# abraj/particleSystem

Hardware: AMD Instinct MI355X
Metric: particle-updates/sec at N=2^20 (higher is better)
Workload: dtype f32

## Files before the change

include/psamd.h:

```cpp
#ifndef PSAMD_H
#define PSAMD_H

#include <stddef.h>
#include <stdint.h>

#ifdef __cplusplus
extern "C" {
#endif

#define PSAMD_ABI_VERSION 8

#define PSAMD_MAX_RANKS 64

typedef enum psamd_status {
    PSAMD_OK = 0,
    PSAMD_ERR_INVALID_ARG   = 1,
    PSAMD_ERR_NO_DEVICE     = 2,
    PSAMD_ERR_HIP           = 3,
    PSAMD_ERR_OUT_OF_MEMORY = 4,
    PSAMD_ERR_OUTSIDE_BOX   = 5,
    PSAMD_ERR_QUEUE_EMPTY   = 6,
    PSAMD_ERR_CELL_OVERFLOW = 7,
    PSAMD_ERR_STATE         = 8,
    PSAMD_ERR_UNSUPPORTED   = 9
// ... 185 lines not shown
int psamd_build_grid(psamd_ctx *ctx);
int psamd_calc_forces(psamd_ctx *ctx);
int psamd_calc_forces_pairs(psamd_ctx *ctx);
int psamd_calc_forces_apply(psamd_ctx *ctx);
int psamd_step(psamd_ctx *ctx, int32_t nsteps);
int psamd_synchronize(psamd_ctx *ctx);
int psamd_set_run_ahead(psamd_ctx *ctx, int steps);

int psamd_download_force4(psamd_ctx *ctx, void *out_float4, int64_t first, int64_t count);

int psamd_snapshot_save(psamd_ctx *ctx);
int psamd_snapshot_restore(psamd_ctx *ctx);

typedef struct psamd_slab_plan {
    int32_t world, rank, grid_dim;
    int32_t cut_lo, cut_hi;
    int32_t state_lo, state_hi;
    int32_t below_lo, below_hi;
    int32_t above_lo, above_hi;
    int32_t lentin_lo, lentin_hi;
    int32_t lentout_lo, lentout_hi;
    int32_t send_up_lo, send_up_hi;
    int32_t send_down_lo, send_down_hi;
    int32_t slot_lo[4], slot_hi[4];
    int32_t rec_lo[4], rec_hi[4];
    int32_t up_rank, down_rank;
} psamd_slab_plan;
int psamd_slab_plan_describe(const psamd_config *cfg, psamd_slab_plan *out);
int psamd_get_slab_plan(const psamd_ctx *ctx, psamd_slab_plan *out);

typedef struct psamd_slab_buffers {
    void   *halo_out[2], *halo_in[2];
    int64_t halo_out_bytes[2], halo_in_bytes[2];
    void   *force_out, *force_in;
    int64_t force_out_bytes, force_in_bytes;
    void   *xfer_out[2], *xfer_in[2];
    int64_t xfer_bytes;
    void   *status_out, *status_in;
    int64_t status_bytes;
    void   *allg_out, *allg_in;
    int64_t allg_bytes;
    void   *xfer2_out[2], *xfer2_in[2];
    int64_t xfer2_bytes;
    void   *far_out, *far_in;
    int64_t far_bytes;
    int64_t xfer_bytes_max;
} psamd_slab_buffers;
int psamd_slab_buffers_get(psamd_ctx *ctx, psamd_slab_buffers *out);

int psamd_slab_build(psamd_ctx *ctx);
int psamd_slab_pairs_interior(psamd_ctx *ctx);
int psamd_slab_pairs(psamd_ctx *ctx);
int psamd_slab_apply(psamd_ctx *ctx);
int psamd_slab_finish(psamd_ctx *ctx);
int psamd_slab_msg_download(psamd_ctx *ctx, int which, void *host, int64_t bytes);
int psamd_slab_msg_upload(psamd_ctx *ctx, int which, const void *host, int64_t bytes);

int psamd_set_stream(psamd_ctx *ctx, void *hip_stream);
int psamd_get_stream(psamd_ctx *ctx, void **hip_stream_out);

int psamd_set_graphs(psamd_ctx *ctx, int enabled);
int psamd_get_graph_stats(psamd_ctx *ctx, int64_t *launches, int64_t *captures);
int psamd_set_wait_policy(psamd_ctx *ctx, int policy);

int psamd_export_live(psamd_ctx *ctx, const psamd_export *spec);
int psamd_download_live(psamd_ctx *ctx, uint32_t fields, void *pos4, void *vel4, void *acc4, int32_t *id,
                        int32_t *cell, int64_t capacity, int64_t *count);
int psamd_live_stats_get(psamd_ctx *ctx, psamd_live_stats *out);

int psamd_inject(psamd_ctx *ctx, const psamd_inject_spec *spec);
int psamd_inject_result_get(psamd_ctx *ctx, psamd_inject_result *out);

int psamd_remove(psamd_ctx *ctx, const psamd_remove_spec *spec);
int psamd_remove_result_get(psamd_ctx *ctx, psamd_remove_result *out);

int psamd_potential(psamd_ctx *ctx, const psamd_potential_spec *spec);
int psamd_potential_result_get(psamd_ctx *ctx, psamd_potential_result *out);
int psamd_download_potential(psamd_ctx *ctx, float *phi, int64_t capacity, psamd_potential_result *out);

int psamd_get_counters(psamd_ctx *ctx, psamd_counters *out);
int psamd_live_count(psamd_ctx *ctx, int64_t *out);
int psamd_device_view_get(psamd_ctx *ctx, psamd_device_view *out);
int psamd_debug_wave_trace(psamd_ctx *ctx, uint64_t *out, int64_t n_words);

int psamd_selftest_math(psamd_ctx *ctx, uint32_t lo_bits, uint32_t hi_bits, uint64_t out24[24]);
#define PSAMD_NUM_TIMERS 9
int psamd_set_timing(psamd_ctx *ctx, int level);
int psamd_set_timing_period(psamd_ctx *ctx, int every);
int psamd_get_timing(psamd_ctx *ctx, double us_out[PSAMD_NUM_TIMERS], int64_t *launches);
int psamd_get_timing_stats(psamd_ctx *ctx, double median_us[PSAMD_NUM_TIMERS], double max_us[PSAMD_NUM_TIMERS], int64_t *samples);

#ifdef __cplusplus
}
#endif
#endif
```

particlesystem_amd/__init__.py:

```python
import contextlib
import ctypes as C
import os

import numpy as np

from . import build as _build
from .slab import (HALO_OUT as MSG_HALO_OUT, HALO_IN as MSG_HALO_IN, FORCE_OUT as MSG_FORCE_OUT, FORCE_IN as MSG_FORCE_IN,
                   XFER_OUT as MSG_XFER_OUT, XFER_IN as MSG_XFER_IN, STATUS_OUT as MSG_STATUS_OUT, STATUS_IN as MSG_STATUS_IN,
                   ALLG_OUT as MSG_ALLG_OUT, ALLG_IN as MSG_ALLG_IN, XFER2_OUT as MSG_XFER2_OUT, XFER2_IN as MSG_XFER2_IN,
                   FAR_OUT as MSG_FAR_OUT, FAR_IN as MSG_FAR_IN)

HERE = os.path.dirname(os.path.abspath(__file__))
LIB_PATH = os.environ.get("PSAMD_LIB") or os.path.join(HERE, "libpsamd.so")

ABI_VERSION = 8
MAX_RANKS = 64
FLAG_EXPLOSIONS = 0x1
FLAG_FAST_MATH = 0x2
FLAG_ALL_PAIRS = 0x4
FLAG_EULER = 0x8
NUM_TIMERS = 9
TIMER_NAMES = ("hist", "scan", "scatter", "sort_cells", "pairs", "apply", "lifecycle", "init_iframe", "collide")

P_DTYPE = np.dtype({
# ... 139 lines not shown

def merge_potential(results):
    results = list(results)
    return {"listed": sum(int(r["listed"]) for r in results), "nonfinite": sum(int(r["nonfinite"]) for r in results),
            "potential": float(sum(float(r["potential"]) for r in results)),
            "phi_min": float(min(float(r["phi_min"]) for r in results)), "phi_max": float(max(float(r["phi_max"]) for r in results))}


def merge_live_stats(stats):
    stats = list(stats)
    out = {}
    for n, _ in LiveStats._fields_:
        vals = [np.asarray(s[n], np.float64) for s in stats]
        if n in ("lo", "age_min"):
            v = np.minimum.reduce(vals)
        elif n in ("hi", "age_max"):
            v = np.maximum.reduce(vals)
        else:
            v = vals[0]
            for x in vals[1:]:
                v = v + x
        out[n] = int(v) if n in ("live", "nonfinite") else (v if v.ndim else float(v))
    return out


class PsamdError(RuntimeError):
    def __init__(self, status, message):
        super().__init__("psamd status %d: %s" % (status, message))
        self.status = status


_vp, _i32, _i64 = C.c_void_p, C.c_int32, C.c_int64
_fp = C.POINTER(C.c_float)
_ip = C.POINTER(C.c_int32)
ABI = [
    ("psamd_abi_version", C.c_int, []),
    ("psamd_status_string", C.c_char_p, [C.c_int]),
    ("psamd_default_config", C.c_int, [C.POINTER(Config)]),
    ("psamd_create", C.c_int, [C.POINTER(Config), C.POINTER(_vp)]),
    ("psamd_destroy", C.c_int, [_vp]),
    ("psamd_last_error", C.c_char_p, [_vp]),
    ("psamd_get_sizes", C.c_int, [_vp, C.POINTER(Sizes)]),
    ("psamd_describe", C.c_int, [C.POINTER(Config), C.POINTER(Sizes), _vp, _vp, _vp, _vp]),
    ("psamd_get_config", C.c_int, [_vp, C.POINTER(Config)]),
    ("psamd_fill_particles", C.c_int, [_vp, _i64, _vp, _vp, _vp, _vp, _vp, _vp, C.POINTER(_i64)]),
    ("psamd_uniform_cloud", C.c_int, [_vp, _i64, C.c_uint32, _vp]),
    ("psamd_upload_particles", C.c_int, [_vp, _vp, _i64, _i64]),
    ("psamd_download_particles", C.c_int, [_vp, _vp, _i64, _i64]),
    ("psamd_download_tdata", C.c_int, [_vp, _vp, _i64, _i64]),
    ("psamd_upload_queues", C.c_int, [_vp, _vp, _vp]),
    ("psamd_download_queues", C.c_int, [_vp, _vp, _vp]),
    ("psamd_download_cellgrid", C.c_int, [_vp, _vp]),
    ("psamd_download_chunkgrid", C.c_int, [_vp, _vp]),
    ("psamd_download_force_counts", C.c_int, [_vp, _vp]),
    ("psamd_get_pkgdistrib", C.c_int, [_vp, _vp]),
    ("psamd_get_cell_table", C.c_int, [_vp, _vp]),
    ("psamd_get_gridmax", C.c_int, [_vp, _ip]),
    ("psamd_init_iframe", C.c_int, [_vp]),
    ("psamd_build_grid", C.c_int, [_vp]),
    ("psamd_calc_forces", C.c_int, [_vp]),
    ("psamd_calc_forces_pairs", C.c_int, [_vp]),
    ("psamd_calc_forces_apply", C.c_int, [_vp]),
    ("psamd_step", C.c_int, [_vp, _i32]),
    ("psamd_synchronize", C.c_int, [_vp]),
    ("psamd_download_force4", C.c_int, [_vp, _vp, _i64, _i64]),
    ("psamd_snapshot_save", C.c_int, [_vp]),
    ("psamd_snapshot_restore", C.c_int, [_vp]),
    ("psamd_set_stream", C.c_int, [_vp, _vp]),
    ("psamd_get_stream", C.c_int, [_vp, C.POINTER(C.c_void_p)]),
    ("psamd_slab_plan_describe", C.c_int, [C.POINTER(Config), C.POINTER(SlabPlan)]),
    ("psamd_get_slab_plan", C.c_int, [_vp, C.POINTER(SlabPlan)]),
    ("psamd_slab_buffers_get", C.c_int, [_vp, C.POINTER(SlabBuffers)]),
    ("psamd_slab_build", C.c_int, [_vp]),
    ("psamd_slab_pairs_interior", C.c_int, [_vp]),
    ("psamd_slab_pairs", C.c_int, [_vp]),
    ("psamd_slab_apply", C.c_int, [_vp]),
    ("psamd_slab_finish", C.c_int, [_vp]),
    ("psamd_slab_msg_download", C.c_int, [_vp, C.c_int, _vp, _i64]),
    ("psamd_slab_msg_upload", C.c_int, [_vp, C.c_int, _vp, _i64]),
    ("psamd_get_counters", C.c_int, [_vp, C.POINTER(Counters)]),
    ("psamd_live_count", C.c_int, [_vp, C.POINTER(_i64)]),
    ("psamd_device_view_get", C.c_int, [_vp, C.POINTER(DeviceView)]),
    ("psamd_debug_wave_trace", C.c_int, [_vp, _vp, _i64]),
    ("psamd_selftest_math", C.c_int, [_vp, C.c_uint32, C.c_uint32, C.POINTER(C.c_uint64)]),
    ("psamd_set_graphs", C.c_int, [_vp, C.c_int]),
    ("psamd_get_graph_stats", C.c_int, [_vp, C.POINTER(_i64), C.POINTER(_i64)]),
    ("psamd_set_wait_policy", C.c_int, [_vp, C.c_int]),
    ("psamd_set_timing", C.c_int, [_vp, C.c_int]),
    ("psamd_set_timing_period", C.c_int, [_vp, C.c_int]),
    ("psamd_get_timing", C.c_int, [_vp, C.POINTER(C.c_double), C.POINTER(_i64)]),
    ("psamd_get_timing_stats", C.c_int, [_vp, C.POINTER(C.c_double), C.POINTER(C.c_double), C.POINTER(_i64)]),
    ("psamd_set_run_ahead", C.c_int, [_vp, C.c_int]),
    ("psamd_set_tdata_mirror", C.c_int, [_vp, C.c_int]),
    ("psamd_export_live", C.c_int, [_vp, C.POINTER(Export)]),
    ("psamd_download_live", C.c_int, [_vp, C.c_uint32, _vp, _vp, _vp, _vp, _vp, _i64, C.POINTER(_i64)]),
    ("psamd_live_stats_get", C.c_int, [_vp, C.POINTER(LiveStats)]),
    ("psamd_inject", C.c_int, [_vp, C.POINTER(Inject)]),
    ("psamd_inject_result_get", C.c_int, [_vp, C.POINTER(InjectResult)]),
    ("psamd_remove", C.c_int, [_vp, C.POINTER(Remove)]),
    ("psamd_remove_result_get", C.c_int, [_vp, C.POINTER(RemoveResult)]),
    ("psamd_potential", C.c_int, [_vp, C.POINTER(Potential)]),
    ("psamd_potential_result_get", C.c_int, [_vp, C.POINTER(PotentialResult)]),
    ("psamd_download_potential", C.c_int, [_vp, _vp, _i64, C.POINTER(PotentialResult)]),
]

_lib = None


def build(force=False):
    return _build.build(force=force)


def load():
    global _lib
    if _lib is None:
        if not os.path.exists(LIB_PATH):
            raise RuntimeError("libpsamd.so is not built (run particlesystem_amd.build()); "
                               "the HIP library is the only implementation, there is no fallback")
        lib = C.CDLL(LIB_PATH)
        for name, res, args in ABI:
            fn = getattr(lib, name)
            fn.restype = res
            fn.argtypes = args
        have = lib.psamd_abi_version()
        if have != ABI_VERSION:
            raise RuntimeError("%s has ABI version %d, this module is written for %d: rebuild it (particlesystem_amd.build(force=True))"
                               % (LIB_PATH, have, ABI_VERSION))
        _lib = lib
    return _lib


def default_config(**over):
    cfg = Config()
    load().psamd_default_config(C.byref(cfg))
    for k, v in over.items():
        if k == "cuts":
            for i, c in enumerate(v):
                cfg.cuts[i] = c
        else:
            setattr(cfg, k, v)
    return cfg


def slab_plan(cfg):
    lib = load()
    plan = SlabPlan()
    st = lib.psamd_slab_plan_describe(C.byref(cfg), C.byref(plan))
    if st != 0:
        raise PsamdError(st, lib.psamd_status_string(st).decode())
    return plan


def _ptr(a):
    return None if a is None else a.ctypes.data_as(C.c_void_p)


def describe(cfg):
    lib = load()
    sizes = Sizes()
    st = lib.psamd_describe(C.byref(cfg), C.byref(sizes), None, None, None, None)
    if st != 0:
        raise PsamdError(st, lib.psamd_status_string(st).decode())
    table = np.zeros((sizes.num_cells, 3), np.int32)
    pkg = np.zeros((sizes.num_chunks, 54), np.int32)
    qi = np.zeros(sizes.queue_info_size, Q_DTYPE)
    q = np.zeros(sizes.container_size, np.int32)
# ... 310 lines not shown
            spec.flags = REMOVE_BOX | (REMOVE_OUTSIDE if outside else 0)
            for k in range(3):
                spec.lo[k], spec.hi[k] = float(box[0][k]), float(box[1][k])
        else:
            assert ids is not None and not outside, "remove: ids or box"
            m = int(ids.shape[0])
            assert ids.dtype == torch.int32 and ids.dim() == 1 and ids.is_contiguous() and ids.is_cuda, "remove: bad ids tensor"
            spec.max_count = m
            spec.ids = ids.data_ptr() if m > 0 else None
            if count is not None:
                assert count.dtype == torch.int64 and tuple(count.shape) == (1,) and count.is_cuda, "remove: bad count tensor"
                spec.count_dev = count.data_ptr()
            if outcome:
                out = torch.full((max(m, 1),), -1, dtype=torch.int32, device=dev)
                spec.outcome_dev = out.data_ptr()
        with self._on_stream(dev):
            self._ck(self.lib.psamd_remove(self.h, C.byref(spec)))
        res = self.remove_result()
        if out is not None:
            res["outcome"] = out[:int(ids.shape[0])]
        return res

    def remove_result(self):
        r = RemoveResult()
        self._ck(self.lib.psamd_remove_result_get(self.h, C.byref(r)))
        return r.to_dict()

    def potential(self, phi=False, capacity=None):
        import torch
        dev = torch.device("cuda", int(self.cfg.device))
        spec = Potential()
        result = torch.zeros(C.sizeof(PotentialResult), dtype=torch.uint8, device=dev)
        spec.result_dev = result.data_ptr()
        out = count = None
        if phi:
            capacity = self.owned_slots() if capacity is None else int(capacity)
            out = torch.empty(max(capacity, 1), dtype=torch.float32, device=dev)
            count = torch.zeros(1, dtype=torch.int64, device=dev)
            spec.phi, spec.capacity = out.data_ptr(), capacity
        with self._on_stream(dev):
            self._ck(self.lib.psamd_potential(self.h, C.byref(spec)))
            if phi:
                self._ck(self.lib.psamd_export_live(self.h, C.byref(Export(fields=0, capacity=0, count_dev=count.data_ptr()))))
        res = PotentialResult.from_device(result).to_dict()
        if phi:
            res["phi"] = out[:min(int(count.item()), capacity)]
        return res

    def potential_result(self):
        r = PotentialResult()
        self._ck(self.lib.psamd_potential_result_get(self.h, C.byref(r)))
        return r.to_dict()

    def download_potential(self, phi=True, capacity=None):
        r = PotentialResult()
        if not phi:
            self._ck(self.lib.psamd_download_potential(self.h, None, 0, C.byref(r)))
            return r.to_dict()
        capacity = self.owned_slots() if capacity is None else int(capacity)
        out = np.full(max(capacity, 1), np.nan, np.float32)
        self._ck(self.lib.psamd_download_potential(self.h, _ptr(out), capacity, C.byref(r)))
        res = r.to_dict()
        n = C.c_int64()
        self._ck(self.lib.psamd_download_live(self.h, 0, None, None, None, None, None, 0, C.byref(n)))
        res["phi"] = out[:min(n.value, capacity)]
        return res

    def energy(self):
        u = self.potential()["potential"]
        k = float(self.live_stats()["kinetic"])
        return {"kinetic": k, "potential": u, "total": k + u}

    def device_view(self):
        v = DeviceView()
        self._ck(self.lib.psamd_device_view_get(self.h, C.byref(v)))
        return v

    def wave_trace(self):
        n = 3 * (self.sizes.num_cells * ((self.sizes.max_per_cell + 63) // 64) + 4)
        out = np.zeros(n, np.uint64)
        self._ck(self.lib.psamd_debug_wave_trace(self.h, _ptr(out), n))
        return out.reshape(-1, 3)

    def selftest_math(self, lo_bits, hi_bits):
        out = (C.c_uint64 * 24)()
        self._ck(self.lib.psamd_selftest_math(self.h, lo_bits, hi_bits, out))
        return list(out)

    def set_graphs(self, on=True):
        self._ck(self.lib.psamd_set_graphs(self.h, 1 if on else 0))

    def graph_stats(self):
        a, b = C.c_int64(), C.c_int64()
        self._ck(self.lib.psamd_get_graph_stats(self.h, C.byref(a), C.byref(b)))
        return a.value, b.value

    def set_wait_policy(self, policy):
        self._ck(self.lib.psamd_set_wait_policy(self.h, int(policy)))

    def set_tdata_mirror(self, on):
        self._ck(self.lib.psamd_set_tdata_mirror(self.h, 1 if on else 0))

    def set_run_ahead(self, steps):
        self._ck(self.lib.psamd_set_run_ahead(self.h, int(steps)))

    def set_timing(self, on=True, every_stage=False, period=1):
        self._ck(self.lib.psamd_set_timing_period(self.h, int(period)))
        self._ck(self.lib.psamd_set_timing(self.h, (2 if every_stage else 1) if on else 0))

    def timing(self):
        us = (C.c_double * NUM_TIMERS)()
        n = C.c_int64()
        self._ck(self.lib.psamd_get_timing(self.h, us, C.byref(n)))
        return dict(zip(TIMER_NAMES, list(us))), n.value

    def timing_stats(self):
        med, mx = (C.c_double * NUM_TIMERS)(), (C.c_double * NUM_TIMERS)()
        n = C.c_int64()
        self._ck(self.lib.psamd_get_timing_stats(self.h, med, mx, C.byref(n)))
        return dict(zip(TIMER_NAMES, list(med))), dict(zip(TIMER_NAMES, list(mx))), n.value
```

particlesystem_amd/csrc/apply.hip:

```cpp
#include "kernels_common.hpp"

namespace psamd {

struct ApplyEmit {
    int id, new_cell, new_rec, old_chunk;
    unsigned bits;
};

__global__ __launch_bounds__(1024) void k_apply(DevParams P, SegLayout S, const StepState *__restrict__ stp,
                                                const uint8_t *__restrict__ flag_slot,
                                                float4 *pos4, float4 *vel4, float4 *acc4,
                                                int *cell_arr, uint8_t *pflags,
                                                const CellInfo *__restrict__ celltab,
                                                uint64_t *op_keys, int *op_args, int ops_cap,
                                                MoveRec *moves, int moves_cap,
                                                Outboxes out,
                                                const int *__restrict__ chunk_count, const uint8_t *__restrict__ chunk_skip,
                                                FrameScalars *fs, DevCounters *ctr)
{
    constexpr int ITEMS = 1;
    __shared__ int s_ops, s_moves, s_base_ops, s_base_moves;
    __shared__ unsigned int s_cnt[4];
    if (threadIdx.x == 0) { s_ops = 0; s_moves = 0; s_cnt[0] = s_cnt[1] = s_cnt[2] = s_cnt[3] = 0; }
    const int chunk_over = fs->chunk_over;
    const int step = (P.flags & PSAMD_FLAG_EXPLOSIONS) ? stp->step : 0;
    int old_cells[ITEMS];
    bool any_active = false;
#pragma unroll
    for (int it = 0; it < ITEMS; it++) {
        const int si = (blockIdx.x * ITEMS + it) * 1024 + (int)threadIdx.x;
        int oc = -1;
        if (si < P.slots_total) oc = cell_arr[si];
        if (oc <= -2) { cell_arr[si] = -1; oc = -1; }
        bool act = oc >= 0 && oc < P.num_cells_global;
        if (chunk_over && act && chunk_count[celltab[oc].chunk] > P.max_per_chunk && chunk_skip[si]) act = false;
        old_cells[it] = act ? oc : -1;
        any_active |= act;
    }
    if (!__syncthreads_or(any_active)) return;

    ApplyEmit em[ITEMS];
    int n_op = 0, n_mv = 0;
    unsigned cnt_moved = 0, cnt_surv = 0, cnt_age = 0, cnt_coll = 0;
#pragma unroll
    for (int it = 0; it < ITEMS; it++) {
        const int si = (blockIdx.x * ITEMS + it) * 1024 + (int)threadIdx.x;
        const int old_cell = old_cells[it];
        const bool active = old_cell >= 0;
        const int id = active ? slot_of_index(P, si) : 0;

    int flag = 0, new_cell = 0;
    float4 f = make_float4(0.f, 0.f, 0.f, 0.f);
    float4 p = f, v = f;
    float fert = 0.f;
    uint8_t pf0 = 0;
    if (active) { p = pos4[si]; v = vel4[si]; f = acc4[si]; pf0 = pflags[si]; flag = (int)flag_slot[si]; fert = f.w; }
    const CellInfo old_ci = active ? celltab[old_cell] : CellInfo{0, 1, 0, 0};

    const bool killed = active && flag == 2, survived = active && flag == 1, moved = active && flag == 0;
    bool died_of_age = false, born = false, relocate = false;
    int new_rec = 0;

    if (killed) {
        died_of_age = v.w > P.life_thr;
        cell_arr[si] = -1; pflags[si] = 0;
        pos4[si] = make_float4(0.f, 0.f, 0.f, 0.f);
        vel4[si] = make_float4(0.f, 0.f, 0.f, 0.f);
        acc4[si] = make_float4(0.f, 0.f, 0.f, 0.f);
    } else if (survived) {
        vel4[si] = make_float4(0.f, 0.f, 0.f, 0.f);
        acc4[si] = make_float4(0.f, 0.f, 0.f, fert);
        pflags[si] = 0;
    } else if (moved) {
        float axv = f.x, ayv = f.y, azv = f.z;
        const float t = P.t;
        if (P.drag > 0.f) { axv -= P.drag * v.x; ayv -= P.drag * v.y; azv -= P.drag * v.z; }
        float dx = (float)((double)(v.x * t) + ((0.5 * (double)axv) * (double)t) * (double)t);
        float dy = (float)((double)(v.y * t) + ((0.5 * (double)ayv) * (double)t) * (double)t);
        float dz = (float)((double)(v.z * t) + ((0.5 * (double)azv) * (double)t) * (double)t);
        if (P.flags & PSAMD_FLAG_EULER) { dx = v.x * t; dy = v.y * t; dz = v.z * t; }
        dx = clamp_mag(dx, P.dmax); dy = clamp_mag(dy, P.dmax); dz = clamp_mag(dz, P.dmax);
        float rx = p.x + dx, ry = p.y + dy, rz = p.z + dz;

        const int G = P.G;
        const double cs = P.cell_size;
        auto to_int = [](double d) { return (d >= -2147483648.0 && d < 2147483648.0) ? (int)d : (int)0x80000000; };
        int i1 = to_int(floor((-1.0 * (double)ry) / cs) + (double)(G / 2));
        int i2 = to_int(floor((1.0 * (double)rx) / cs) + (double)(G / 2));
        int i3 = to_int(floor((-1.0 * (double)rz) / cs) + (double)(G / 2));
        for (int guard = 0; guard < 64 &&
             !((i1 >= 0 && i1 < G) && (i2 >= 0 && i2 < G) && (i3 >= 0 && i3 < G)); guard++) {
            if (!(i1 >= 0 && i1 < G)) { const int o = i1; i1 = (i1 + G) % G; ry = (float)((double)ry + (-1.0 * (double)(i1 - o) * cs)); }
            if (!(i2 >= 0 && i2 < G)) { const int o = i2; i2 = (i2 + G) % G; rx = (float)((double)rx + ((double)(i2 - o) * cs)); }
            if (!(i3 >= 0 && i3 < G)) { const int o = i3; i3 = (i3 + G) % G; rz = (float)((double)rz + (-1.0 * (double)(i3 - o) * cs)); }
        }
        i1 = min(max(i1, 0), G - 1); i2 = min(max(i2, 0), G - 1); i3 = min(max(i3, 0), G - 1);
        new_cell = i3 * G * G + i1 * G + i2;

        float vx = v.x + axv * t, vy = v.y + ayv * t, vz = v.z + azv * t;
        vx = clamp_mag(vx, P.vmax); vy = clamp_mag(vy, P.vmax); vz = clamp_mag(vz, P.vmax);
        const float age = v.w + t;
        uint8_t pf = pf0;
        const CellInfo new_ci = celltab[new_cell];
        new_rec = segment_record(S, new_ci.seg_type, new_ci.seg_tid);

        if ((P.flags & PSAMD_FLAG_EXPLOSIONS) && (age >= fert) && !(pf & 1)) {
            const uint64_t h0 = splitmix64(P.seed ^ ((uint64_t)(uint32_t)step << 32) ^ (uint64_t)(uint32_t)id);
            const uint64_t h1 = splitmix64(h0), h2 = splitmix64(h1);
            const int r0 = (int)((double)(h0 >> 11) * (1.0 / 9007199254740992.0) * 100.0) - 50;
            const int r1 = (int)((double)(h1 >> 11) * (1.0 / 9007199254740992.0) * 100.0) - 50;
            const int r2 = (int)((double)(h2 >> 11) * (1.0 / 9007199254740992.0) * 100.0) - 50;
            float ux = (float)r0, uy = (float)r1, uz = (float)r2;
            const float mag = sqrtf((float)((double)(ux * ux) + (double)(uy * uy) + (double)(uz * uz)));
            ux /= mag; uy /= mag; uz /= mag;
            vx = (float)((double)ux * P.expl_speed);
            vy = (float)((double)uy * P.expl_speed);
            vz = (float)((double)uz * P.expl_speed);
            pf |= 1;
            born = true;
        }
        pos4[si] = make_float4(rx, ry, rz, p.w);
        vel4[si] = make_float4(vx, vy, vz, age);
        if (P.drag > 0.f) acc4[si] = make_float4(axv, ayv, azv, fert);
        cell_arr[si] = new_cell;
        pflags[si] = pf;
        relocate = (new_ci.seg_type != old_ci.seg_type || new_ci.seg_tid != old_ci.seg_tid);
    }

    const bool remote_ = (born || relocate) && P.world > 1 && !owns_record(P, new_rec);
    const int GG = P.G * P.G;
    const int layers_up = ((new_cell / GG) - (old_cell / GG) + P.G) % P.G;
    bool up_ = remote_ && (layers_up == 1 || layers_up == 2);
    bool hop2_ = false, far_ = false;
    if (remote_ && !nbr_owns_record(P, up_ ? 1 : 0, new_rec)) {
        const bool near2 = layers_up == 1 || layers_up == 2 || layers_up >= P.G - 2;
        if (nbr_owns_record(P, up_ ? 0 : 1, new_rec)) up_ = !up_;
        else if (P.xfer2_cap > 0 && (near2 || P.far_cap <= 0)) hop2_ = true;
        else if (P.far_cap > 0) far_ = true;
        else atomicOr(&fs->error, ERR_FOREIGN_CELL);
    }

        em[it].id = id; em[it].new_cell = new_cell; em[it].new_rec = new_rec; em[it].old_chunk = old_ci.chunk;
        em[it].bits = (killed ? 1u : 0u) | (born ? 2u : 0u) | (relocate ? 4u : 0u) | (remote_ ? 8u : 0u) | (up_ ? 16u : 0u) | (hop2_ ? 32u : 0u) | (far_ ? 64u : 0u);
        n_op += (killed ? 1 : 0) + ((born && !remote_) ? 1 : 0) + (relocate ? (remote_ ? 1 : 2) : 0);
        n_mv += (born ? 1 : 0) + (relocate ? 1 : 0);
        cnt_moved += (unsigned)__popcll(__ballot(moved)); cnt_surv += (unsigned)__popcll(__ballot(survived));
        cnt_age += (unsigned)__popcll(__ballot(killed && died_of_age)); cnt_coll += (unsigned)__popcll(__ballot(killed && !died_of_age));
    }
// ... 9 lines not shown
        if (cnt_surv) atomicAdd(&s_cnt[1], cnt_surv);
        if (cnt_age) atomicAdd(&s_cnt[2], cnt_age);
        if (cnt_coll) atomicAdd(&s_cnt[3], cnt_coll);
    }
    wave_ops = __shfl(wave_ops, 63); wave_moves = __shfl(wave_moves, 63);
    __syncthreads();
    if (threadIdx.x == 0) {
        DevCounters *mine = ctr + (blockIdx.x % COUNTER_COPIES);
        if (s_cnt[0]) atomicAdd(&mine->integrated, (unsigned long long)s_cnt[0]);
        if (s_cnt[1]) atomicAdd(&mine->survives, (unsigned long long)s_cnt[1]);
        if (s_cnt[2]) atomicAdd(&mine->deaths_age, (unsigned long long)s_cnt[2]);
        if (s_cnt[3]) atomicAdd(&mine->deaths_collision, (unsigned long long)s_cnt[3]);
        if (s_ops | s_moves) {
            const unsigned long long both = ((unsigned long long)(unsigned)s_moves << 32) | (unsigned)s_ops;
            const unsigned long long old = atomicAdd((unsigned long long *)&fs->n_ops, both);
            s_base_ops = (int)(old & 0xffffffffull); s_base_moves = (int)(old >> 32);
        }
    }
    __syncthreads();
    int k = s_base_ops + wave_ops + op_incl - n_op;
    int m = s_base_moves + wave_moves + mv_incl - n_mv;
    const bool room = k + n_op <= ops_cap && m + n_mv <= moves_cap;
    if (!room && (n_op || n_mv)) atomicOr(&fs->error, ERR_OPS_OVERFLOW);
#pragma unroll
    for (int it = 0; it < ITEMS; it++) {
        const unsigned bits = (room && (n_op || n_mv)) ? em[it].bits : 0u;
        const bool killed = bits & 1u, born = bits & 2u, relocate = bits & 4u, remote = bits & 8u, up = bits & 16u, hop2 = bits & 32u, far = bits & 64u;
        const int id = em[it].id, new_cell = em[it].new_cell;
        const int own_r = segment_record_of_slot(S, id);
        const int box = far ? 4 : (up ? 1 : 0) + (hop2 ? 2 : 0);
        int out_base[2] = {0, 0};
        if (P.world > 1) {
#pragma unroll
            for (int dir = 0; dir < 5; dir++) {
                if (dir >= 2 && (dir == 4 ? P.far_cap : P.xfer2_cap) <= 0) continue;
                const bool mine = remote && box == dir;
                const int want = mine ? ((born ? 1 : 0) + (relocate ? 1 : 0)) : 0;
                if (__any(want > 0)) {
                    const int incl = wave_incl_scan(want);
                    int base = 0;
                    if (lane == 63) base = atomicAdd(&fs->n_out[dir], incl);
                    base = __shfl(base, 63) + incl - want;
                    if (mine) { out_base[1] = base; out_base[0] = base + (born ? 1 : 0); }
                }
            }
        }
        if (!(bits & 7u)) continue;
        const uint64_t key = ((uint64_t)(uint32_t)(em[it].old_chunk + 1) << P.key_chunk_shift) | ((uint64_t)(uint32_t)id << 2);
        const uint64_t own_rec = (uint64_t)(uint32_t)own_r << P.key_rec_shift;
        const uint64_t dst_rec = (uint64_t)(uint32_t)em[it].new_rec << P.key_rec_shift;
        auto depart = [&](int kind, uint64_t sub) -> int {
            const int o = out_base[kind];
            if (o >= (far ? P.far_cap : hop2 ? P.xfer2_cap : P.xfer_cap)) { atomicOr(&fs->error, ERR_HALO_OVERFLOW); return -1; }
            XferRec *x = out.o[box] + o;
            x->key = dst_rec | key | sub; x->new_cell = new_cell; x->kind = kind;
            return o;
        };
        if (killed) { op_keys[k] = own_rec | key | 2ull; op_args[k] = id; k++; }
        if (born) {
            if (remote) moves[m] = {id, depart(1, 0ull), 1 | MOVE_OUT | (up ? MOVE_UP : 0) | (hop2 ? MOVE_HOP2 : 0) | (far ? MOVE_FAR : 0), new_cell};
            else {
                moves[m] = {id, -1, 1, new_cell};
                op_keys[k] = dst_rec | key | 0ull; op_args[k] = m;
                k++;
            }
            m++;
        }
        if (relocate) {
            if (remote) moves[m] = {id, depart(0, 1ull), 0 | MOVE_OUT | (up ? MOVE_UP : 0) | (hop2 ? MOVE_HOP2 : 0) | (far ? MOVE_FAR : 0), new_cell};
            else {
                moves[m] = {id, -1, 0, new_cell};
                op_keys[k] = dst_rec | key | 1ull; op_args[k] = m;
                k++;
            }
            m++;
            op_keys[k] = own_rec | key | 2ull; op_args[k] = id; k++;
        }
    }
}

hipError_t launch_apply(hipStream_t st, const DevParams &P, const SegLayout &S, const DeviceState &d)
{
    if (P.slots_total <= 0) return hipSuccess;
    k_apply<<<(P.slots_total + 1023) / 1024, 1024, 0, st>>>(P, S, d.st, d.flag_slot, d.pos4, d.vel4, d.acc4, d.cell, d.pflags, d.celltab,
                                                        d.op_keys, d.op_args, d.ops_cap, d.moves, d.moves_cap,
                                                        Outboxes{{d.xfer_out[0], d.xfer_out[1], d.xfer_out[2], d.xfer_out[3], d.xfer_out[4]}},
                                                        d.chunk_count, d.chunk_skip, d.fs, d.ctr);
    PS_LAUNCH_CHECK();
    return hipSuccess;
}

}
```

particlesystem_amd/csrc/create.hip:

```cpp
#include <cmath>
#include <new>

#include "context.hpp"

const char *psamd::status_text(int s)
{
    switch (s) {
    case PSAMD_OK: return "ok";
    case PSAMD_ERR_INVALID_ARG: return "invalid argument";
    case PSAMD_ERR_NO_DEVICE: return "no usable HIP device (the HIP path is the only path)";
    case PSAMD_ERR_HIP: return "HIP runtime error";
    case PSAMD_ERR_OUT_OF_MEMORY: return "out of device memory";
    case PSAMD_ERR_OUTSIDE_BOX: return "particle location outside box";
    case PSAMD_ERR_QUEUE_EMPTY: return "overflow: reserved space of the segment is full";
    case PSAMD_ERR_CELL_OVERFLOW: return "cell or queue-op capacity exceeded on device";
    case PSAMD_ERR_STATE: return "stage called out of order";
    case PSAMD_ERR_UNSUPPORTED: return "unsupported";
    }
    return "unknown status";
}

extern "C" {

int psamd_abi_version(void) { return PSAMD_ABI_VERSION; }
// ... 171 lines not shown
    d.cell_count = frame; d.chunk_count = frame + LC; d.rec_count = d.chunk_count + g.num_chunks;
    d.rec_cursor = d.rec_count + g.queue_infos;
    d.halo_count = d.rec_cursor + g.queue_infos;
    d.active_count = d.halo_count + LC;
    d.task_ready = d.active_count + LC;
    c->frame_ints = frame_ints;
    PS_HIP(c, dev_alloc(c, &d.halo_f, (size_t)3 * LC * HALO_CAP + 64));
    PS_HIP(c, dev_alloc(c, &d.halo_id, LC * HALO_CAP + 64));
    PS_HIP(c, dev_alloc(c, &d.active_list, SC));
    PS_HIP(c, dev_alloc(c, &d.snap_cid, SC));
    PS_HIP(c, dev_alloc(c, &d.task_list2, LC * P.slices));
    PS_HIP(c, dev_alloc(c, &d.merged_tasks, LC));
    PS_HIP(c, dev_alloc(c, &d.task_cost, LC));
    PS_HIP(c, dev_alloc(c, &d.ctask_start, 2 * LC + 2));
    PS_HIP(c, dev_alloc(c, &d.cost_start, 2 * LC + 2));
    PS_HIP(c, dev_alloc(c, &d.wave_pos, (size_t)MAX_PAIR_WAVES + 1));
    PS_HIP(c, dev_alloc(c, &d.rec_start, (size_t)g.queue_infos + 1));
    PS_HIP(c, dev_alloc(c, &d.fs, 1));
    PS_HIP(c, dev_alloc(c, &d.st, 1));
    PS_HIP(c, hipMemsetAsync(d.st, 0, sizeof(StepState), c->stream));
    PS_HIP(c, dev_alloc(c, &d.cell_start, LC + 1));
    PS_HIP(c, dev_alloc(c, &d.cursor, LC));
    PS_HIP(c, dev_alloc(c, &d.task_start, LC + 1));
    PS_HIP(c, dev_alloc(c, &d.task_list, LC * P.slices));
    PS_HIP(c, dev_alloc(c, &d.sorted_id, SC));
    PS_HIP(c, dev_alloc(c, &d.flag_slot, C));
    PS_HIP(c, dev_alloc(c, &d.snap_soa, 4 * (size_t)P.sorted_cap + 64));
    PS_HIP(c, dev_alloc(c, &d.snap_age, SC));
    PS_HIP(c, dev_alloc(c, &d.force4, SC));
    PS_HIP(c, dev_alloc(c, &d.celltab, (size_t)g.num_cells));
    if (P.flags & PSAMD_FLAG_ALL_PAIRS) {
        d.part_tasks = (int)(SC / 64 + 1);
        PS_HIP(c, dev_alloc(c, &d.part_acc, (size_t)ALLP_PARTS * d.part_tasks * 64));
        PS_HIP(c, dev_alloc(c, &d.act_start, LC + 1));
        PS_HIP(c, dev_alloc(c, &d.dense_gi, SC));
        PS_HIP(c, dev_alloc(c, &d.dense_cell, SC));
    }
    PS_HIP(c, dev_alloc(c, &d.chunk_skip, C));
    PS_HIP(c, dev_alloc(c, &d.chunk_segs, (size_t)g.num_chunks * 27));
    {
        std::vector<int2> segs((size_t)g.num_chunks * 27);
        for (int ch = 0; ch < g.num_chunks; ch++) {
            Pair pk[27];
            g.chunk_segments(ch, pk);
            for (int j = 0; j < 27; j++) {
                const int k = seg_index(pk[j].c);
                segs[(size_t)ch * 27 + j] = make_int2(g.seg_base[k] + pk[j].p * g.seg_size_t[k], g.seg_size_t[k]);
            }
            std::sort(segs.begin() + (size_t)ch * 27, segs.begin() + (size_t)ch * 27 + 27, [](const int2 &a, const int2 &b) { return a.x < b.x; });
        }
        PS_HIP(c, hipMemcpy(d.chunk_segs, segs.data(), segs.size() * sizeof(int2), hipMemcpyHostToDevice));
    }
    PS_HIP(c, dev_alloc(c, &d.op_keys, (size_t)d.ops_cap));
    PS_HIP(c, dev_alloc(c, &d.op_keys_sorted, (size_t)d.ops_cap));
    PS_HIP(c, dev_alloc(c, &d.op_args, (size_t)d.ops_cap));
    PS_HIP(c, dev_alloc(c, &d.op_args_sorted, (size_t)d.ops_cap));
    PS_HIP(c, hipHostMalloc((void **)&c->h_fs, 2 * sizeof(FrameScalars), hipHostMallocMapped | hipHostMallocCoherent));
    std::memset(c->h_fs, 0, 2 * sizeof(FrameScalars));
    PS_HIP(c, hipHostGetDevicePointer((void **)&c->d.fs_host, c->h_fs, 0));
    PS_HIP(c, dev_alloc(c, &d.moves, (size_t)d.moves_cap));
    PS_HIP(c, dev_alloc(c, &d.stage, 3 * (size_t)d.moves_cap));
    PS_HIP(c, dev_alloc(c, &d.ctr, (size_t)COUNTER_COPIES));
    PS_HIP(c, dev_alloc(c, &d.exp_count, (size_t)slot_tiles(P.slots_total)));
    PS_HIP(c, dev_alloc(c, &d.exp_tiles, (size_t)slot_tiles(P.slots_total)));
    PS_HIP(c, dev_alloc(c, &d.exp_out, 1));
    PS_HIP(c, dev_alloc(c, &d.pot_sorted, SC));
    PS_HIP(c, dev_alloc(c, &d.pot_slot, C));
    PS_HIP(c, dev_alloc(c, &d.pot_tiles, (size_t)slot_tiles(P.slots_total)));
    PS_HIP(c, dev_alloc(c, &d.pot_count, (size_t)slot_tiles(P.slots_total)));
    PS_HIP(c, dev_alloc(c, &d.pot_out, 1));
    PS_HIP(c, hipMemsetAsync(d.pot_out, 0, sizeof(PotOut), c->stream));
    PS_HIP(c, dev_alloc(c, &c->inj.removed, (size_t)g.queue_infos));
    PS_HIP(c, dev_alloc(c, &c->inj.hdr, 2));
    PS_HIP(c, dev_alloc(c, &c->inj.own, 1));
    PS_HIP(c, hipMemsetAsync(c->inj.own, 0, sizeof(psamd_inject_result), c->stream));
    PS_HIP(c, dev_alloc(c, &c->rem.claim, C));
    PS_HIP(c, dev_alloc(c, &c->rem.ins, (size_t)g.queue_infos));
    PS_HIP(c, dev_alloc(c, &c->rem.prefix, C + 1));
    PS_HIP(c, dev_alloc(c, &c->rem.tile_sel, (size_t)slot_tiles(P.slots_total)));
    PS_HIP(c, dev_alloc(c, &c->rem.tile_live, (size_t)slot_tiles(P.slots_total)));
    PS_HIP(c, dev_alloc(c, &c->rem.own, 1));
    PS_HIP(c, hipMemsetAsync(c->rem.own, 0, sizeof(psamd_remove_result), c->stream));
    PS_HIP(c, dev_alloc(c, &d.trace, 3 * (LC * P.slices + 4)));
    PS_HIP(c, hipMemsetAsync(d.trace, 0, 3 * (LC * P.slices + 4) * sizeof(unsigned long long), c->stream));
    return PSAMD_OK;
}

static hipError_t alloc_msg(psamd_ctx *c, int which, size_t bytes, size_t alloc = 0)
{
    SlabMsg &m = c->msg[which];
    m.bytes = bytes; m.alloc = alloc ? alloc : bytes;
    const hipError_t e = dev_alloc(c, &m.ptr, m.alloc / sizeof(int));
    return e != hipSuccess ? e : hipMemsetAsync(m.ptr, 0, m.alloc, c->stream);
}

static int alloc_slab_msgs(psamd_ctx *c)
{
    const Geometry &g = c->geo; const DevParams &P = c->P; const SlabPlan &pl = c->plan; DeviceState &d = c->d;
    if (P.world <= 1) return PSAMD_OK;
    const int GG = g.G * g.G;
    auto halo_bytes = [&](int cells) { return ((size_t)MSG_HEADER_WORDS + (size_t)cells + 6 * (size_t)cells * P.halo_cap_cell) * sizeof(int); };
        c->halo_out_cells[0] = (pl.send_down_hi - pl.send_down_lo) * GG; c->halo_out_c0[0] = (pl.send_down_lo - pl.state_lo) * GG;
        c->halo_out_cells[1] = (pl.send_up_hi - pl.send_up_lo) * GG;     c->halo_out_c0[1] = (pl.send_up_lo - pl.state_lo) * GG;
        c->halo_in_cells[0] = (pl.below_hi - pl.below_lo) * GG;
        c->halo_in_cells[1] = (pl.above_hi - pl.above_lo) * GG;
    for (int k = 0; k < 2; k++) {
        if (c->halo_out_cells[k] > 0) {
            PS_HIP(c, alloc_msg(c, MSG_HALO_OUT + k, halo_bytes(c->halo_out_cells[k])));
            PS_HIP(c, dev_alloc(c, &c->pack_off[k], (size_t)c->halo_out_cells[k] + 1));
        }
        if (c->halo_in_cells[k] > 0) {
            PS_HIP(c, alloc_msg(c, MSG_HALO_IN + k, halo_bytes(c->halo_in_cells[k])));
            PS_HIP(c, dev_alloc(c, &c->unpack_off[k], (size_t)c->halo_in_cells[k] + 1));
        }
    }
    auto force_bytes = [&](int cells) { return ((size_t)MSG_HEADER_WORDS + 4 * (size_t)cells * P.halo_cap_cell) * sizeof(int); };
    if (P.reg_layers[2] > 0) PS_HIP(c, alloc_msg(c, MSG_FORCE_OUT, force_bytes(P.reg_layers[2] * GG)));
    if (P.lentout_c1 > P.lentout_c0) PS_HIP(c, alloc_msg(c, MSG_FORCE_IN, force_bytes(P.lentout_c1 - P.lentout_c0)));
    for (int k = 0; k < 2; k++) {
        PS_HIP(c, alloc_msg(c, MSG_XFER_OUT + k, xfer_msg_bytes((size_t)P.xfer_cap + 1), xfer_msg_bytes(xfer_room(P))));
        PS_HIP(c, alloc_msg(c, MSG_XFER_IN + k, xfer_msg_bytes((size_t)P.xfer_cap + 1), xfer_msg_bytes(xfer_room(P))));
    }
    for (int k = 0; k < 2 && P.xfer2_cap > 0; k++) {
        PS_HIP(c, alloc_msg(c, MSG_XFER2_OUT + k, xfer_msg_bytes((size_t)P.xfer2_cap)));
        PS_HIP(c, alloc_msg(c, MSG_XFER2_IN + k, xfer_msg_bytes((size_t)P.xfer2_cap)));
    }
    if (P.far_cap > 0) {
        PS_HIP(c, alloc_msg(c, MSG_FAR_OUT, xfer_msg_bytes((size_t)P.far_cap)));
        PS_HIP(c, alloc_msg(c, MSG_FAR_IN, xfer_msg_bytes((size_t)P.far_cap) * (size_t)P.world));
    }
    const int outbox[5] = {MSG_XFER_OUT, MSG_XFER_OUT + 1, MSG_XFER2_OUT, MSG_XFER2_OUT + 1, MSG_FAR_OUT};
    for (int k = 0; k < 5; k++)
        if (c->msg[outbox[k]].ptr) d.xfer_out[k] = reinterpret_cast<XferRec *>(c->msg[outbox[k]].ptr + MSG_HEADER_WORDS);
    if (P.flags & PSAMD_FLAG_ALL_PAIRS) {
        const size_t block = (size_t)P.allg_block * sizeof(int);
        PS_HIP(c, alloc_msg(c, MSG_ALLG_OUT, block));
        PS_HIP(c, alloc_msg(c, MSG_ALLG_IN, block * P.world, block * P.world + 64 * sizeof(int)));
            PS_HIP(c, dev_alloc(c, &d.gstart, (size_t)g.num_cells + 1));
            PS_HIP(c, dev_alloc(c, &d.gn, (size_t)g.num_cells + 1));
            PS_HIP(c, hipMemsetAsync(d.gstart, 0, ((size_t)g.num_cells + 1) * sizeof(int), c->stream));
            PS_HIP(c, hipMemsetAsync(d.gn, 0, ((size_t)g.num_cells + 1) * sizeof(int), c->stream));
        d.allg_in = c->msg[MSG_ALLG_IN].ptr;
    }
    PS_HIP(c, alloc_msg(c, MSG_STATUS_OUT, (size_t)P.status_words * sizeof(int)));
    PS_HIP(c, alloc_msg(c, MSG_STATUS_IN, (size_t)P.status_words * sizeof(int) * P.world));
    d.status_out = c->msg[MSG_STATUS_OUT].ptr;
    return PSAMD_OK;
}

static int probe_eps_f32(psamd_ctx *c, const psamd_config *cfg)
{
    DevParams &P = c->P;
    if (P.lean_math && cfg->eps2 > 0) {
        const float d2_max = (float)max_d2(c->geo);
        unsigned long long *bad = (unsigned long long *)c->d.fs;
        auto fbits = [](float f) { uint32_t u; std::memcpy(&u, &f, 4); return u; };
        for (double mult : {1.5, 2.0, 4.0, 8.0, 16.0, 64.0}) {
            const float from = (float)(mult * cfg->eps2);
            if (!(from < d2_max)) break;
            unsigned long long h_bad = 1;
            PS_HIP(c, hipMemsetAsync(bad, 0, sizeof(unsigned long long), c->stream));
            PS_HIP(c, launch_validate_eps(c->stream, fbits(from), fbits(d2_max), cfg->eps2, P.eps2f, bad));
            PS_HIP(c, hipMemcpyAsync(&h_bad, bad, sizeof h_bad, hipMemcpyDeviceToHost, c->stream));
            PS_HIP(c, hipStreamSynchronize(c->stream));
            if (h_bad == 0) { P.eps_f32_from = from; break; }
        }
    }
    P.slow_below = std::max(P.eps_f32_from, std::nextafterf(P.coll_d2_gate, INFINITY));
    return PSAMD_OK;
}

static void split_interior(psamd_ctx *c)
{
    const Geometry &g = c->geo; const DevParams &P = c->P; const SlabPlan &pl = c->plan;
    const int GG = g.G * g.G, lo = std::max(pl.cut_lo, pl.state_lo), hi = std::min(pl.cut_hi, pl.state_hi);
    auto own = [&](int l) { return l < 0 || l >= g.G || (l >= pl.state_lo && l < pl.state_hi); };
    int i0 = lo, i1 = lo;
    for (int l = lo; l < hi; l++) if (own(l - 1) && own(l + 1)) { if (i1 == i0) i0 = l; i1 = l + 1; } else if (i1 > i0) break;
    c->P_int = P; c->P_rest = P;
    c->have_interior = P.world > 1 && P.two_pass && P.lean_math && i1 > i0 && (i1 - i0) < (hi - lo) + (pl.lentin_hi - pl.lentin_lo)
                       && !(P.flags & PSAMD_FLAG_ALL_PAIRS);
    if (c->have_interior) {
        const int a = (i0 - pl.state_lo) * GG, b = (i1 - pl.state_lo) * GG;
        c->P_int.comp_lo[0] = a; c->P_int.comp_hi[0] = b;
        c->P_int.comp_lo[1] = c->P_int.comp_hi[1] = c->P_int.comp_lo[2] = c->P_int.comp_hi[2] = 0;
        c->P_rest.comp_lo[1] = P.own_comp0; c->P_rest.comp_hi[1] = a;
        c->P_rest.comp_lo[2] = b; c->P_rest.comp_hi[2] = P.own_comp1;
    }
}

static int init_state(psamd_ctx *c)
{
    const Geometry &g = c->geo; const DevParams &P = c->P; DeviceState &d = c->d;
    const size_t C = (size_t)P.slots_total, SC = (size_t)P.sorted_cap + 64, LC = (size_t)P.n_local_cells;
    c->wait_policy = P.world > 1 ? 1 : 0;
    if (const char *lim = std::getenv("PSAMD_WAIT_LIMIT_S")) c->wait_limit_s = std::max(0.05, std::atof(lim));
    for (float4 *a : {d.pos4, d.vel4, d.acc4}) PS_HIP(c, hipMemsetAsync(a, 0, std::max<size_t>(C, 1) * sizeof(float4), c->stream));
    PS_HIP(c, hipMemsetAsync(d.pflags, 0, std::max<size_t>(C, 1), c->stream));
    PS_HIP(c, hipMemsetAsync(d.force4, 0, SC * sizeof(float4), c->stream));
    PS_HIP(c, hipMemsetAsync(d.flag_slot, 0, std::max<size_t>(C, 1), c->stream));
    PS_HIP(c, hipMemsetAsync(d.fs, 0, sizeof(FrameScalars), c->stream));
    PS_HIP(c, hipMemsetAsync(d.ctr, 0, sizeof(DevCounters) * COUNTER_COPIES, c->stream));
    PS_HIP(c, hipMemsetAsync(d.cell_count, 0, c->frame_ints * sizeof(int), c->stream));
    PS_HIP(c, hipMemsetAsync(d.cell_start, 0, (LC + 1) * sizeof(int), c->stream));
    PS_HIP(c, launch_fill_int(c->stream, d.cell, -1, C));
    PS_HIP(c, launch_fill_int(c->stream, c->rem.claim, INT32_MAX, C));
    PS_HIP(c, launch_init_tdata(c->stream, P, d));
    g.initial_queues(c->h_qinfo, c->h_queue);
    c->celltab = g.cell_table();
    PS_HIP(c, hipMemcpyAsync(d.celltab, c->celltab.data(), c->celltab.size() * sizeof(CellInfo), hipMemcpyHostToDevice, c->stream));
    {
        const int cell_off = P.reg_first[0] * g.G * g.G;
        std::vector<int> order((size_t)std::max(P.n_own_cells, 1), 0);
        for (int lc = 0; lc < P.n_own_cells; lc++) order[(size_t)lc] = lc;
        std::stable_sort(order.begin(), order.begin() + P.n_own_cells, [&](int a, int b) {
            const CellInfo &x = c->celltab[(size_t)(a + cell_off)], &y = c->celltab[(size_t)(b + cell_off)];
            if (x.chunk != y.chunk) return x.chunk < y.chunk;
            if (x.seg_type != y.seg_type) return x.seg_type < y.seg_type;
            return x.seg_tid < y.seg_tid;
        });
        PS_HIP(c, dev_alloc(c, &d.cell_order, order.size()));
        PS_HIP(c, hipMemcpy(d.cell_order, order.data(), order.size() * sizeof(int), hipMemcpyHostToDevice));
    }
    return push_queues(c);
}

int psamd_create(const psamd_config *cfg, psamd_ctx **out)
{
    if (!cfg || !out) return PSAMD_ERR_INVALID_ARG;
    *out = nullptr;
    psamd_ctx *c = new (std::nothrow) psamd_ctx();
    if (!c) return PSAMD_ERR_OUT_OF_MEMORY;
    *out = c;
    if (!c->geo.init(*cfg)) return fail(c, PSAMD_ERR_INVALID_ARG, "bad configuration (chunk_dim >= 3, sizes > 0, container < 2^31)");
    if (cfg->world < 1 || cfg->world > PSAMD_MAX_RANKS || cfg->rank < 0 || cfg->rank >= cfg->world) return fail(c, PSAMD_ERR_INVALID_ARG, "rank/world");
    const Geometry &g = c->geo;
    c->plan = plan_for(g, *cfg);
    if (!c->plan.valid) return fail(c, PSAMD_ERR_UNSUPPORTED, "no slab partition for this grid and world size (every rank needs >= 2 cell layers "
                                                                "and its neighbours must hold every layer it reads)");

    int ndev = 0;
    if (hipGetDeviceCount(&ndev) != hipSuccess || ndev <= 0) return fail(c, PSAMD_ERR_NO_DEVICE, "hipGetDeviceCount found none");
    if (cfg->device < 0 || cfg->device >= ndev) return fail(c, PSAMD_ERR_NO_DEVICE, "device ordinal out of range");
    PS_HIP(c, hipSetDevice(cfg->device));
    PS_HIP(c, hipStreamCreateWithFlags(&c->own_stream, hipStreamNonBlocking));
    c->stream = c->own_stream;
    PS_HIP(c, hipStreamCreateWithFlags(&c->d.side_stream, hipStreamNonBlocking));
    PS_HIP(c, hipEventCreateWithFlags(&c->d.ev_fork, hipEventDisableTiming));
    PS_HIP(c, hipEventCreateWithFlags(&c->d.ev_join, hipEventDisableTiming));

    int rc = derive_params(c, cfg);
    if (rc == PSAMD_OK) rc = alloc_step_arrays(c);
    if (rc == PSAMD_OK) rc = alloc_slab_msgs(c);
    if (rc == PSAMD_OK) rc = probe_eps_f32(c, cfg);
    if (rc != PSAMD_OK) return rc;
    split_interior(c);
    return init_state(c);
}

int psamd_destroy(psamd_ctx *c)
{
    if (!c) return PSAMD_OK;
    if (c->stream) (void)hipStreamSynchronize(c->stream);
    drop_graphs(c);
    for (void *p : c->allocs) (void)hipFree(p);
    if (c->staging) (void)hipFree(c->staging);
    for (const EntryScratch &e : {c->inj.e, c->rem.e})
        for (void *p : {(void *)e.ent, (void *)e.tcount, (void *)e.tile_out}) if (p) (void)hipFree(p);
    if (c->h_fs) (void)hipHostFree(c->h_fs);
    if (c->ev_made) for (auto &set : c->ev) for (auto &e : set) (void)hipEventDestroy(e);
    if (c->d.ev_fork) (void)hipEventDestroy(c->d.ev_fork);
    if (c->d.ev_join) (void)hipEventDestroy(c->d.ev_join);
    if (c->d.side_stream) (void)hipStreamDestroy(c->d.side_stream);
    if (c->own_stream) (void)hipStreamDestroy(c->own_stream);
    delete c;
    return PSAMD_OK;
}

static void fill_sizes(const Geometry &g, psamd_sizes *o)
{
    std::memset(o, 0, sizeof *o);
    o->grid_dim = g.G; o->num_cells = g.num_cells; o->num_chunks = g.num_chunks;
    o->cells_per_chunk = g.cells_per_chunk; o->max_per_cell = g.max_per_cell; o->max_per_chunk = g.max_per_chunk;
    o->container_size = g.container; o->queue_info_size = g.queue_infos;
    o->n_chunkgrid = (int64_t)g.num_chunks * (1 + (int64_t)g.max_per_chunk);
    o->n_cellgrid = (int64_t)g.num_cells * (1 + (int64_t)g.max_per_cell);
    o->n_pkgdistrib = g.num_chunks * 27;
    for (int k = 0; k < 4; k++) { o->seg_count[k] = g.seg_count[k]; o->seg_size_t[k] = g.seg_size_t[k]; o->seg_size[k] = g.seg_size[k]; }
// ... 66 lines not shown
```

particlesystem_amd/csrc/grid.hip:

```cpp
#include "kernels_common.hpp"

namespace psamd {

__global__ void k_unpack_aos(DevParams P, const uint32_t *__restrict__ aos, int first, int count, float half_box,
                             float4 *pos4, float4 *vel4, float4 *acc4, int *cell, uint8_t *pflags,
                             FrameScalars *fs)
{
    const int i = blockIdx.x * blockDim.x + threadIdx.x;
    if (i >= count) return;
    const uint32_t *r = aos + (size_t)18 * i;
    const int slot = first + i;
    if ((int)r[0] != slot) atomicOr(&fs->error, ERR_BAD_ID);
    const int si = slot_index(P, slot);
    if (si < 0) return;
    if ((int)r[1] >= 0) {
        const float x = __uint_as_float(r[9]), y = __uint_as_float(r[10]), z = __uint_as_float(r[11]);
        bool bad = (int)r[1] >= P.num_cells_global;
        if (!bad) {
            const int c = (int)r[1], G = P.G, i3 = c / (G * G), i1 = (c - i3 * G * G) / G, i2 = c - i3 * G * G - i1 * G;
            const float cs = (float)P.cell_size, tol = 1e-4f * cs, h = (float)(G / 2);
            int lost = (int)0x80000000;
            for (int guard = 0; guard < 4 && !(lost >= 0 && lost < G); guard++) lost = (lost + G) % G;
            auto axis_ok = [&](float v, float sign, int idx) {
                if ((__float_as_uint(v) & 0x7f800000u) == 0x7f800000u) return idx == lost;
                if (!(fabsf(v) <= half_box)) return false;
                const float u = (sign * v / cs + h - (float)idx) * cs;
                return u >= -tol && u <= cs + tol;
            };
            bad = !(axis_ok(x, 1.0f, i2) && axis_ok(y, -1.0f, i1) && axis_ok(z, -1.0f, i3));
        }
        if (bad) atomicOr(&fs->error, ERR_BAD_POS);
    }
    cell[si] = (int)r[1];
    if ((int)r[1] < 0) {
        pflags[si] = 0;
        pos4[si] = vel4[si] = acc4[si] = make_float4(0.f, 0.f, 0.f, 0.f);
        return;
    }
    pflags[si] = ((r[5] >> 8) & 0xffu) ? 1 : 0;
    pos4[si] = make_float4(__uint_as_float(r[9]), __uint_as_float(r[10]), __uint_as_float(r[11]), __uint_as_float(r[6]));
    vel4[si] = make_float4(__uint_as_float(r[12]), __uint_as_float(r[13]), __uint_as_float(r[14]), __uint_as_float(r[7]));
    acc4[si] = make_float4(__uint_as_float(r[15]), __uint_as_float(r[16]), __uint_as_float(r[17]), __uint_as_float(r[8]));
}

__global__ void k_pack_aos(DevParams P, uint32_t *__restrict__ aos, int first, int count,
                           const float4 *pos4, const float4 *vel4, const float4 *acc4, const int *cell,
                           const uint8_t *pflags, const CellInfo *celltab)
{
    const int i = blockIdx.x * blockDim.x + threadIdx.x;
    if (i >= count) return;
    uint32_t *r = aos + (size_t)18 * i;
    const int slot = first + i;
    const int si = slot_index(P, slot);
    const int c = si >= 0 ? cell[si] : -1;
    CellInfo ci = {-1, -1, -1, 0};
    if (c >= 0 && c < P.num_cells_global) ci = celltab[c];
    const float4 zero = make_float4(0.f, 0.f, 0.f, 0.f);
    const float4 p = si >= 0 ? pos4[si] : zero, v = si >= 0 ? vel4[si] : zero, a = si >= 0 ? acc4[si] : zero;
    r[0] = (uint32_t)slot; r[1] = (uint32_t)c; r[2] = (uint32_t)ci.chunk;
    r[3] = (uint32_t)ci.seg_type; r[4] = (uint32_t)ci.seg_tid;
    r[5] = (si >= 0 && pflags[si]) ? 0x100u : 0u;
    r[6] = __float_as_uint(p.w); r[7] = __float_as_uint(v.w); r[8] = __float_as_uint(a.w);
    r[9] = __float_as_uint(p.x); r[10] = __float_as_uint(p.y); r[11] = __float_as_uint(p.z);
    r[12] = __float_as_uint(v.x); r[13] = __float_as_uint(v.y); r[14] = __float_as_uint(v.z);
    r[15] = __float_as_uint(a.x); r[16] = __float_as_uint(a.y); r[17] = __float_as_uint(a.z);
}

__global__ void k_place(DevParams P, int n, const int *__restrict__ ids, const float4 *__restrict__ p,
                        const float4 *__restrict__ v, const float4 *__restrict__ a,
                        const int *__restrict__ cells, float4 *pos4, float4 *vel4, float4 *acc4,
                        int *cell, uint8_t *pflags)
{
    const int i = blockIdx.x * blockDim.x + threadIdx.x;
    if (i >= n) return;
    const int si = slot_index(P, ids[i]);
    if (si < 0) return;
    pos4[si] = p[i]; vel4[si] = v[i]; acc4[si] = a[i];
    cell[si] = cells[i]; pflags[si] = 0;
}

__global__ void k_restore(int n, const float4 *__restrict__ s_pos, const float4 *__restrict__ s_vel,
                          const float4 *__restrict__ s_acc, const int *__restrict__ s_cell,
                          const uint8_t *__restrict__ s_flags, const int *__restrict__ s_queue,
                          const int *__restrict__ s_qinfo, int qinfo_words, int step, StepState *st,
                          float4 *pos4, float4 *vel4, float4 *acc4, int *cell, uint8_t *pflags, int *queue, int *qinfo)
{
    const int i = blockIdx.x * blockDim.x + threadIdx.x;
    if (i == 0) { st->step = step; st->pending = 0; }
    if (i < qinfo_words) qinfo[i] = s_qinfo[i];
    if (i >= n) return;
    queue[i] = s_queue[i];
    const int cs = s_cell[i];
    if (cs < 0 && cell[i] < 0) return;
    pos4[i] = s_pos[i]; vel4[i] = s_vel[i]; acc4[i] = s_acc[i];
    cell[i] = cs; pflags[i] = s_flags[i];
}

hipError_t launch_restore(hipStream_t st, int n, const void *s_pos, const void *s_vel, const void *s_acc,
                          const void *s_cell, const void *s_flags, const void *s_queue, const void *s_qinfo, int qinfo_words,
                          int step, const DeviceState &d)
{
    const int threads = std::max(std::max(n, qinfo_words), 1);
    k_restore<<<(threads + 255) / 256, 256, 0, st>>>(n, (const float4 *)s_pos, (const float4 *)s_vel, (const float4 *)s_acc,
                                                    (const int *)s_cell, (const uint8_t *)s_flags, (const int *)s_queue,
                                                    (const int *)s_qinfo, qinfo_words, step, d.st, d.pos4, d.vel4, d.acc4,
                                                    d.cell, d.pflags, d.queue, (int *)d.qinfo);
    return hipGetLastError();
}

__global__ void k_fill_int(int *p, int v, size_t n)
{
    size_t i = (size_t)blockIdx.x * blockDim.x + threadIdx.x;
    const size_t stride = (size_t)gridDim.x * blockDim.x;
    for (; i < n; i += stride) p[i] = v;
}

__global__ void k_init_tdata(DevParams P, uint32_t *tdata)
{
    const int i = blockIdx.x * blockDim.x + threadIdx.x;
    if (i >= P.slots_total) return;
    uint32_t *r = tdata + (size_t)6 * i;
    r[0] = (uint32_t)slot_of_index(P, i); r[1] = r[2] = r[3] = r[4] = r[5] = 0u;
}

__device__ __forceinline__ int hist_window(const DevParams &P, const int (&mine)[SLOTS_PER_WG / 1024], int *s_min)
{
    if (P.n_own_cells <= LDS_CELLS) return 0;
    if (threadIdx.x == 0) *s_min = 0x7fffffff;
    __syncthreads();
    int m = 0x7fffffff;
#pragma unroll
    for (int i = 0; i < SLOTS_PER_WG / 1024; i++) if (mine[i] >= 0) m = min(m, mine[i]);
    for (int d = 32; d > 0; d >>= 1) m = min(m, __shfl_xor(m, d));
    if ((threadIdx.x & 63) == 0 && m != 0x7fffffff) atomicMin(s_min, m);
    __syncthreads();
    return *s_min;
}

constexpr int SCAN_LDS_CHUNKS = 4096;

__global__ __launch_bounds__(1024) void k_hist_lds(DevParams P, const int *__restrict__ cell, int *__restrict__ cell_count,
                                                    FrameScalars *fs, StepState *st)
{
    __shared__ int h[LDS_CELLS];
    __shared__ int s_min;
    const int tid = threadIdx.x, base = blockIdx.x * SLOTS_PER_WG, ncell = P.n_own_cells;
    if (blockIdx.x == 0 && tid == 0 && st->pending) { st->step += 1; st->pending = 0; }
    int mine[SLOTS_PER_WG / 1024];
#pragma unroll
    for (int i = 0; i < SLOTS_PER_WG / 1024; i++) {
        const int si = base + i * 1024 + tid;
        mine[i] = si < P.slots_total ? own_local_cell(P, cell[si], fs) : -1;
    }
    const int w0 = hist_window(P, mine, &s_min);
    if (w0 == 0x7fffffff) return;
    const int span = min(ncell - w0, LDS_CELLS);
    for (int c = tid; c < span; c += 1024) h[c] = 0;
    __syncthreads();
#pragma unroll
    for (int i = 0; i < SLOTS_PER_WG / 1024; i++) {
        const int c = mine[i];
        if (c < 0) continue;
        if (c - w0 < LDS_CELLS) atomicAdd(&h[c - w0], 1); else atomicAdd(&cell_count[c], 1);
    }
    __syncthreads();
    for (int c = tid; c < span; c += 1024) {
        const int v = h[c];
        if (v) atomicAdd(&cell_count[w0 + c], v);
    }
}
template <bool ROWS>
__global__ __launch_bounds__(1024) void k_scatter_lds(DevParams P, int nwg, const int *__restrict__ cell, int *__restrict__ cursor,
                                                       int *__restrict__ sorted_id, const int *__restrict__ chunk_count,
                                                       const CellInfo *__restrict__ celltab, const int2 *__restrict__ chunk_segs,
                                                       uint8_t *__restrict__ chunk_skip,
                                                       const float4 *__restrict__ pos4, const float4 *__restrict__ vel4,
                                                       uint32_t *__restrict__ tdata)
{
    if ((int)blockIdx.x >= nwg) { chunk_cap_block(P, (int)blockIdx.x - nwg, chunk_count, cell, celltab, chunk_segs, chunk_skip, nullptr); return; }
    __shared__ int h[LDS_CELLS];
    __shared__ int s_min;
    const int tid = threadIdx.x, base = blockIdx.x * SLOTS_PER_WG, ncell = P.n_own_cells;
    int mine[SLOTS_PER_WG / 1024];
#pragma unroll
    for (int i = 0; i < SLOTS_PER_WG / 1024; i++) {
        const int si = base + i * 1024 + tid;
        int c = -1;
        if (si < P.slots_total) {
            c = cell[si];
            c = (c < 0 || c >= P.num_cells_global) ? -1 : c - P.reg_first[0] * P.G * P.G;
            if (c < 0 || c >= ncell) c = -1;
        }
        mine[i] = c;
    }
    const int w0 = hist_window(P, mine, &s_min);
    if (w0 == 0x7fffffff) return;
    const int span = min(ncell - w0, LDS_CELLS);
    for (int c = tid; c < span; c += 1024) h[c] = 0;
    __syncthreads();
#pragma unroll
    for (int i = 0; i < SLOTS_PER_WG / 1024; i++)
        if (mine[i] >= 0 && mine[i] - w0 < LDS_CELLS) atomicAdd(&h[mine[i] - w0], 1);
    __syncthreads();
    for (int c = tid; c < span; c += 1024) {
        const int v = h[c];
        if (v) h[c] = atomicAdd(&cursor[w0 + c], v);
    }
    __syncthreads();
#pragma unroll
    for (int i = 0; i < SLOTS_PER_WG / 1024; i++)
        if (mine[i] >= 0) {
            const int c = mine[i];
            const int pos = c - w0 < LDS_CELLS ? atomicAdd(&h[c - w0], 1) : atomicAdd(&cursor[c], 1);
            const int si = base + i * 1024 + tid, id = slot_of_index(P, si);
            sorted_id[pos] = id;
            if (ROWS) {
                const float4 p = pos4[si];
                const float age = vel4[si].w;
                uint2 *t = reinterpret_cast<uint2 *>(tdata + (size_t)6 * si);
                t[0] = make_uint2((uint32_t)id, __float_as_uint(p.x));
                t[1] = make_uint2(__float_as_uint(p.y), __float_as_uint(p.z));
                t[2] = make_uint2(__float_as_uint(p.w), __float_as_uint(age));
            }
        }
}

__global__ __launch_bounds__(1024) void k_scan(DevParams P, const int *__restrict__ cell_count,
                                                int *__restrict__ cell_start, int *__restrict__ cursor,
                                                int *__restrict__ task_start, int *__restrict__ task_list,
                                                int *__restrict__ chunk_count,
                                                const CellInfo *__restrict__ celltab, int *__restrict__ status_out, FrameScalars *fs)
{
    __shared__ long long wave_tot[16];
    __shared__ int maxcell_s, maxraw_s;
    __shared__ int chunk_s[SCAN_LDS_CHUNKS];
    constexpr int LDS_CHUNKS = SCAN_LDS_CHUNKS;
    const int tid = threadIdx.x, lane = tid & 63, wv = tid >> 6;
    const bool chunks_in_lds = P.num_chunks <= LDS_CHUNKS;
    const int ncell = P.n_own_cells, cell_off = P.reg_first[0] * P.G * P.G;
    if (tid == 0) { maxcell_s = 0; maxraw_s = 0; }
    if (chunks_in_lds) for (int ch = tid; ch < P.num_chunks; ch += 1024) chunk_s[ch] = 0;
    __syncthreads();
    const int per = (ncell + 1023) / 1024;
    const int c0 = min(ncell, tid * per), c1 = min(ncell, c0 + per);
    auto word = [&](int c, int v) {
        const bool computed = c >= P.own_comp0 && c < P.own_comp1;
        return ((long long)(computed ? (min(v, P.max_per_cell) + 63) >> 6 : 0) << 32) | (long long)v;
    };
    long long mine = 0;
    int mymax = 0, myraw = 0;
    constexpr int KEEP = 8;
    int kept[KEEP];
    CellInfo kci[KEEP];
#pragma unroll
    for (int k = 0; k < KEEP; k++) kept[k] = (c0 + k < c1) ? cell_count[c0 + k] : 0;
#pragma unroll
    for (int k = 0; k < KEEP; k++) if (kept[k] > 0) kci[k] = celltab[c0 + k + cell_off];
    auto census = [&](int c, int v, const CellInfo &ci) {
        if (chunks_in_lds) atomicAdd(&chunk_s[ci.chunk], v);
        else atomicAdd(&chunk_count[ci.chunk], v);
        if (P.world > 1) atomicAdd(&status_out[STATUS_CHUNK_OFF + 4 * ci.chunk + (ci.seg_type == 1 ? 0 : ci.seg_type == 2 ? 1 : ci.seg_type == 4 ? 2 : 3)], v);
    };
#pragma unroll
    for (int k = 0; k < KEEP; k++) {
        const int c = c0 + k, v = kept[k];
        if (c >= c1) continue;
        mymax = max(mymax, min(v, P.max_per_cell)); myraw = max(myraw, v);
        mine += word(c, v);
        if (v > 0) census(c, v, kci[k]);
    }
    for (int c = c0 + KEEP; c < c1; c++) {
        const int v = cell_count[c];
        mymax = max(mymax, min(v, P.max_per_cell)); myraw = max(myraw, v);
        mine += word(c, v);
        if (v > 0) census(c, v, celltab[c + cell_off]);
    }
    long long incl = mine;
    for (int d = 1; d < 64; d <<= 1) {
        const long long o = __shfl_up(incl, d);
        if (lane >= d) incl += o;
    }
    if (lane == 63) wave_tot[wv] = incl;
    if (mymax) atomicMax(&maxcell_s, mymax);
    if (myraw > P.max_per_cell || myraw > 1024) atomicMax(&maxraw_s, myraw);
    __syncthreads();
    long long run = incl - mine, total = 0;
    for (int k = 0; k < 16; k++) { if (k < wv) run += wave_tot[k]; total += wave_tot[k]; }
    auto place = [&](int c, int v) {
        const int excl = (int)(run & 0xffffffffll);
        cell_start[c] = excl;
        cursor[c] = excl;
        const int t0 = (int)(run >> 32);
        task_start[c] = t0;
        const long long w = word(c, v);
        if (!P.two_pass) for (int sl = 0; sl < (int)(w >> 32); sl++) task_list[t0 + sl] = c * P.slices + sl;
        run += w;
    };
#pragma unroll
    for (int k = 0; k < KEEP; k++) if (c0 + k < c1) place(c0 + k, kept[k]);
    for (int c = c0 + KEEP; c < c1; c++) place(c, cell_count[c]);
    if (tid == 0) {
        cell_start[ncell] = (int)(total & 0xffffffffll);
        task_start[ncell] = (int)(total >> 32);
        fs->live = (int)(total & 0xffffffffll);
        fs->n_tasks = (int)(total >> 32);
        fs->gridmax[1] = maxcell_s;
        fs->max_cell_raw = max(maxraw_s, maxcell_s);
    }
    int cm = 0;
    bool over = false;
    if (chunks_in_lds) {
        for (int ch = tid; ch < P.num_chunks; ch += 1024) {
            const int v = chunk_s[ch];
            chunk_count[ch] = v;
            over |= v > P.max_per_chunk;
            cm = max(cm, min(v, P.max_per_chunk));
        }
    } else {
        __threadfence();
        __syncthreads();
        for (int ch = tid; ch < P.num_chunks; ch += 1024) { const int v = chunk_count[ch]; over |= v > P.max_per_chunk; cm = max(cm, min(v, P.max_per_chunk)); }
    }
    if (cm > 0) atomicMax(&fs->gridmax[0], cm);
    if (over && P.world == 1) fs->chunk_over = 1;
}
template <int CAP>
__device__ __forceinline__ void sort_cell(const DevParams &P, const int c, const bool take_big, const int *__restrict__ cell_start,
                                                     int *__restrict__ sorted_id, int *__restrict__ scratch_ids,
                                                     float4 *pos4, float4 *vel4, float4 *acc4,
                                                     int *cell_arr, uint8_t *pflags,
                                                     float *__restrict__ snap_soa,
                                                     float *__restrict__ snap_age,
                                                     uint64_t *op_keys, int *op_args, int ops_cap,
                                                     int *__restrict__ halo_count, float *__restrict__ halo_f,
                                                     int *__restrict__ halo_id, int *__restrict__ snap_cid,
                                                     int *__restrict__ status_out, FrameScalars *fs, DevCounters *ctr)
{
    constexpr int SMALL = 1024;
    static_assert(CAP == SMALL || CAP == SORT_MAX, "two instances: ordinary cells, crowded cells");
    __shared__ __attribute__((aligned(16))) int ids[CAP + 4];
    __shared__ int ordered[CAP];
    __shared__ int s_halo[27], s_halo_base[27];
    constexpr int BITMAP_WORDS = 512;
    __shared__ unsigned bitmap[BITMAP_WORDS];
    __shared__ int s_lo, s_hi, s_wt[4], s_total;
    const int tid = threadIdx.x;
    if (tid < 27) s_halo[tid] = 0;
    if (tid == 0) { s_lo = 0x7fffffff; s_hi = -1; s_total = 0; }
    const int start = cell_start[c];
    const int n = cell_start[c + 1] - start;
    if (n == 0) return;
    if (CAP == SMALL ? (n > SMALL && !take_big) : n <= SMALL) return;
    const bool in_lds = n <= CAP;
    int ci1, ci2, ci3;
    cell_coords(P, c, ci1, ci2, ci3);
    if (in_lds) for (int e = tid; e < n; e += 256) ids[e] = sorted_id[start + e];
    __syncthreads();
    auto id_at = [&](int e) { return in_lds ? ids[e] : sorted_id[start + e]; };
    int lo = 0x7fffffff, hi = -1;
    for (int e = tid; e < n; e += 256) { const int v = id_at(e); lo = min(lo, v); hi = max(hi, v); }
#pragma unroll
    for (int sft = 32; sft > 0; sft >>= 1) { lo = min(lo, __shfl_xor(lo, sft)); hi = max(hi, __shfl_xor(hi, sft)); }
    if ((tid & 63) == 0) { atomicMin(&s_lo, lo); atomicMax(&s_hi, hi); }
    __syncthreads();
    const int id_lo = s_lo, id_hi = s_hi;
    int *ordered_out = in_lds ? ordered : scratch_ids + start;
    for (int w0 = id_lo; w0 <= id_hi; w0 += BITMAP_WORDS * 32) {
        const int span = min(id_hi - w0 + 1, BITMAP_WORDS * 32), words = (span + 31) >> 5;
        const bool whole = w0 == id_lo && span == id_hi - id_lo + 1;
        for (int w = tid; w < words; w += 256) bitmap[w] = 0;
        __syncthreads();
        for (int e = tid; e < n; e += 256) { const int b = id_at(e) - w0; if (whole || (b >= 0 && b < span)) atomicOr(&bitmap[b >> 5], 1u << (b & 31)); }
        __syncthreads();
        constexpr int WPT = BITMAP_WORDS / 256;
        unsigned w[WPT];
        int cnt = 0;
#pragma unroll
        for (int i = 0; i < WPT; i++) { w[i] = (WPT * tid + i < words) ? bitmap[WPT * tid + i] : 0u; cnt += __popc(w[i]); }
        const int incl = wave_incl_scan(cnt);
        if ((tid & 63) == 63) s_wt[tid >> 6] = incl;
        __syncthreads();
        int pos = s_total + incl - cnt;
        for (int k = 0; k < (tid >> 6); k++) pos += s_wt[k];
#pragma unroll
        for (int i = 0; i < WPT; i++)
            for (unsigned m = w[i]; m; m &= m - 1) ordered_out[pos++] = w0 + (WPT * tid + i) * 32 + (__ffs(m) - 1);
        __syncthreads();
        if (tid == 0) s_total += s_wt[0] + s_wt[1] + s_wt[2] + s_wt[3];
        __syncthreads();
    }
    constexpr int KR = CAP == SMALL ? SMALL / 256 : 1;
    float hx[KR], hy[KR], hz[KR];
    int hid[KR], hm3[KR];
#pragma unroll
    for (int k = 0; k < KR; k++) hm3[k] = 0;
    bool wild_any = false;
    const bool regs = CAP == SMALL && in_lds;
    auto row = [&](int e, int k) {
        const int id = ordered_out[e], si = slot_index(P, id);
        float4 p = pos4[si];
        const float age = vel4[si].w;
        if (age < P.kid_thr) p.x = p.y = p.z = 0.0f;
        if (e < P.max_per_cell) {
            sorted_id[start + e] = id;
            const float w_eff = (age < P.kid_thr) ? 0.0f : (P.force_sign < 0.f ? -p.w : p.w);
            {
                const size_t cap = (size_t)P.sorted_cap;
                snap_soa[start + e] = p.x; snap_soa[cap + start + e] = p.y;
                snap_soa[2 * cap + start + e] = p.z; snap_soa[3 * cap + start + e] = w_eff;
            }
            snap_age[start + e] = age;
            const bool collides = !(age < P.kid_thr) && !(age > P.life_thr);
            snap_cid[start + e] = collides ? id : -1;
            const int m3 = !(halo_count && collides) ? 0 : regs ? halo_dirs_of_numbers(P, ci1, ci2, ci3, p.x, p.y, p.z)
                                                                : halo_dirs(P, ci1, ci2, ci3, p.x, p.y, p.z);
            if (regs && halo_count && collides && !finite3(p.x, p.y, p.z)) wild_any = true;
            if (m3) {
                if (regs) {
#pragma unroll
                    for (int m = 1; m < 8; m++) { const int dir = halo_dir_of_subset(m3, m); if (dir >= 0) atomicAdd(&s_halo[dir], 1); }
                    hx[k] = p.x; hy[k] = p.y; hz[k] = p.z; hid[k] = id; hm3[k] = m3;
                } else
                    for_each_halo_dir(m3, [&](int dir) { atomicAdd(&s_halo[dir], 1); });
            }
        } else {
            sorted_id[start + e] = -1;
            cell_arr[si] = P.world > 1 ? -2 - cell_arr[si] : -1; pflags[si] = 0;
            pos4[si] = make_float4(0.f, 0.f, 0.f, 0.f);
            vel4[si] = make_float4(0.f, 0.f, 0.f, 0.f);
            acc4[si] = make_float4(0.f, 0.f, 0.f, 0.f);
            atomicAdd(&(ctr + (blockIdx.x % COUNTER_COPIES))->cell_overflow_kills, 1ull);
            if (owns_record(P, 0)) {
                const int k2 = atomicAdd(&fs->n_ops, 1);
                if (k2 < ops_cap) { op_keys[k2] = ((uint64_t)(uint32_t)id << 2) | 2ull; op_args[k2] = id; }
                else atomicOr(&fs->error, ERR_OPS_OVERFLOW);
            } else {
                const int k2 = atomicAdd(&status_out[0], 1);
                if (k2 < STATUS_KILL_CAP) status_out[MSG_HEADER_WORDS + k2] = id;
                else atomicOr(&fs->error, ERR_REMOTE_RECORD0);
            }
        }
    };
    if (regs) {
#pragma unroll
        for (int k = 0; k < KR; k++) { const int e = tid + 256 * k; if (e < n) row(e, k); }
    } else {
        for (int e = tid; e < n; e += 256) row(e, 0);
    }
    if (!halo_count) return;
    const bool wild_cell = __syncthreads_or(wild_any);
    if (!regs) {
        list_in_neighbour_halos(P, c, start, min(n, P.max_per_cell), SnapSoa{snap_soa, (size_t)P.sorted_cap}, snap_cid, halo_count, halo_f, halo_id, s_halo, s_halo_base, true);
        return;
    }
    auto for_each_wild = [&](auto fn) {
        const size_t cap = (size_t)P.sorted_cap;
        for (int e = tid; e < min(n, P.max_per_cell); e += 256) {
            const int id = snap_cid[start + e];
            const float x = snap_soa[start + e], y = snap_soa[cap + start + e], z = snap_soa[2 * cap + start + e];
            if (id >= 0 && !finite3(x, y, z)) fn(id, x, y, z);
        }
    };
    if (wild_cell) {
        for_each_wild([&](int, float, float, float) { for (int dir = 0; dir < 27; dir++) if (dir != 13) atomicAdd(&s_halo[dir], 1); });
        __syncthreads();
    }
    if (tid < 27) {
        int base = -1;
        const int cnt = s_halo[tid];
        if (cnt > 0) {
            const int nc = halo_neighbour(P, ci1, ci2, ci3, tid);
            if (nc >= 0) base = atomicAdd(&halo_count[nc], cnt);
        }
        s_halo_base[tid] = base;
        s_halo[tid] = 0;
    }
    __syncthreads();
    const size_t plane = (size_t)P.n_local_cells * HALO_CAP;
#pragma unroll
    for (int k = 0; k < KR; k++) {
        if (!hm3[k]) continue;
#pragma unroll
        for (int m = 1; m < 8; m++) {
            const int dir = halo_dir_of_subset(hm3[k], m);
            if (dir < 0 || s_halo_base[dir] < 0) continue;
            const int kk = s_halo_base[dir] + atomicAdd(&s_halo[dir], 1);
            if (kk < HALO_CAP) {
                const size_t at = (size_t)halo_neighbour(P, ci1, ci2, ci3, dir) * HALO_CAP + kk;
                halo_f[at] = hx[k]; halo_f[plane + at] = hy[k]; halo_f[2 * plane + at] = hz[k];
                halo_id[at] = hid[k];
            }
        }
    }
    if (wild_cell)
        for_each_wild([&](int id, float x, float y, float z) {
            for (int dir = 0; dir < 27; dir++) {
                if (dir == 13 || s_halo_base[dir] < 0) continue;
                const int kk = s_halo_base[dir] + atomicAdd(&s_halo[dir], 1);
                if (kk < HALO_CAP) {
                    const size_t at = (size_t)halo_neighbour(P, ci1, ci2, ci3, dir) * HALO_CAP + kk;
                    halo_f[at] = x; halo_f[plane + at] = y; halo_f[2 * plane + at] = z;
                    halo_id[at] = id;
                }
            }
        });
}

template <int CAP>
__global__ __launch_bounds__(256) void k_sort_cells(DevParams P, int take_big, const int *__restrict__ cell_order, const int *__restrict__ cell_start, int *__restrict__ sorted_id,
                                                     int *__restrict__ scratch_ids,
                                                     float4 *pos4, float4 *vel4, float4 *acc4, int *cell_arr, uint8_t *pflags,
                                                     float *__restrict__ snap_soa, float *__restrict__ snap_age,
                                                     uint64_t *op_keys, int *op_args, int ops_cap,
                                                     int *__restrict__ halo_count, float *__restrict__ halo_f,
                                                     int *__restrict__ halo_id, int *__restrict__ snap_cid,
                                                     int *__restrict__ status_out, FrameScalars *fs, DevCounters *ctr)
{
    if (CAP == 1024) {
        sort_cell<CAP>(P, cell_order[xcd_contiguous((int)blockIdx.x, (int)gridDim.x)], take_big != 0, cell_start, sorted_id, scratch_ids, pos4, vel4, acc4, cell_arr, pflags, snap_soa, snap_age,
                       op_keys, op_args, ops_cap, halo_count, halo_f, halo_id, snap_cid, status_out, fs, ctr);
        return;
    }
    if (fs->max_cell_raw <= 1024) return;
    for (int c = blockIdx.x; c < P.n_own_cells; c += gridDim.x) {
        sort_cell<CAP>(P, c, true, cell_start, sorted_id, scratch_ids, pos4, vel4, acc4, cell_arr, pflags, snap_soa, snap_age,
                       op_keys, op_args, ops_cap, halo_count, halo_f, halo_id, snap_cid, status_out, fs, ctr);
        __syncthreads();
    }
}

hipError_t launch_unpack_aos(hipStream_t st, const DevParams &P, const void *aos, int first, int count, float half_box,
                             const DeviceState &d)
{
    if (count <= 0) return hipSuccess;
    k_unpack_aos<<<(count + 255) / 256, 256, 0, st>>>(P, (const uint32_t *)aos, first, count, half_box,
                                                      d.pos4, d.vel4, d.acc4, d.cell, d.pflags, d.fs);
    PS_LAUNCH_CHECK();
    return hipSuccess;
}

hipError_t launch_pack_aos(hipStream_t st, const DevParams &P, void *aos, int first, int count, const DeviceState &d)
{
    if (count <= 0) return hipSuccess;
    k_pack_aos<<<(count + 255) / 256, 256, 0, st>>>(P, (uint32_t *)aos, first, count, d.pos4, d.vel4,
                                                    d.acc4, d.cell, d.pflags, d.celltab);
    PS_LAUNCH_CHECK();
    return hipSuccess;
}

hipError_t launch_place(hipStream_t st, const DevParams &P, int n, const int *ids, const float4 *p, const float4 *v, const float4 *a,
                        const int *cells, const DeviceState &d)
{
    if (n <= 0) return hipSuccess;
    k_place<<<(n + 255) / 256, 256, 0, st>>>(P, n, ids, p, v, a, cells, d.pos4, d.vel4, d.acc4, d.cell, d.pflags);
    PS_LAUNCH_CHECK();
    return hipSuccess;
}

__global__ void k_frame_reset(int *frame, size_t n, FrameScalars *fs, StepState *st, int *status_out, int status_table)
{
    const size_t i = (size_t)blockIdx.x * blockDim.x + threadIdx.x;
    if (i < n) frame[i] = 0;
    if (i == 0) {
        const int err = fs->error;
        *fs = FrameScalars{};
        fs->error = err;
        if (st->pending) { st->step += 1; st->pending = 0; }
    }
    if (status_out) {
        if (i < (size_t)MSG_HEADER_WORDS) status_out[i] = 0;
        if (i < (size_t)status_table) status_out[STATUS_CHUNK_OFF + i] = 0;
    }
}

hipError_t launch_frame_reset(hipStream_t st, const DeviceState &d, size_t frame_ints, int status_table)
{
    const size_t n = std::max(frame_ints, (size_t)status_table);
    k_frame_reset<<<(unsigned)((n + 1023) / 1024), 1024, 0, st>>>(d.cell_count, frame_ints, d.fs, d.st, d.status_out, d.status_out ? status_table : 0);
    return hipGetLastError();
}
hipError_t launch_fill_int(hipStream_t st, int *p, int v, size_t n)
{
    if (n == 0) return hipSuccess;
    k_fill_int<<<blocks_for(n, 256), 256, 0, st>>>(p, v, n);
    PS_LAUNCH_CHECK();
    return hipSuccess;
}

hipError_t launch_init_tdata(hipStream_t st, const DevParams &P, const DeviceState &d)
{
    if (P.slots_total <= 0) return hipSuccess;
    k_init_tdata<<<(P.slots_total + 255) / 256, 256, 0, st>>>(P, d.tdata);
    PS_LAUNCH_CHECK();
    return hipSuccess;
}

__global__ void k_force_gather(DevParams P, const int *__restrict__ cell_start, const int *__restrict__ sorted_id,
                               const float4 *__restrict__ force4, const float4 *__restrict__ acc4, const uint8_t *__restrict__ flag_slot,
                               float4 *__restrict__ out, int first, int count)
{
    const int i = blockIdx.x * blockDim.x + threadIdx.x;
    if (i >= count) return;
    const int gi = first + i;
    float4 v = make_float4(0.f, 0.f, 0.f, 0.f);
    if (gi < cell_start[P.n_own_cells]) {
        const int id = sorted_id[gi], si = id >= 0 ? slot_index(P, id) : -1;
        if (si >= 0) { const float4 a = acc4[si]; v = make_float4(a.x, a.y, a.z, __int_as_float((int)flag_slot[si])); }
    } else if (gi >= P.reg_sorted[1] && P.world > 1) v = force4[gi];
    out[i] = v;
}

hipError_t launch_force_gather(hipStream_t st, const DevParams &P, const DeviceState &d, void *out, int first, int count)
{
    if (count <= 0) return hipSuccess;
    k_force_gather<<<(count + 255) / 256, 256, 0, st>>>(P, d.cell_start, d.sorted_id, d.force4, d.acc4, d.flag_slot, (float4 *)out, first, count);
    return hipGetLastError();
}

hipError_t launch_build_grid(hipStream_t st, const DevParams &P, const DeviceState &d, hipEvent_t *ev, bool tdata_rows, bool big_cells)
{
    const int nwg = std::max(1, (P.slots_total + SLOTS_PER_WG - 1) / SLOTS_PER_WG);
    if (ev) (void)hipEventRecord(ev[0], st);
    k_hist_lds<<<nwg, 1024, 0, st>>>(P, d.cell, d.cell_count, d.fs, d.st);
    PS_LAUNCH_CHECK();
    if (ev) (void)hipEventRecord(ev[1], st);
    k_scan<<<1, 1024, 0, st>>>(P, d.cell_count, d.cell_start, d.cursor, d.task_start, d.task_list, d.chunk_count, d.celltab, d.status_out, d.fs);
    PS_LAUNCH_CHECK();
    if (ev) (void)hipEventRecord(ev[2], st);
    const int grid = nwg + (P.world == 1 ? P.num_chunks : 0);
    if (tdata_rows) k_scatter_lds<true><<<grid, 1024, 0, st>>>(P, nwg, d.cell, d.cursor, d.sorted_id, d.chunk_count, d.celltab, d.chunk_segs, d.chunk_skip, d.pos4, d.vel4, d.tdata);
    else k_scatter_lds<false><<<grid, 1024, 0, st>>>(P, nwg, d.cell, d.cursor, d.sorted_id, d.chunk_count, d.celltab, d.chunk_segs, d.chunk_skip, d.pos4, d.vel4, d.tdata);
    PS_LAUNCH_CHECK();
    if (ev) (void)hipEventRecord(ev[3], st);
    k_sort_cells<1024><<<P.n_own_cells, 256, 0, st>>>(P, big_cells ? 0 : 1, d.cell_order, d.cell_start, d.sorted_id, d.active_list, d.pos4, d.vel4, d.acc4, d.cell,
                                               d.pflags, d.snap_soa, d.snap_age, d.op_keys, d.op_args, d.ops_cap,
                                               P.two_pass ? d.halo_count : nullptr, d.halo_f, d.halo_id, d.snap_cid, d.status_out, d.fs, d.ctr);
    PS_LAUNCH_CHECK();
    if (big_cells) {
        k_sort_cells<SORT_MAX><<<std::min(P.n_own_cells, 512), 256, 0, st>>>(P, 1, d.cell_order, d.cell_start, d.sorted_id, d.active_list, d.pos4, d.vel4, d.acc4, d.cell,
                                               d.pflags, d.snap_soa, d.snap_age, d.op_keys, d.op_args, d.ops_cap,
                                               P.two_pass ? d.halo_count : nullptr, d.halo_f, d.halo_id, d.snap_cid, d.status_out, d.fs, d.ctr);
        PS_LAUNCH_CHECK();
    }
    if (ev) (void)hipEventRecord(ev[4], st);
    return hipSuccess;
}

}
```

particlesystem_amd/csrc/inject.hip:

```cpp
#include "multisplit.hpp"

namespace psamd {

constexpr int INJ_NOT_MINE = -1, INJ_OUTSIDE = -2;

__device__ __forceinline__ bool inject_locate(const DevParams &P, float x, float y, float z, int &cell)
{
    const double cs = P.cell_size, h = (double)(P.G / 2), g = (double)P.G;
    const double d1 = floor((-1.0 * (double)y) / cs) + h;
    const double d2 = floor((1.0 * (double)x) / cs) + h;
    const double d3 = floor((-1.0 * (double)z) / cs) + h;
    if (!(d1 >= 0.0 && d1 < g && d2 >= 0.0 && d2 < g && d3 >= 0.0 && d3 < g)) return false;
    cell = ((int)d3 * P.G + (int)d1) * P.G + (int)d2;
    return true;
}

template <bool LDS>
__global__ void __launch_bounds__(SPLIT_THREADS) k_inject_locate(DevParams P, SegLayout S, int nrec, const CellInfo *__restrict__ celltab,
                                                                 const float4 *__restrict__ pos4, int64_t max_count, const int64_t *count_dev,
                                                                 int2 *__restrict__ ent, int *__restrict__ tcount, int *__restrict__ tile_out)
{
    extern __shared__ int lds_cnt[];
    __shared__ int s_first_out;
    const int n = entry_count(count_dev, max_count);
    const int t = (int)blockIdx.x;
    if (t * ENTRY_TILE >= n) return;
    if (threadIdx.x == 0) s_first_out = INT_MAX;
    SplitKeys k;
    split_tile_begin<LDS>(t, nrec, lds_cnt, tcount, k);
    int first_out = INT_MAX;
#pragma unroll
    for (int g = 0; g < SPLIT_GROUPS; g++) {
        const int i = split_entry(t, g);
        int r = INJ_NOT_MINE;
        if (i < n) {
            const float4 p = pos4[i];
            int cell;
            if (!inject_locate(P, p.x, p.y, p.z, cell)) { r = INJ_OUTSIDE; first_out = min(first_out, i); }
            else {
                const CellInfo ci = celltab[cell];
                const int sr = segment_record(S, ci.seg_type, ci.seg_tid);
                r = owns_record(P, sr) ? sr : INJ_NOT_MINE;
            }
        }
        k.rec[g] = r;
        split_group_rank(r, (int)threadIdx.x & 63, k.in_rank[g], k.pop[g], k.lead[g]);
    }
    if (first_out != INT_MAX) atomicMin(&s_first_out, first_out);
    split_tile_store<LDS>(t, n, nrec, k, ent, tcount);
    if (threadIdx.x == 0) tile_out[t] = s_first_out;
}

__global__ void __launch_bounds__(1024) k_inject_scan(int nrec, int64_t max_count, const int64_t *count_dev, int *__restrict__ tcount,
                                                      const int *__restrict__ tile_out, int *__restrict__ removed, int *__restrict__ hdr)
{
    __shared__ int s_min;
    const int n = entry_count(count_dev, max_count), tiles = entry_tiles(n);
    const int tid = (int)threadIdx.x;
    if (tid == 0) s_min = INT_MAX;
    __syncthreads();
    int m = INT_MAX;
    for (int t = tid; t < tiles; t += 1024) m = min(m, tile_out[t]);
    if (m != INT_MAX) atomicMin(&s_min, m);
    for (int r = tid; r < nrec; r += 1024) {
        (void)split_tile_prefix(tcount, nrec, tiles, r);
        removed[r] = 0;
    }
    __syncthreads();
    if (tid == 0) { hdr[0] = s_min; hdr[1] = INT_MAX; }
}

__global__ void k_inject_fail(int nrec, int64_t max_count, const int64_t *count_dev, const int *__restrict__ tcount,
                              const QueueInfo *__restrict__ qinfo, int2 *__restrict__ ent, int *__restrict__ hdr)
{
    const int n = entry_count(count_dev, max_count);
    const int64_t i64 = (int64_t)blockIdx.x * blockDim.x + threadIdx.x;
    if (i64 >= n) return;
    const int i = (int)i64;
    int2 e = ent[i];
    if (e.x < 0) return;
    e.y += tcount[(size_t)(i / ENTRY_TILE) * nrec + e.x];
    ent[i] = e;
    if (e.y == qinfo[e.x].count) atomicMin(&hdr[1], i);
}

__global__ void k_inject_place(DevParams P, int64_t max_count, const int64_t *count_dev, const float4 *__restrict__ pos4,
                               const float4 *__restrict__ vel4, const float *__restrict__ fert, const int2 *__restrict__ ent,
                               const int *__restrict__ hdr, const QueueInfo *__restrict__ qinfo, int *__restrict__ queue,
                               int *__restrict__ ids, int *__restrict__ removed, float4 *d_pos4, float4 *d_vel4, float4 *d_acc4,
                               int *d_cell, uint8_t *d_pflags)
{
    const int n = entry_count(count_dev, max_count);
    const int64_t i64 = (int64_t)blockIdx.x * blockDim.x + threadIdx.x;
    if (i64 >= n) return;
    const int i = (int)i64;
    const int F = min(min(hdr[0], hdr[1]), n);
    const int2 e = ent[i];
    int slot = -1;
    if (i < F && e.x >= 0) {
        const QueueInfo q = qinfo[e.x];
        const int k = e.y;
        const int off = (q.front - q.rloc + k) % q.seg_size;
        const int qi = slot_index(P, q.rloc) + off;
        slot = queue[qi];
        queue[qi] = -1;
        const int si = slot_index(P, slot);
        if (si >= 0) {
            const float4 p = pos4[i];
            int cell = -1;
            (void)inject_locate(P, p.x, p.y, p.z, cell);
            d_pos4[si] = p;
            d_vel4[si] = vel4 ? vel4[i] : make_float4(0.f, 0.f, 0.f, 0.f);
            d_acc4[si] = make_float4(0.f, 0.f, 0.f, fert ? fert[i] : 0.f);
            d_cell[si] = cell;
            d_pflags[si] = 0;
        }
        atomicMax(&removed[e.x], k + 1);
    }
    if (ids) ids[i] = slot;
}

__global__ void __launch_bounds__(1024) k_inject_commit(int nrec, int64_t max_count, const int64_t *count_dev, const int *__restrict__ hdr,
                                                        const int *__restrict__ removed, QueueInfo *qinfo, psamd_inject_result *own,
                                                        psamd_inject_result *out)
{
    __shared__ unsigned long long s_placed[1];
    const int n = entry_count(count_dev, max_count);
    const int tid = (int)threadIdx.x;
    long long placed[1] = {0}, sum[1];
    for (int r = tid; r < nrec; r += 1024) {
        const int R = removed[r];
        if (R <= 0) continue;
        QueueInfo q = qinfo[r];
        q.count -= R;
        if (q.count == 0) { q.front = -1; q.rear = -1; }
        else q.front = q.rloc + (q.front - q.rloc + R) % q.seg_size;
        qinfo[r] = q;
        placed[0] += R;
    }
    block_sum(placed, s_placed, sum);
    if (tid == 0) {
        const int fo = hdr[0], ff = hdr[1];
        const int F = min(min(fo, ff), n);
        psamd_inject_result res;
        res.done = F;
        res.placed = sum[0];
        res.status = F == n ? PSAMD_OK : F == fo ? PSAMD_ERR_OUTSIDE_BOX : PSAMD_ERR_QUEUE_EMPTY;
        res.reserved = 0;
        write_result(own, out, res);
    }
}

hipError_t launch_inject(hipStream_t st, const DevParams &P, const SegLayout &S, const DeviceState &d, int nrec, const InjectArgs &a,
                         const InjectScratch &s)
{
    const int64_t tiles = (a.max_count + ENTRY_TILE - 1) / ENTRY_TILE;
    if (nrec <= SPLIT_LDS_RECORDS)
        k_inject_locate<true><<<(unsigned)tiles, SPLIT_THREADS, (size_t)nrec * sizeof(int), st>>>(P, S, nrec, d.celltab, a.pos4, a.max_count,
                                                                                                a.count_dev, s.e.ent, s.e.tcount, s.e.tile_out);
    else
        k_inject_locate<false><<<(unsigned)tiles, SPLIT_THREADS, 0, st>>>(P, S, nrec, d.celltab, a.pos4, a.max_count, a.count_dev,
                                                                        s.e.ent, s.e.tcount, s.e.tile_out);
    PS_LAUNCH_CHECK();
    k_inject_scan<<<1, 1024, 0, st>>>(nrec, a.max_count, a.count_dev, s.e.tcount, s.e.tile_out, s.removed, s.hdr);
    PS_LAUNCH_CHECK();
    const unsigned blocks = (unsigned)((a.max_count + 255) / 256);
    k_inject_fail<<<blocks, 256, 0, st>>>(nrec, a.max_count, a.count_dev, s.e.tcount, d.qinfo, s.e.ent, s.hdr);
    PS_LAUNCH_CHECK();
    k_inject_place<<<blocks, 256, 0, st>>>(P, a.max_count, a.count_dev, a.pos4, a.vel4, a.fert_age, s.e.ent, s.hdr, d.qinfo, d.queue,
                                           a.ids, s.removed, d.pos4, d.vel4, d.acc4, d.cell, d.pflags);
    PS_LAUNCH_CHECK();
    k_inject_commit<<<1, 1024, 0, st>>>(nrec, a.max_count, a.count_dev, s.hdr, s.removed, d.qinfo, s.own, a.result);
    PS_LAUNCH_CHECK();
    return hipSuccess;
}

}
```

particlesystem_amd/csrc/io.hip:

```cpp
#include <random>

#include "context.hpp"

int psamd::ensure_staging(psamd_ctx *c, size_t bytes)
{
    if (bytes <= c->staging_bytes) return PSAMD_OK;
    if (c->staging) (void)hipFree(c->staging);
    c->staging = nullptr; c->staging_bytes = 0;
    PS_HIP(c, hipMalloc(&c->staging, bytes));
    c->staging_bytes = bytes;
    return PSAMD_OK;
}

template <typename F>
static void for_owned_ranges(const psamd_ctx *c, F fn)
{
    size_t off = 0;
    for (int t = 0; t < 4; t++) {
        const int n = c->P.slot_n[t];
        if (n > 0) fn((size_t)c->P.slot_lo[t], (size_t)n, off);
        off += (size_t)n;
    }
}

// ... 302 lines not shown
    o->force_in = m[MSG_FORCE_IN].ptr; o->force_in_bytes = (int64_t)m[MSG_FORCE_IN].bytes;
    o->xfer_bytes = (int64_t)m[MSG_XFER_OUT].bytes; o->xfer2_bytes = (int64_t)m[MSG_XFER2_OUT].bytes;
    o->xfer_bytes_max = c->P.world > 1 ? (int64_t)xfer_msg_bytes((size_t)c->P.xfer_cap_max + 1) : 0;
    o->status_out = m[MSG_STATUS_OUT].ptr; o->status_in = m[MSG_STATUS_IN].ptr; o->status_bytes = (int64_t)m[MSG_STATUS_OUT].bytes;
    o->allg_out = m[MSG_ALLG_OUT].ptr; o->allg_in = m[MSG_ALLG_IN].ptr; o->allg_bytes = (int64_t)m[MSG_ALLG_OUT].bytes;
    o->far_out = m[MSG_FAR_OUT].ptr; o->far_in = m[MSG_FAR_IN].ptr; o->far_bytes = (int64_t)m[MSG_FAR_OUT].bytes;
    return PSAMD_OK;
}

static int msg_copy(psamd_ctx *c, int which, void *host, int64_t bytes, hipMemcpyKind kind)
{
    if (!c || !host || which < 0 || which >= MSG_COUNT || bytes < 0 || (size_t)bytes > c->msg[which].bytes) return PSAMD_ERR_INVALID_ARG;
    if (bytes == 0) return PSAMD_OK;
    const bool up = kind == hipMemcpyHostToDevice;
    PS_HIP(c, hipMemcpyAsync(up ? c->msg[which].ptr : host, up ? host : c->msg[which].ptr, (size_t)bytes, kind, c->stream));
    PS_HIP(c, hipStreamSynchronize(c->stream));
    return PSAMD_OK;
}

int psamd_slab_msg_download(psamd_ctx *c, int which, void *host, int64_t bytes) { return msg_copy(c, which, host, bytes, hipMemcpyDeviceToHost); }
int psamd_slab_msg_upload(psamd_ctx *c, int which, const void *host, int64_t bytes) { return msg_copy(c, which, (void *)host, bytes, hipMemcpyHostToDevice); }

int psamd_get_counters(psamd_ctx *c, psamd_counters *o)
{
    if (!c || !o) return PSAMD_ERR_INVALID_ARG;
    (void)drain_scalars(c, true);
    DevCounters copies[COUNTER_COPIES];
    PS_HIP(c, hipMemcpy(copies, c->d.ctr, sizeof copies, hipMemcpyDeviceToHost));
    DevCounters d{};
    for (const DevCounters &k : copies) {
        d.deaths_age += k.deaths_age; d.deaths_collision += k.deaths_collision; d.survives += k.survives;
        d.integrated += k.integrated; d.relocations += k.relocations; d.relocations_lost += k.relocations_lost;
        d.births += k.births; d.births_failed += k.births_failed; d.cell_overflow_kills += k.cell_overflow_kills;
    }
    o->deaths_age = (int64_t)d.deaths_age; o->deaths_collision = (int64_t)d.deaths_collision;
    o->survives = (int64_t)d.survives; o->integrated = (int64_t)d.integrated;
    o->relocations = (int64_t)d.relocations; o->relocations_lost = (int64_t)d.relocations_lost;
    o->births = (int64_t)d.births; o->births_failed = (int64_t)d.births_failed;
    o->cell_overflow_kills = (int64_t)d.cell_overflow_kills;
    o->steps = c->steps_total;
    o->particles_processed = c->processed_total;
    o->max_ops_one_queue = c->max_bucket_seen;
    return PSAMD_OK;
}

int psamd_live_count(psamd_ctx *c, int64_t *out)
{
    if (!c || !out) return PSAMD_ERR_INVALID_ARG;
    PS_HIP(c, hipStreamSynchronize(c->stream));
    std::vector<int> cells((size_t)std::max(c->P.slots_total, 1));
    PS_HIP(c, hipMemcpy(cells.data(), c->d.cell, (size_t)c->P.slots_total * sizeof(int), hipMemcpyDeviceToHost));
    int64_t n = 0;
    for (int i = 0; i < c->P.slots_total; i++) n += (cells[(size_t)i] >= 0 && cells[(size_t)i] < c->geo.num_cells) ? 1 : 0;
    *out = n;
    return PSAMD_OK;
}

int psamd_device_view_get(psamd_ctx *c, psamd_device_view *o)
{
    if (!c || !o) return PSAMD_ERR_INVALID_ARG;
    o->pos4 = c->d.pos4; o->vel4 = c->d.vel4; o->acc4 = c->d.acc4; o->cell = c->d.cell; o->pflags = c->d.pflags;
    o->sorted_id = c->d.sorted_id; o->snap_soa = c->d.snap_soa; o->sorted_cap = c->P.sorted_cap; o->force4 = c->d.force4; o->cell_start = c->d.cell_start;
    o->container_size = c->P.slots_total; o->num_cells = c->P.n_own_cells;
    o->live = c->live_at_build;
    o->stream = (void *)c->stream;
    return PSAMD_OK;
}

int psamd_download_force4(psamd_ctx *c, void *out, int64_t first, int64_t count)
{
    if (!c || !out || first < 0 || count < 0 || first + count > c->P.sorted_cap) return PSAMD_ERR_INVALID_ARG;
    if (count == 0) return PSAMD_OK;
    int rc = ensure_staging(c, (size_t)count * sizeof(float4));
    if (rc != PSAMD_OK) return rc;
    PS_HIP(c, launch_force_gather(c->stream, c->P, c->d, c->staging, (int)first, (int)count));
    PS_HIP(c, hipMemcpyAsync(out, c->staging, (size_t)count * sizeof(float4), hipMemcpyDeviceToHost, c->stream));
    PS_HIP(c, hipStreamSynchronize(c->stream));
    return PSAMD_OK;
}

static size_t snapshot_bytes(const psamd_ctx *c)
{
    const size_t C = (size_t)c->P.slots_total;
    return C * (3 * sizeof(float4) + sizeof(int) + 1) + (size_t)c->geo.queue_infos * sizeof(QueueInfo) + C * sizeof(int);
}

static int snapshot_copy(psamd_ctx *c, bool save)
{
    const size_t C = (size_t)c->P.slots_total;
    char *p = c->snapshot;
    char *s_pos = p, *s_vel = s_pos + C * sizeof(float4), *s_acc = s_vel + C * sizeof(float4);
    char *s_cell = s_acc + C * sizeof(float4);
    char *s_qinfo = s_cell + C * sizeof(int);
    char *s_queue = s_qinfo + (size_t)c->geo.queue_infos * sizeof(QueueInfo);
    char *s_flags = s_queue + C * sizeof(int);
    if (save) {
        struct { void *dev; char *snap; size_t bytes; } parts[] = {
            {c->d.pos4, s_pos, C * sizeof(float4)}, {c->d.vel4, s_vel, C * sizeof(float4)},
            {c->d.acc4, s_acc, C * sizeof(float4)}, {c->d.cell, s_cell, C * sizeof(int)},
            {c->d.pflags, s_flags, C},
        };
        for (auto &part : parts) PS_HIP(c, hipMemcpyAsync(part.snap, part.dev, part.bytes, hipMemcpyDeviceToDevice, c->stream));
        PS_HIP(c, hipMemcpyAsync(s_qinfo, c->d.qinfo, (size_t)c->geo.queue_infos * sizeof(QueueInfo), hipMemcpyDeviceToDevice, c->stream));
        PS_HIP(c, hipMemcpyAsync(s_queue, c->d.queue, C * sizeof(int), hipMemcpyDeviceToDevice, c->stream));
    } else {
        PS_HIP(c, launch_restore(c->stream, (int)C, s_pos, s_vel, s_acc, s_cell, s_flags, s_queue, s_qinfo,
                                 (int)((size_t)c->geo.queue_infos * sizeof(QueueInfo) / sizeof(int)), c->step, c->d));
    }
    return PSAMD_OK;
}

int psamd_snapshot_save(psamd_ctx *c)
{
    if (!c) return PSAMD_ERR_INVALID_ARG;
    if (!c->snapshot) PS_HIP(c, dev_alloc(c, &c->snapshot, snapshot_bytes(c)));
    c->snapshot_step = c->step;
    c->snapshot_live_bound = c->live_bound;
    return snapshot_copy(c, true);
}

int psamd_snapshot_restore(psamd_ctx *c)
{
    if (!c) return PSAMD_ERR_INVALID_ARG;
    if (!c->snapshot) return fail(c, PSAMD_ERR_STATE, "snapshot_restore without a saved snapshot");
    c->step = c->snapshot_step;
    c->live_bound = c->snapshot_live_bound;
    end_frame(c);
    c->frame_reset = false;
    return snapshot_copy(c, false);
}

int psamd_debug_wave_trace(psamd_ctx *c, uint64_t *out, int64_t n_words)
{
    if (!c || !out) return PSAMD_ERR_INVALID_ARG;
    const int64_t have = 3 * ((int64_t)c->P.n_local_cells * c->P.slices + 4);
    PS_HIP(c, hipStreamSynchronize(c->stream));
    PS_HIP(c, hipMemcpy(out, c->d.trace, (size_t)std::min(have, n_words) * sizeof(uint64_t), hipMemcpyDeviceToHost));
    return PSAMD_OK;
}

int psamd_selftest_math(psamd_ctx *c, uint32_t lo_bits, uint32_t hi_bits, uint64_t out24[24])
{
    if (!c || !out24 || hi_bits < lo_bits) return PSAMD_ERR_INVALID_ARG;
    unsigned long long *d = nullptr;
    PS_HIP(c, hipMalloc((void **)&d, 26 * sizeof(unsigned long long)));
    hipError_t e = hipMemsetAsync(d, 0, 26 * sizeof(unsigned long long), c->stream);
    if (e == hipSuccess) e = launch_selftest_math(c->stream, lo_bits, hi_bits, d);
    if (e == hipSuccess) e = hipStreamSynchronize(c->stream);
    if (e == hipSuccess) e = hipMemcpy(out24, d, 24 * sizeof(unsigned long long), hipMemcpyDeviceToHost);
    (void)hipFree(d);
    if (e != hipSuccess) return hip_fail(c, e, "selftest_math");
    return PSAMD_OK;
}

}
```

particlesystem_amd/csrc/kernels.h:

```cpp
#pragma once

#include <hip/hip_runtime.h>

#include "../../include/psamd.h"
#include "device_types.h"
#include "geometry.hpp"

namespace psamd {

constexpr int SLOT_TILE = 4096;
constexpr int ENTRY_TILE = 4096;
inline int slot_tiles(int slots_total) { return (slots_total + SLOT_TILE - 1) / SLOT_TILE; }
struct EntryScratch {
    int2 *ent;
    int *tcount;
    int *tile_out;
    int64_t cap;
};

constexpr int EXPORT_SUMS = 9;
struct __align__(16) ExportTile {
    double sum[EXPORT_SUMS];
    float lo[4], hi[4];
    int nonfinite, pad;
};
struct ExportFields {
    float4 *pos4, *vel4, *acc4;
    int *id, *cell;
};
struct ExportOut {
    int64_t count;
    psamd_live_stats stats;
};

struct InjectArgs {
    const float4 *pos4, *vel4;
    const float *fert_age;
    int64_t max_count;
    const int64_t *count_dev;
    int *ids;
    psamd_inject_result *result;
};
struct InjectScratch {
    EntryScratch e;
    int *removed;
    int *hdr;
    psamd_inject_result *own;
};

struct RemoveArgs {
    const int *ids;
    int64_t max_count;
    const int64_t *count_dev;
    int *outcome;
    psamd_remove_result *result;
};
struct RemoveScratch {
    EntryScratch e;
    int *claim;
    int2 *ins;
    int *prefix;
    int *tile_sel, *tile_live;
    psamd_remove_result *own;
};

constexpr int POT_TILE = SLOT_TILE;
struct __align__(16) PotTile {
    double u;
    float lo, hi;
    int listed, nonfinite;
    int pad[2];
};
struct PotOut {
    psamd_potential_result result;
    int64_t live;
};

struct SegLayout {
    int32_t seg_base[5];
    int32_t info_base[5];
    int32_t seg_size_t[4];
};

struct DeviceState {
    float4 *pos4 = nullptr;
    float4 *vel4 = nullptr;
    float4 *acc4 = nullptr;
    int *cell = nullptr;
    uint8_t *pflags = nullptr;
    uint32_t *tdata = nullptr;
    QueueInfo *qinfo = nullptr;
    int *queue = nullptr;
    int *cell_count = nullptr;
    int *chunk_count = nullptr;
    uint8_t *chunk_skip = nullptr;
    int2 *chunk_segs = nullptr;
    FrameScalars *fs = nullptr;
    FrameScalars *fs_host = nullptr;
    StepState *st = nullptr;
    int *cell_start = nullptr;
    int *cursor = nullptr;
    int *task_start = nullptr;
    int *task_list = nullptr;
    int *halo_count = nullptr;
    float *halo_f = nullptr;
    int *halo_id = nullptr;
    int *snap_cid = nullptr;
    int *active_list = nullptr;
    int *active_count = nullptr;
    int *task_list2 = nullptr;
    int *task_cost = nullptr;
    int *ctask_start = nullptr;
    long long *cost_start = nullptr;
    long long *wave_pos = nullptr;
    int *task_ready = nullptr;
    int4 *merged_tasks = nullptr;
    hipStream_t side_stream = nullptr;
    hipEvent_t ev_fork = nullptr, ev_join = nullptr;
    int *sorted_id = nullptr;
    float *snap_soa = nullptr;
    float *snap_age = nullptr;
    float4 *force4 = nullptr;
    int *cell_order = nullptr;
    uint8_t *flag_slot = nullptr;
    CellInfo *celltab = nullptr;
    uint64_t *op_keys = nullptr, *op_keys_sorted = nullptr;
    int *op_args = nullptr, *op_args_sorted = nullptr;
    int ops_cap = 0;
    int *rec_count = nullptr;
    int *rec_start = nullptr;
    int *rec_cursor = nullptr;
    MoveRec *moves = nullptr;
    int moves_cap = 0;
    float4 *stage = nullptr;
    XferRec *xfer_out[5] = {nullptr, nullptr, nullptr, nullptr, nullptr};
    int *status_out = nullptr;
    const int *allg_in = nullptr;
    int *gstart = nullptr, *gn = nullptr;
    float4 *part_acc = nullptr;
    int part_tasks = 0;
    int *act_start = nullptr;
    int *dense_gi = nullptr;
    int *dense_cell = nullptr;
    DevCounters *ctr = nullptr;
    int *exp_count = nullptr;
    ExportTile *exp_tiles = nullptr;
    ExportOut *exp_out = nullptr;
    float *pot_sorted = nullptr;
    float *pot_slot = nullptr;
    PotTile *pot_tiles = nullptr;
    int *pot_count = nullptr;
    PotOut *pot_out = nullptr;
    unsigned long long *trace = nullptr;
};

hipError_t launch_unpack_aos(hipStream_t st, const DevParams &P, const void *aos, int first, int count, float half_box,
                             const DeviceState &d);
hipError_t launch_pack_aos(hipStream_t st, const DevParams &P, void *aos, int first, int count, const DeviceState &d);
hipError_t launch_place(hipStream_t st, const DevParams &P, int n, const int *ids, const float4 *p, const float4 *v, const float4 *a,
                        const int *cells, const DeviceState &d);
hipError_t launch_fill_int(hipStream_t st, int *p, int v, size_t n);
hipError_t launch_restore(hipStream_t st, int n, const void *s_pos, const void *s_vel, const void *s_acc,
                          const void *s_cell, const void *s_flags, const void *s_queue, const void *s_qinfo, int qinfo_words,
                          int step, const DeviceState &d);
hipError_t launch_validate_eps(hipStream_t st, uint32_t lo_bits, uint32_t hi_bits, double eps2, float eps2f,
                               unsigned long long *out);
hipError_t launch_selftest_math(hipStream_t st, uint32_t lo_bits, uint32_t hi_bits, unsigned long long *out24);
hipError_t launch_init_tdata(hipStream_t st, const DevParams &P, const DeviceState &d);
hipError_t launch_build_grid(hipStream_t st, const DevParams &P, const DeviceState &d, hipEvent_t *ev, bool tdata_rows, bool big_cells);
hipError_t launch_force_gather(hipStream_t st, const DevParams &P, const DeviceState &d, void *out, int first, int count);
hipError_t launch_pairs(hipStream_t st, const DevParams &P, const DeviceState &d, hipEvent_t ev_force, int64_t tasks_hint, int pass, int64_t live_bound);
uint64_t launch_pairs_shape(const DevParams &P, int64_t tasks_hint);
void launch_collide(hipStream_t st, const DevParams &P, const DeviceState &d);
void launch_plan_force(hipStream_t st, const DevParams &P, const DeviceState &d, int nw, bool merge, int pass);
void launch_allpairs_far(hipStream_t st, const DevParams &P, const DeviceState &d, bool fast, int64_t live_bound);
hipError_t launch_apply(hipStream_t st, const DevParams &P, const SegLayout &S, const DeviceState &d);
hipError_t launch_frame_reset(hipStream_t st, const DeviceState &d, size_t frame_ints, int status_table);
hipError_t launch_lifecycle(hipStream_t st, const DevParams &P, const DeviceState &d, int nrec, int64_t live_hint, int cap0,
                            size_t frame_ints, int status_table);
hipError_t launch_pack_halos(hipStream_t st, const DevParams &P, const DeviceState &d, const int c0[2], const int ncell[2],
                             int *const msg[2], int *const pack_off[2]);
hipError_t launch_unpack_halos(hipStream_t st, const DevParams &P, const DeviceState &d, int ncell_below, const int *msg_below,
                               int *off_below, int ncell_above, const int *msg_above, int *off_above);
hipError_t launch_pack_force(hipStream_t st, const DevParams &P, const DeviceState &d, int *msg, int cap_bodies);
hipError_t launch_outbox_close(hipStream_t st, const DevParams &P, const DeviceState &d, int64_t live_hint, int *const msgs[5]);
hipError_t launch_inbox_merge(hipStream_t st, const DevParams &P, const DeviceState &d, const int *const msgs[5]);
hipError_t launch_allg_pack(hipStream_t st, const DevParams &P, const DeviceState &d, int *msg);
hipError_t launch_allg_index(hipStream_t st, const DevParams &P, const DeviceState &d);
hipError_t launch_chunk_census(hipStream_t st, const DevParams &P, const DeviceState &d, const int *status_all);
hipError_t launch_status_merge(hipStream_t st, const DevParams &P, const DeviceState &d, const int *status_all,
                               int force_j0, const int *force_msg, const int *pack_off);

hipError_t launch_export_live(hipStream_t st, const DevParams &P, const DeviceState &d, const ExportFields &out,
                              int64_t capacity, int64_t *count_out, psamd_live_stats *stats_out);

hipError_t launch_potential(hipStream_t st, const DevParams &P, const DeviceState &d, float *phi, int64_t capacity,
                            psamd_potential_result *result_dev);

hipError_t launch_inject(hipStream_t st, const DevParams &P, const SegLayout &S, const DeviceState &d, int nrec, const InjectArgs &a,
                         const InjectScratch &s);

hipError_t launch_remove_ids(hipStream_t st, const DevParams &P, const SegLayout &S, const DeviceState &d, int nrec, const RemoveArgs &a,
                             const RemoveScratch &s);
hipError_t launch_remove_box(hipStream_t st, const DevParams &P, const SegLayout &S, const DeviceState &d, int nrec, const float lo[3],
                             const float hi[3], bool outside, psamd_remove_result *result, const RemoveScratch &s);

}
```

particlesystem_amd/csrc/kernels_common.hpp:

```cpp
#pragma once

#include <hip/hip_runtime.h>
#include <type_traits>

#include <algorithm>
#include <cstdlib>

#include "device_types.h"
#include "geometry.hpp"
#include "kernels.h"

namespace psamd {

#define PS_LAUNCH_CHECK() do { hipError_t e_ = hipGetLastError(); if (e_ != hipSuccess) return e_; } while (0)
#define PS_WAVE_SYNC() do { __builtin_amdgcn_fence(__ATOMIC_SEQ_CST, "wavefront"); __builtin_amdgcn_wave_barrier(); } while (0)

static inline int blocks_for(size_t n, int threads, int cap = 4096)
{
    size_t b = (n + threads - 1) / threads;
    if (b > (size_t)cap) b = cap;
    return b < 1 ? 1 : (int)b;
}

constexpr int BALANCED_WAVES = 7;

static __constant__ signed char c_stencil[27][3] = {
    {0, 0, 0},
    {-1, 0, 0}, {+1, 0, 0},
    {-1, -1, 0}, {0, -1, 0}, {+1, -1, 0},
    {-1, +1, 0}, {0, +1, 0}, {+1, +1, 0},
    {-1, -1, -1}, {0, -1, -1}, {+1, -1, -1},
    {-1, 0, -1}, {0, 0, -1}, {+1, 0, -1},
    {-1, +1, -1}, {0, +1, -1}, {+1, +1, -1},
    {-1, -1, +1}, {0, -1, +1}, {+1, -1, +1},
    {-1, 0, +1}, {0, 0, +1}, {+1, 0, +1},
    {-1, +1, +1}, {0, +1, +1}, {+1, +1, +1},
};

__device__ __forceinline__ int xcd_contiguous(int b, int nb)
{
    const int xcd = b & 7, idx = b >> 3, q = nb >> 3, r = nb & 7;
    return (xcd < r ? xcd * (q + 1) : r * (q + 1) + (xcd - r) * q) + idx;
}

__device__ __forceinline__ int wave_incl_scan(int v)
{
    const int lane = (int)__lane_id();
    for (int d = 1; d < 64; d <<= 1) {
        const int o = __shfl_up(v, d);
        if (lane >= d) v += o;
    }
    return v;
}

constexpr int LDS_CELLS = 8192;
constexpr int SLOTS_PER_WG = 4096;

__device__ __forceinline__ int own_local_cell(const DevParams &P, int gc, FrameScalars *fs)
{
    if (gc < 0 || gc >= P.num_cells_global) return -1;
    const int lc = gc - P.reg_first[0] * P.G * P.G;
    if (lc < 0 || lc >= P.n_own_cells) { atomicOr(&fs->error, ERR_FOREIGN_CELL); return -1; }
    return lc;
}

__device__ __forceinline__ void chunk_cap_block(const DevParams &P, int ch, const int *__restrict__ chunk_count,
                                                const int *__restrict__ cell_arr, const CellInfo *__restrict__ celltab,
                                                const int2 *__restrict__ chunk_segs, uint8_t *__restrict__ chunk_skip,
                                                const int *__restrict__ before4)
{
    __shared__ int wave_tot[16];
    const int tid = threadIdx.x, lane = tid & 63, wv = tid >> 6;
    if (!before4 && chunk_count[ch] <= P.max_per_chunk) return;
    int run = 0, cur_t = -1;
    for (int sgi = 0; sgi < 27; sgi++) {
        const int2 sg = chunk_segs[ch * 27 + sgi];
        if (before4) {
            if (slot_index(P, sg.x) < 0) continue;
            const int t = sgi < 1 ? 0 : sgi < 7 ? 1 : sgi < 19 ? 2 : 3;
            if (t != cur_t) { cur_t = t; run = before4[t]; }
        }
        for (int b = 0; b < sg.y; b += 1024) {
            const int slot = sg.x + b + tid;
            int c = -1;
            if (b + tid < sg.y) c = cell_arr[slot_index(P, slot)];
            if (c <= -2) c = -2 - c;
            const bool in = c >= 0 && c < P.num_cells_global && celltab[c].chunk == ch;
            const unsigned long long m = __ballot(in);
            if (lane == 0) wave_tot[wv] = __popcll(m);
            __syncthreads();
            int before = 0, total = 0;
            for (int k = 0; k < 16; k++) { if (k < wv) before += wave_tot[k]; total += wave_tot[k]; }
            if (in) chunk_skip[slot_index(P, slot)] = (run + before + __popcll(m & ((1ull << lane) - 1ull))) >= P.max_per_chunk ? 1 : 0;
            run += total;
            __syncthreads();
        }
    }
}

constexpr int HALO_ALL = 0x40;
__device__ __forceinline__ bool finite3(float x, float y, float z)
{
    return (__float_as_uint(x) & 0x7f800000u) != 0x7f800000u && (__float_as_uint(y) & 0x7f800000u) != 0x7f800000u &&
           (__float_as_uint(z) & 0x7f800000u) != 0x7f800000u;
}

__device__ __forceinline__ int halo_dirs_of_numbers(const DevParams &P, int i1, int i2, int i3, float x, float y, float z);
__device__ __forceinline__ int halo_dirs(const DevParams &P, int i1, int i2, int i3, float x, float y, float z)
{
    if (!finite3(x, y, z)) return HALO_ALL;
    return halo_dirs_of_numbers(P, i1, i2, i3, x, y, z);
}

__device__ __forceinline__ int halo_dirs_of_numbers(const DevParams &P, int i1, int i2, int i3, float x, float y, float z)
{
    const int G = P.G;
    const float cs = (float)P.cell_size, half = (float)(G / 2), reach = P.halo_reach;
    const float u2 = (x / cs + half - (float)i2) * cs, u1 = (-y / cs + half - (float)i1) * cs,
                u3 = (-z / cs + half - (float)i3) * cs;
    int n2 = u2 < reach ? 1 : (cs - u2 < reach ? 2 : 0), n1 = u1 < reach ? 1 : (cs - u1 < reach ? 2 : 0),
        n3 = u3 < reach ? 1 : (cs - u3 < reach ? 2 : 0);
    if ((n2 == 1 && i2 == 0) || (n2 == 2 && i2 == G - 1)) n2 = 0;
    if ((n1 == 1 && i1 == 0) || (n1 == 2 && i1 == G - 1)) n1 = 0;
    if ((n3 == 1 && i3 == 0) || (n3 == 2 && i3 == G - 1)) n3 = 0;
    return n2 | (n1 << 2) | (n3 << 4);
}

__device__ __forceinline__ int halo_dir_of_subset(int dirs, int m)
{
    const int n2 = dirs & 3, n1 = (dirs >> 2) & 3, n3 = (dirs >> 4) & 3;
    if (((m & 1) && !n2) || ((m & 2) && !n1) || ((m & 4) && !n3)) return -1;
    const int d2 = (m & 1) ? (n2 == 1 ? -1 : 1) : 0, d1 = (m & 2) ? (n1 == 1 ? -1 : 1) : 0,
              d3 = (m & 4) ? (n3 == 1 ? -1 : 1) : 0;
    return (d3 + 1) * 9 + (d1 + 1) * 3 + (d2 + 1);
}

template <class F>
__device__ __forceinline__ void for_each_halo_dir(int dirs, F fn)
{
    if (dirs != HALO_ALL) {
#pragma unroll
        for (int m = 1; m < 8; m++) {
            const int dir = halo_dir_of_subset(dirs, m);
            if (dir >= 0) fn(dir);
        }
    } else {
// ... 145 lines not shown
```

particlesystem_amd/csrc/lifecycle.hip:

```cpp
#include "kernels_common.hpp"

namespace psamd {

constexpr int REPLAY_THREADS = 512;
constexpr int MSD_LEVELS = 4;

__device__ __forceinline__ void moves_stage_reset(const DevParams &P, int m, int n, MoveRec *moves,
                                                  float4 *pos4, float4 *vel4, float4 *acc4, int *cell_arr, uint8_t *pflags,
                                                  float4 *stage)
{
    const MoveRec r = moves[m];
    if (r.kind & MOVE_IN) return;
    const int kind = r.kind & 0xff;
    const int si = slot_index(P, r.src);
    const float4 zero = make_float4(0.f, 0.f, 0.f, 0.f);
    if (P.world > 1) {
        if (kind == 0) { cell_arr[si] = -1; pflags[si] = 0; pos4[si] = zero; vel4[si] = zero; acc4[si] = zero; }
        return;
    }
    if (kind == 1) {
        if (m + 1 < n) { const MoveRec nx = moves[m + 1]; if (nx.src == r.src && (nx.kind & 0xff) == 0) return; }
        float4 *s = stage + (size_t)3 * m;
        s[0] = pos4[si]; s[1] = vel4[si]; s[2] = acc4[si];
        return;
    }
    const float4 p = pos4[si], v = vel4[si], a = acc4[si];
    float4 *s = stage + (size_t)3 * m;
    s[0] = p; s[1] = v; s[2] = a;
    if (pflags[si]) moves[m].kind = MOVE_PARENT;
    if (m > 0) {
        const MoveRec pv = moves[m - 1];
        if (pv.src == r.src && (pv.kind & 0xff) == 1) { float4 *b = stage + (size_t)3 * (m - 1); b[0] = p; b[1] = v; b[2] = a; }
    }
    cell_arr[si] = -1; pflags[si] = 0; pos4[si] = zero; vel4[si] = zero; acc4[si] = zero;
}

__global__ __launch_bounds__(1024) void k_ops_hist(DevParams P, int nhist, const uint64_t *__restrict__ keys, const FrameScalars *fs,
                                                    int ops_cap, int rec_shift, int nrec, int *rec_count,
                                                    MoveRec *moves, int moves_cap, float4 *pos4, float4 *vel4, float4 *acc4,
                                                    int *cell_arr, uint8_t *pflags, float4 *stage)
{
    __shared__ int h[LDS_CELLS];
    const int tid = threadIdx.x;
    if ((int)blockIdx.x >= nhist) {
        const int nm = min(fs->n_moves, moves_cap), stride = ((int)gridDim.x - nhist) * 1024;
        for (int m = ((int)blockIdx.x - nhist) * 1024 + tid; m < nm; m += stride)
            moves_stage_reset(P, m, nm, moves, pos4, vel4, acc4, cell_arr, pflags, stage);
        return;
    }
    const int n = min(fs->n_ops, ops_cap);
    if ((long long)blockIdx.x * SLOTS_PER_WG >= n) return;
    const bool lds = nrec <= LDS_CELLS;
    if (lds) { for (int r = tid; r < nrec; r += 1024) h[r] = 0; __syncthreads(); }
    for (long long b0 = (long long)blockIdx.x * SLOTS_PER_WG; b0 < n; b0 += (long long)nhist * SLOTS_PER_WG)
        for (int i = tid; i < SLOTS_PER_WG; i += 1024) {
            const long long e = b0 + i;
            if (e < n) {
                const int r = (int)(keys[e] >> rec_shift);
                if (lds) atomicAdd(&h[r], 1); else atomicAdd(&rec_count[r], 1);
            }
        }
    if (lds) {
        __syncthreads();
        for (int r = tid; r < nrec; r += 1024) if (h[r]) atomicAdd(&rec_count[r], h[r]);
    }
}

__device__ __forceinline__ void publish_scalars(const FrameScalars *fs, FrameScalars *fs_host, int longest, StepState *st)
{
    constexpr int WORDS = (int)(sizeof(FrameScalars) / sizeof(int)), SKIP = (int)(offsetof(FrameScalars, max_bucket) / sizeof(int)),
                  SEQ = (int)(offsetof(FrameScalars, seq) / sizeof(int));
    static_assert(sizeof(FrameScalars) % sizeof(int) == 0, "copied word by word");
    const int seq = st->seq + 1;
    const int *src = reinterpret_cast<const int *>(fs);
    int *dst = reinterpret_cast<int *>(fs_host + (seq & 1));
    for (int i = threadIdx.x; i < WORDS; i += blockDim.x)
        if (i != SEQ) dst[i] = i == SKIP ? longest : src[i];
    __threadfence_system();
    __syncthreads();
    if (threadIdx.x == 0) {
        st->seq = seq; st->pending = 1;
        __hip_atomic_store(&fs_host[seq & 1].seq, seq, __ATOMIC_RELEASE, __HIP_MEMORY_SCOPE_SYSTEM);
    }
}

__global__ __launch_bounds__(1024) void k_ops_scan(int nrec, const int *__restrict__ rec_count,
                                                    int *__restrict__ rec_start, FrameScalars *fs, FrameScalars *fs_host, StepState *st)
{
    __shared__ int wave_tot[16];
    __shared__ int carry_s, max_s;
    const int tid = threadIdx.x, lane = tid & 63, wv = tid >> 6;
    if (tid == 0) { carry_s = 0; max_s = 0; }
    __syncthreads();
    int mymax = 0;
    for (int base = 0; base < nrec; base += 1024) {
        const int r = base + tid;
        const int v = (r < nrec) ? rec_count[r] : 0;
        mymax = max(mymax, v);
        const int incl = wave_incl_scan(v);
        if (lane == 63) wave_tot[wv] = incl;
        __syncthreads();
        int woff = 0;
        for (int k = 0; k < wv; k++) woff += wave_tot[k];
        const int excl = carry_s + woff + incl - v;
        if (r < nrec) rec_start[r] = excl;
        __syncthreads();
        if (tid == 1023) carry_s = excl + v;
        __syncthreads();
    }
    atomicMax(&max_s, mymax);
    __syncthreads();
    if (tid == 0) { rec_start[nrec] = carry_s; fs->max_bucket = max_s; }
    publish_scalars(fs, fs_host, max_s, st);
}

template <bool SCAN>
__global__ __launch_bounds__(1024) void k_ops_scatter(const uint64_t *__restrict__ keys, const int *__restrict__ args,
                                                       FrameScalars *fs, FrameScalars *fs_host, StepState *st, int ops_cap, int rec_shift, int nrec,
                                                       const int *__restrict__ rec_count, int *__restrict__ rec_start,
                                                       int *__restrict__ rec_cursor,
                                                       uint64_t *__restrict__ keys_out, int *__restrict__ args_out)
{
    __shared__ int h[LDS_CELLS];
    __shared__ int s_start[SCAN ? LDS_CELLS + 1 : 1];
    __shared__ int wave_tot[16];
    __shared__ int max_s;
    const int n = min(fs->n_ops, ops_cap);
    const int tid = threadIdx.x, lane = tid & 63, wv = tid >> 6;
    const bool publisher = SCAN && blockIdx.x == gridDim.x - 1;
    if ((long long)blockIdx.x * SLOTS_PER_WG >= n && (!SCAN || (blockIdx.x != 0 && !publisher))) return;
    const int *start = rec_start;
    if (SCAN) {
        if (tid == 0) max_s = 0;
        const int per = (nrec + 1023) / 1024, r0 = min(nrec, tid * per), r1 = min(nrec, r0 + per);
        int mine = 0, mymax = 0;
        for (int r = r0; r < r1; r++) { const int v = rec_count[r]; mine += v; mymax = max(mymax, v); }
        const int incl = wave_incl_scan(mine);
        if (lane == 63) wave_tot[wv] = incl;
        __syncthreads();
        if (mymax) atomicMax(&max_s, mymax);
        int run = incl - mine, total = 0;
        for (int k = 0; k < 16; k++) { if (k < wv) run += wave_tot[k]; total += wave_tot[k]; }
        for (int r = r0; r < r1; r++) { s_start[r] = run; run += rec_count[r]; }
        if (tid == 0) s_start[nrec] = total;
        __syncthreads();
        const int longest = max_s;
        if (blockIdx.x == 0) {
            for (int r = tid; r <= nrec; r += 1024) rec_start[r] = s_start[r];
            if (tid == 0) fs->max_bucket = longest;
        }
        if (publisher) publish_scalars(fs, fs_host, longest, st);
        start = s_start;
    }
    const bool lds = nrec <= LDS_CELLS;
    for (long long base = (long long)blockIdx.x * SLOTS_PER_WG; base < n; base += (long long)gridDim.x * SLOTS_PER_WG) {
        int mine[SLOTS_PER_WG / 1024];
        __syncthreads();
        if (lds) { for (int r = tid; r < nrec; r += 1024) h[r] = 0; __syncthreads(); }
#pragma unroll
        for (int i = 0; i < SLOTS_PER_WG / 1024; i++) {
            const long long e = base + i * 1024 + tid;
            mine[i] = (e < n) ? (int)(keys[e] >> rec_shift) : -1;
            if (lds && mine[i] >= 0) atomicAdd(&h[mine[i]], 1);
        }
        if (lds) {
            __syncthreads();
            for (int r = tid; r < nrec; r += 1024) { const int v = h[r]; if (v) h[r] = start[r] + atomicAdd(&rec_cursor[r], v); }
            __syncthreads();
        }
#pragma unroll
        for (int i = 0; i < SLOTS_PER_WG / 1024; i++)
            if (mine[i] >= 0) {
                const long long e = base + i * 1024 + tid;
                const int pos = lds ? atomicAdd(&h[mine[i]], 1) : start[mine[i]] + atomicAdd(&rec_cursor[mine[i]], 1);
                keys_out[pos] = keys[e]; args_out[pos] = args[e];
            }
    }
}

struct ParticleArrays { float4 *pos4, *vel4, *acc4; int *cell; uint8_t *pflags; };

__device__ __forceinline__ void commit_move(const DevParams &P, const StepState *__restrict__ stp, const MoveRec *__restrict__ moves, int m, int dst,
                                            const ParticleArrays &A, const float4 *__restrict__ stage)
{
    if (dst < 0) return;
    const MoveRec r = moves[m];
    const float4 *s = stage + (size_t)3 * m;
    const int di = slot_index(P, dst);
    if ((r.kind & 0xff) == 0) {
        A.pos4[di] = s[0]; A.vel4[di] = s[1]; A.acc4[di] = s[2];
        A.cell[di] = r.new_cell;
        A.pflags[di] = (r.kind & MOVE_PARENT) ? 1 : 0;
    } else {
        const uint64_t h0 = splitmix64(P.seed ^ ((uint64_t)(uint32_t)stp->step << 32) ^ (uint64_t)(uint32_t)r.src);
        const uint64_t h3 = splitmix64(splitmix64(splitmix64(h0)));
        const double u = (double)(h3 >> 11) * (1.0 / 9007199254740992.0);
        const float fert = (float)((double)P.fert_lo + u * (double)(P.fert_hi - P.fert_lo));
        const float4 pp = s[0], pv = s[1];
        A.pos4[di] = make_float4(pp.x, pp.y, pp.z, P.w_default);
        A.vel4[di] = make_float4((float)(-1.0 * (double)pv.x), (float)(-1.0 * (double)pv.y),
                                 (float)(-1.0 * (double)pv.z), 0.0f);
        A.acc4[di] = make_float4(0.f, 0.f, 0.f, fert);
        A.cell[di] = r.new_cell;
        A.pflags[di] = 0;
    }
}

struct SerialTally { unsigned long long lost = 0, reloc = 0, births = 0, births_failed = 0; };
template <typename At>
__device__ __forceinline__ void serial_op(QueueInfo &q, int sub, int arg, At at, MoveRec *moves, SerialTally &t)
{
    if (sub == 2) {
        if (q.count == q.seg_size) return;
        if (q.count == 0) { q.front = q.rloc; q.rear = q.rloc; }
        else if (q.rear == q.rloc + q.seg_size - 1) q.rear = q.rloc;
        else q.rear++;
        q.count++;
        at(q.rear) = arg;
    } else {
        int item = -1;
        if (q.count > 0) {
            const int pos = q.front;
            if (q.count == 1) { q.front = -1; q.rear = -1; }
            else if (q.front == q.rloc + q.seg_size - 1) q.front = q.rloc;
            else q.front++;
            q.count--;
            item = at(pos); at(pos) = -1;
        }
        moves[arg].dst = item;
        if (sub == 1) { if (item >= 0) t.reloc++; else t.lost++; }
        else { if (item >= 0) t.births++; else t.births_failed++; }
    }
}

template <bool ARGS>
__device__ __forceinline__ void lds_bitonic(uint64_t *kbuf, int *abuf, int np)
{
    constexpr int NT = REPLAY_THREADS;
    const int tid = threadIdx.x;
    for (int k = 2; k <= np; k <<= 1)
        for (int j = k >> 1; j > 0; j >>= 1) {
            for (int t = tid; t < (np >> 1); t += NT) {
                const int e = ((t & ~(j - 1)) << 1) | (t & (j - 1));
                const int partner = e | j;
                const uint64_t a = kbuf[e], b = kbuf[partner];
                const bool up = (e & k) == 0;
                if ((a > b) == up) {
                    kbuf[e] = b; kbuf[partner] = a;
                    if (ARGS) { const int x = abuf[e]; abuf[e] = abuf[partner]; abuf[partner] = x; }
                }
            }
            const int next_j = j > 1 ? (j >> 1) : k;
            if (j > 64 || next_j > 64) __syncthreads();
            else PS_WAVE_SYNC();
        }
    __syncthreads();
}

template <int CAP>
struct ReplayLds {
    static constexpr int KEY_BYTES = (CAP + 64) * 8, SORT_BYTES = KEY_BYTES + CAP * 4;
    static constexpr int WINDOW_SLOTS = KEY_BYTES / 4;
    static_assert(CAP * 4 <= KEY_BYTES, "abuf must survive the reuse of the key area");
    uint64_t *kbuf; int *abuf; int *window; unsigned char *sub; int *wave_tot; int *flag;
};

template <int CAP>
__device__ __forceinline__ void replay_short(const DevParams &P, const int rec, const int start, const int n,
                                             const uint64_t *__restrict__ keys, const int *__restrict__ args,
                                             QueueInfo *qinfo, int *queue, MoveRec *moves, DevCounters *ctr,
                                             const StepState *__restrict__ stp, const ParticleArrays &A, const float4 *__restrict__ stage,
                                             const ReplayLds<CAP> &L)
{
    constexpr int NT = REPLAY_THREADS;
    uint64_t *kbuf = L.kbuf;
    int *abuf = L.abuf, *window = L.window, *wave_tot = L.wave_tot;
    unsigned char *s_sub = L.sub;
    const int tid = threadIdx.x, lane = tid & 63, wv = tid >> 6;
    QueueInfo q = qinfo[rec];
    const bool in_lds = q.seg_size <= ReplayLds<CAP>::WINDOW_SLOTS;
    queue += slot_index(P, q.rloc) - q.rloc;
    constexpr int IDX_BITS = CAP == 2048 ? 11 : CAP == 4096 ? 12 : 13;
    static_assert((1 << IDX_BITS) >= CAP, "an operation's place in the bucket must fit");
    const bool packed_keys = P.key_rec_shift + IDX_BITS <= 64;
    const uint64_t low_mask = P.key_rec_shift >= 64 ? ~0ull : ((1ull << P.key_rec_shift) - 1ull);
    for (int e = tid; e < n; e += NT) {
// ... 316 lines not shown
    __shared__ unsigned char s_sub[CAP];
    __shared__ int wave_tot[2 * (REPLAY_THREADS / 64)];
    __shared__ int s_flag[3];
    __shared__ int s_cnt[MSD_LEVELS][256];
    __shared__ int s_cur[MSD_LEVELS], s_misc[2 * MSD_LEVELS];
    const int tid = threadIdx.x, rec = blockIdx.x;
    {
        const unsigned per = (frame_ints + gridDim.x - 1) / gridDim.x, a = min(frame_ints, blockIdx.x * per), b = min(frame_ints, a + per);
        for (unsigned i = a + tid; i < b; i += REPLAY_THREADS) frame[i] = 0;
        if (rec == 0) {
            if (tid == 0) {
                stp->last_departures = max(fs->n_out[0], fs->n_out[1]);
                const int err = fs->error; *fs = FrameScalars{}; fs->error = err;
            }
            if (status_out) {
                for (int i = tid; i < MSG_HEADER_WORDS; i += REPLAY_THREADS) status_out[i] = 0;
                for (int i = tid; i < status_table; i += REPLAY_THREADS) status_out[STATUS_CHUNK_OFF + i] = 0;
            }
        }
    }
    if (rec >= nrec) return;
    const int start = rec_start[rec], n = rec_start[rec + 1] - start;
    if (n <= 0) return;
    ReplayLds<CAP> L{reinterpret_cast<uint64_t *>(raw), reinterpret_cast<int *>(raw + ReplayLds<CAP>::KEY_BYTES), reinterpret_cast<int *>(raw),
                     s_sub, wave_tot, s_flag};
    if (n <= CAP) replay_short<CAP>(P, rec, start, n, keys, args, qinfo, queue, moves, ctr, stp, A, stage, L);
    else replay_long<CAP>(P, rec, start, n, keys, args, keys2, args2, qinfo, queue, moves, ctr, stp, A, stage, L, s_cnt, s_cur, s_misc);
}

__global__ void k_moves_stage(DevParams P, MoveRec *moves, int moves_cap, const FrameScalars *__restrict__ fs,
                              const float4 *pos4, const float4 *vel4, const float4 *acc4,
                              const uint8_t *pflags, float4 *stage, Outboxes out, OutboxMsgs msgs)
{
    const int g = blockIdx.x * blockDim.x + threadIdx.x;
    if (g < 5 && msgs.m[g]) {
        int *h = msgs.m[g];
        h[0] = min(fs->n_out[g], g < 2 ? P.xfer_cap : g < 4 ? P.xfer2_cap : P.far_cap); h[1] = 0; h[2] = fs->error;
        if (g == 4) h[3] = FAR_MAGIC;
    }
    const int n = min(fs->n_moves, moves_cap);
    for (int m = g; m < n; m += gridDim.x * blockDim.x) {
        const MoveRec r = moves[m];
        if (r.kind & MOVE_IN) continue;
        const int si = slot_index(P, r.src);
        if (r.kind & MOVE_OUT) {
            if (r.dst < 0) continue;
            XferRec *x = out.o[(r.kind & MOVE_FAR) ? 4 : ((r.kind & MOVE_UP) ? 1 : 0) + ((r.kind & MOVE_HOP2) ? 2 : 0)] + r.dst;
            const float4 p = pos4[si], v = vel4[si], a = acc4[si];
            x->pos[0] = p.x; x->pos[1] = p.y; x->pos[2] = p.z; x->pos[3] = p.w;
            x->vel[0] = v.x; x->vel[1] = v.y; x->vel[2] = v.z; x->vel[3] = v.w;
            x->acc[0] = a.x; x->acc[1] = a.y; x->acc[2] = a.z; x->acc[3] = a.w;
            if ((r.kind & 0xff) == 0 && pflags[si]) x->kind |= MOVE_PARENT;
            continue;
        }
        float4 *s = stage + (size_t)3 * m;
        s[0] = pos4[si]; s[1] = vel4[si]; s[2] = acc4[si];
        if (r.kind == 0 && pflags[si]) moves[m].kind = MOVE_PARENT;
    }
}

static int stride_blocks(int64_t items, int per_block, int cap)
{
    return (int)std::max<int64_t>(1, std::min<int64_t>((items + per_block - 1) / per_block, cap));
}

hipError_t launch_outbox_close(hipStream_t st, const DevParams &P, const DeviceState &d, int64_t live_hint, int *const msgs[5])
{
    const int64_t max_moves = std::min<int64_t>(d.moves_cap, 2 * std::max<int64_t>(live_hint, 1));
    k_moves_stage<<<stride_blocks(max_moves, 256, 2048), 256, 0, st>>>(P, d.moves, d.moves_cap, d.fs, d.pos4, d.vel4, d.acc4, d.pflags, d.stage,
                                      Outboxes{{d.xfer_out[0], d.xfer_out[1], d.xfer_out[2], d.xfer_out[3], d.xfer_out[4]}}, OutboxMsgs{{msgs[0], msgs[1], msgs[2], msgs[3], msgs[4]}});
    PS_LAUNCH_CHECK();
    return hipSuccess;
}

hipError_t launch_lifecycle(hipStream_t st, const DevParams &P, const DeviceState &d, int nrec, int64_t live_hint, int cap0,
                            size_t frame_ints, int status_table)
{
    const int64_t hint = std::max<int64_t>(live_hint, 1);
    const int64_t max_ops = std::max<int64_t>(1, std::min<int64_t>(d.ops_cap, 3 * hint));
    const int nwg = stride_blocks(max_ops, SLOTS_PER_WG, 2048);
    const int nhist = std::min(nwg, 512);
    const int nstage = stride_blocks(std::min<int64_t>(d.moves_cap, 2 * hint), 1024, 256);
    k_ops_hist<<<nhist + nstage, 1024, 0, st>>>(P, nhist, d.op_keys, d.fs, d.ops_cap, P.key_rec_shift, nrec, d.rec_count,
                                                d.moves, d.moves_cap, d.pos4, d.vel4, d.acc4, d.cell, d.pflags, d.stage);
    PS_LAUNCH_CHECK();
    if (nrec <= LDS_CELLS)
        k_ops_scatter<true><<<nwg, 1024, 0, st>>>(d.op_keys, d.op_args, d.fs, d.fs_host, d.st, d.ops_cap, P.key_rec_shift, nrec, d.rec_count, d.rec_start,
                                                  d.rec_cursor, d.op_keys_sorted, d.op_args_sorted);
    else {
        k_ops_scan<<<1, 1024, 0, st>>>(nrec, d.rec_count, d.rec_start, d.fs, d.fs_host, d.st);
        PS_LAUNCH_CHECK();
        k_ops_scatter<false><<<nwg, 1024, 0, st>>>(d.op_keys, d.op_args, d.fs, nullptr, nullptr, d.ops_cap, P.key_rec_shift, nrec, d.rec_count, d.rec_start,
                                                   d.rec_cursor, d.op_keys_sorted, d.op_args_sorted);
    }
    PS_LAUNCH_CHECK();
    const ParticleArrays A{d.pos4, d.vel4, d.acc4, d.cell, d.pflags};
    const int grid = std::max(nrec, 64);
#define PS_REPLAY(CAP) k_replay_commit<CAP><<<grid, REPLAY_THREADS, 0, st>>>(P, nrec, d.rec_start, d.op_keys_sorted, d.op_args_sorted, d.op_keys, d.op_args, \
        d.qinfo, d.queue, d.moves, d.ctr, d.st, A, d.stage, d.cell_count, (unsigned)frame_ints, d.fs, d.status_out, d.status_out ? status_table : 0)
    if (cap0 > 4096) PS_REPLAY(BUCKET_MAX); else if (cap0 > 2048) PS_REPLAY(4096); else PS_REPLAY(2048);
#undef PS_REPLAY
    PS_LAUNCH_CHECK();
    return hipSuccess;
}

}
```

particlesystem_amd/csrc/remove.hip:

```cpp
#include "multisplit.hpp"

namespace psamd {

enum { REM_REMOVED = 0, REM_NOT_LIVE = 1, REM_FOREIGN = 2, REM_INVALID = 3, REM_DROPPED = 4 };

__device__ __forceinline__ int remove_classify(const DevParams &P, int id, const int *__restrict__ cell)
{
    if (id < 0 || id >= P.container) return -1 - REM_INVALID;
    const int si = slot_index(P, id);
    if (si < 0) return -1 - REM_FOREIGN;
    return slot_live(P, cell[si]) ? si : -1 - REM_NOT_LIVE;
}

__device__ __forceinline__ void remove_reset(int si, float4 *d_pos4, float4 *d_vel4, float4 *d_acc4, int *d_cell, uint8_t *d_pflags)
{
    const float4 z = make_float4(0.f, 0.f, 0.f, 0.f);
    d_pos4[si] = z; d_vel4[si] = z; d_acc4[si] = z;
    d_cell[si] = -1;
    d_pflags[si] = 0;
}

__device__ __forceinline__ int remove_commit_record(QueueInfo *qinfo, int2 *__restrict__ ins, int r, int R)
{
    QueueInfo q = qinfo[r];
    const int room = q.seg_size - q.count, A = min(R, room);
    const int first = q.count == 0 ? 0 : (q.rear - q.rloc + 1) % q.seg_size;
    ins[r] = make_int2(first, room);
    if (A > 0) {
        if (q.count == 0) q.front = q.rloc;
        q.rear = q.rloc + (first + A - 1) % q.seg_size;
        q.count += A;
        qinfo[r] = q;
    }
    return R - A;
}

__device__ __forceinline__ int remove_insert(const DevParams &P, const QueueInfo *__restrict__ qinfo, const int2 *__restrict__ ins,
                                             int *__restrict__ queue, int r, int k, int id)
{
    const int2 rule = ins[r];
    if (k >= rule.y) return REM_DROPPED;
    const QueueInfo q = qinfo[r];
    queue[slot_index(P, q.rloc) + (rule.x + k) % q.seg_size] = id;
    return REM_REMOVED;
}


__global__ void k_remove_claim(DevParams P, int64_t max_count, const int64_t *count_dev, const int *__restrict__ ids,
                               const int *__restrict__ cell, int *__restrict__ claim)
{
    const int n = entry_count(count_dev, max_count);
    const int64_t i64 = (int64_t)blockIdx.x * blockDim.x + threadIdx.x;
    if (i64 >= n) return;
    const int si = remove_classify(P, ids[i64], cell);
    if (si >= 0) atomicMin(&claim[si], (int)i64);
}

template <bool LDS>
__global__ void __launch_bounds__(SPLIT_THREADS) k_remove_rank(DevParams P, SegLayout S, int nrec, int64_t max_count, const int64_t *count_dev,
                                                               const int *__restrict__ ids, const int *__restrict__ cell,
                                                               const int *__restrict__ claim, int2 *__restrict__ ent,
                                                               int *__restrict__ tcount, int *__restrict__ tile_out)
{
    extern __shared__ int lds_cnt[];
    __shared__ int s_out[3];
    const int n = entry_count(count_dev, max_count);
    const int t = (int)blockIdx.x, tid = (int)threadIdx.x;
    if (t * ENTRY_TILE >= n) return;
    if (tid < 3) s_out[tid] = 0;
    SplitKeys k;
    split_tile_begin<LDS>(t, nrec, lds_cnt, tcount, k);
#pragma unroll
    for (int g = 0; g < SPLIT_GROUPS; g++) {
        const int i = split_entry(t, g), lane = tid & 63;
        int r = INT_MIN;
        if (i < n) {
            const int id = ids[i];
            const int si = remove_classify(P, id, cell);
            r = si < 0 ? si : claim[si] == i ? segment_record_of_slot(S, id) : -1 - REM_NOT_LIVE;
        }
        k.rec[g] = r;
        split_group_rank(r, lane, k.in_rank[g], k.pop[g], k.lead[g]);
#pragma unroll
        for (int code = REM_NOT_LIVE; code <= REM_INVALID; code++) {
            const unsigned long long m = __ballot(r == -1 - code);
            if (lane == 0 && m) atomicAdd(&s_out[code - 1], __popcll(m));
        }
    }
    split_tile_store<LDS>(t, n, nrec, k, ent, tcount);
    if (tid < 3) tile_out[3 * t + tid] = s_out[tid];
}

__device__ __forceinline__ void remove_write_result(const long long (&v)[6], psamd_remove_result *own, psamd_remove_result *out)
{
    psamd_remove_result res;
    res.done = v[0]; res.removed = v[1]; res.not_live = v[2]; res.foreign = v[3]; res.invalid = v[4]; res.dropped = v[5];
    write_result(own, out, res);
}

__global__ void __launch_bounds__(1024) k_remove_commit(int nrec, int64_t max_count, const int64_t *count_dev, int *__restrict__ tcount,
                                                        const int *__restrict__ tile_out, QueueInfo *qinfo, int2 *__restrict__ ins,
                                                        psamd_remove_result *own, psamd_remove_result *out)
{
    __shared__ unsigned long long s_sum[6];
    const int n = entry_count(count_dev, max_count), tiles = entry_tiles(n);
    const int tid = (int)threadIdx.x;
    long long v[6] = {0, 0, 0, 0, 0, 0}, sum[6];
    for (int r = tid; r < nrec; r += 1024) {
        const int R = split_tile_prefix(tcount, nrec, tiles, r);
        if (R <= 0) continue;
        v[1] += R;
        v[5] += remove_commit_record(qinfo, ins, r, R);
    }
    for (int t = tid; t < tiles; t += 1024) { v[2] += tile_out[3 * t]; v[3] += tile_out[3 * t + 1]; v[4] += tile_out[3 * t + 2]; }
    block_sum(v, s_sum, sum);
    sum[0] = n;
    if (tid == 0) remove_write_result(sum, own, out);
}

__global__ void k_remove_place(DevParams P, int nrec, int64_t max_count, const int64_t *count_dev, const int *__restrict__ ids,
                               const int2 *__restrict__ ent, const int *__restrict__ tcount, const QueueInfo *__restrict__ qinfo,
                               const int2 *__restrict__ ins, int *__restrict__ queue, int *__restrict__ claim,
                               int *__restrict__ outcome, float4 *d_pos4, float4 *d_vel4, float4 *d_acc4, int *d_cell, uint8_t *d_pflags)
{
    const int n = entry_count(count_dev, max_count);
    const int64_t i64 = (int64_t)blockIdx.x * blockDim.x + threadIdx.x;
    if (i64 >= n) return;
    const int i = (int)i64;
    const int2 e = ent[i];
    int code = -1 - e.x;
    if (e.x >= 0) {
        const int id = ids[i], si = slot_index(P, id);
        const int k = e.y + tcount[(size_t)(i / ENTRY_TILE) * nrec + e.x];
        remove_reset(si, d_pos4, d_vel4, d_acc4, d_cell, d_pflags);
        claim[si] = INT_MAX;
        code = remove_insert(P, qinfo, ins, queue, e.x, k, id);
    }
    if (outcome) outcome[i] = code;
}


struct RemoveBox {
    float lo[3], hi[3];
    int outside;
    __device__ __forceinline__ bool selects(const float4 p) const
    {
        const bool in = lo[0] <= p.x && p.x < hi[0] && lo[1] <= p.y && p.y < hi[1] && lo[2] <= p.z && p.z < hi[2];
        return outside ? !in : in;
    }
};

__device__ __forceinline__ bool remove_box_selected(const DevParams &P, const RemoveBox &B, int i, const int *cell, const float4 *pos4,
                                                    bool &live)
{
    live = i < P.slots_total && slot_live(P, cell[i]);
    return live && B.selects(pos4[i]);
}

__global__ void __launch_bounds__(SLOT_THREADS) k_remove_box_count(DevParams P, RemoveBox B, const int *__restrict__ cell,
                                                                         const float4 *__restrict__ pos4, int *__restrict__ tile_sel,
                                                                         int *__restrict__ tile_live)
{
    __shared__ int s_n[SLOT_WAVES][2];
    const int lane = threadIdx.x & 63, wv = threadIdx.x >> 6, t = blockIdx.x;
    const int first = slot_first(t, wv, lane);
    int sel = 0, live = 0;
#pragma unroll 4
    for (int k = 0; k < SLOT_ITEMS; k++) {
        bool l;
        const bool s = remove_box_selected(P, B, first + 64 * k, cell, pos4, l);
        sel += __popcll(__ballot(s));
        live += __popcll(__ballot(l));
    }
    if (lane == 0) { s_n[wv][0] = sel; s_n[wv][1] = live; }
    __syncthreads();
    if (threadIdx.x == 0) {
        int a = 0, b = 0;
        for (int w = 0; w < SLOT_WAVES; w++) { a += s_n[w][0]; b += s_n[w][1]; }
        tile_sel[t] = a; tile_live[t] = b;
    }
}

__global__ void __launch_bounds__(SLOT_THREADS) k_remove_box_prefix(DevParams P, RemoveBox B, int ntiles, const int *__restrict__ cell,
                                                                          const float4 *__restrict__ pos4,
                                                                          const int *__restrict__ tile_sel, int *__restrict__ prefix)
{
    const int lane = threadIdx.x & 63, wv = threadIdx.x >> 6, t = blockIdx.x;
    const int before = tiles_before(tile_sel, t);
    const int first = slot_first(t, wv, lane);
    unsigned long long mask[SLOT_ITEMS];
    int sel = 0;
#pragma unroll
    for (int k = 0; k < SLOT_ITEMS; k++) {
        bool l;
        mask[k] = __ballot(remove_box_selected(P, B, first + 64 * k, cell, pos4, l));
        sel += __popcll(mask[k]);
    }
    int at = wave_offset<int>(before, sel, wv, lane);
#pragma unroll
    for (int k = 0; k < SLOT_ITEMS; k++) {
        const unsigned long long m = mask[k];
        const int i = first + 64 * k;
        if (i < P.slots_total) prefix[i] = at + lane_rank(m);
        at += __popcll(m);
    }
    if (t == ntiles - 1 && threadIdx.x == SLOT_THREADS - 1) prefix[P.slots_total] = at;
}

__global__ void __launch_bounds__(1024) k_remove_box_commit(DevParams P, int nrec, int ntiles, const int *__restrict__ prefix,
                                                            const int *__restrict__ tile_live, QueueInfo *qinfo, int2 *__restrict__ ins,
                                                            psamd_remove_result *own, psamd_remove_result *out)
{
    __shared__ unsigned long long s_sum[6];
    const int tid = (int)threadIdx.x;
    long long v[6] = {0, 0, 0, 0, 0, 0}, sum[6];
    for (int r = tid; r < nrec; r += 1024) {
        if (!owns_record(P, r)) continue;
        const int rloc = qinfo[r].rloc, seg = qinfo[r].seg_size, rs = slot_index(P, rloc);
        const int R = prefix[rs + seg] - prefix[rs];
        if (R <= 0) continue;
        v[1] += R;
        v[5] += remove_commit_record(qinfo, ins, r, R);
    }
    for (int t = tid; t < ntiles; t += 1024) v[0] += tile_live[t];
    block_sum(v, s_sum, sum);
    if (tid == 0) remove_write_result(sum, own, out);
}

__global__ void __launch_bounds__(SLOT_THREADS) k_remove_box_place(DevParams P, SegLayout S, RemoveBox B, const int *__restrict__ prefix,
                                                                         const QueueInfo *__restrict__ qinfo, const int2 *__restrict__ ins,
                                                                         int *__restrict__ queue, float4 *d_pos4, float4 *d_vel4,
                                                                         float4 *d_acc4, int *d_cell, uint8_t *d_pflags)
{
    const int i = (int)(blockIdx.x * SLOT_THREADS + threadIdx.x);
    bool live;
    if (!remove_box_selected(P, B, i, d_cell, d_pos4, live)) return;
    const int id = slot_of_index(P, i), r = segment_record_of_slot(S, id);
    const int k = prefix[i] - prefix[slot_index(P, qinfo[r].rloc)];
    remove_reset(i, d_pos4, d_vel4, d_acc4, d_cell, d_pflags);
    (void)remove_insert(P, qinfo, ins, queue, r, k, id);
}

hipError_t launch_remove_ids(hipStream_t st, const DevParams &P, const SegLayout &S, const DeviceState &d, int nrec, const RemoveArgs &a,
                             const RemoveScratch &s)
{
    const int64_t tiles = (a.max_count + ENTRY_TILE - 1) / ENTRY_TILE;
    const unsigned blocks = (unsigned)((a.max_count + 255) / 256);
    k_remove_claim<<<blocks, 256, 0, st>>>(P, a.max_count, a.count_dev, a.ids, d.cell, s.claim);
    PS_LAUNCH_CHECK();
    if (nrec <= SPLIT_LDS_RECORDS)
        k_remove_rank<true><<<(unsigned)tiles, SPLIT_THREADS, (size_t)nrec * sizeof(int), st>>>(P, S, nrec, a.max_count, a.count_dev, a.ids, d.cell,
                                                                                              s.claim, s.e.ent, s.e.tcount, s.e.tile_out);
    else
        k_remove_rank<false><<<(unsigned)tiles, SPLIT_THREADS, 0, st>>>(P, S, nrec, a.max_count, a.count_dev, a.ids, d.cell, s.claim, s.e.ent,
                                                                      s.e.tcount, s.e.tile_out);
    PS_LAUNCH_CHECK();
    k_remove_commit<<<1, 1024, 0, st>>>(nrec, a.max_count, a.count_dev, s.e.tcount, s.e.tile_out, d.qinfo, s.ins, s.own, a.result);
    PS_LAUNCH_CHECK();
    k_remove_place<<<blocks, 256, 0, st>>>(P, nrec, a.max_count, a.count_dev, a.ids, s.e.ent, s.e.tcount, d.qinfo, s.ins, d.queue, s.claim,
                                           a.outcome, d.pos4, d.vel4, d.acc4, d.cell, d.pflags);
    PS_LAUNCH_CHECK();
    return hipSuccess;
}

hipError_t launch_remove_box(hipStream_t st, const DevParams &P, const SegLayout &S, const DeviceState &d, int nrec, const float lo[3],
                             const float hi[3], bool outside, psamd_remove_result *result, const RemoveScratch &s)
{
    const int ntiles = slot_tiles(P.slots_total);
    RemoveBox B;
    for (int k = 0; k < 3; k++) { B.lo[k] = lo[k]; B.hi[k] = hi[k]; }
    B.outside = outside ? 1 : 0;
    if (ntiles > 0) {
        k_remove_box_count<<<ntiles, SLOT_THREADS, 0, st>>>(P, B, d.cell, d.pos4, s.tile_sel, s.tile_live);
        PS_LAUNCH_CHECK();
        k_remove_box_prefix<<<ntiles, SLOT_THREADS, 0, st>>>(P, B, ntiles, d.cell, d.pos4, s.tile_sel, s.prefix);
        PS_LAUNCH_CHECK();
    }
    k_remove_box_commit<<<1, 1024, 0, st>>>(P, ntiles > 0 ? nrec : 0, ntiles, s.prefix, s.tile_live, d.qinfo, s.ins, s.own, result);
    PS_LAUNCH_CHECK();
    if (ntiles > 0) {
        k_remove_box_place<<<ntiles * SLOT_ITEMS, SLOT_THREADS, 0, st>>>(P, S, B, s.prefix, d.qinfo, s.ins, d.queue,
                                                                                                      d.pos4, d.vel4, d.acc4, d.cell, d.pflags);
        PS_LAUNCH_CHECK();
    }
    return hipSuccess;
}

}
```

Measured before the change: 476.5 million.

## Add per-slot liveness bitmap to skip dead slots in hist, scatter, apply, restore

Adds a device bitmask with one bit per particle slot, kept in sync wherever a slot's cell is set or cleared (unpack, place, apply, sort, move commit, remove). The hist, scatter and apply kernels read cells through this bitmap, and hist and scatter return early when a whole workgroup has no live slots, so reads of the full cell array over dead slots are avoided. Restore uses the saved bitmap to skip slots that were dead both then and now. The cost is bitmap maintenance with atomics or extra stores on every lifecycle change, plus a risk of the bits drifting out of sync with the cell array.

```diff
diff --git a/include/psamd.h b/include/psamd.h
--- a/include/psamd.h
+++ b/include/psamd.h
@@ -291,6 +291,7 @@
 int psamd_live_count(psamd_ctx *ctx, int64_t *out);
 int psamd_device_view_get(psamd_ctx *ctx, psamd_device_view *out);
 int psamd_debug_wave_trace(psamd_ctx *ctx, uint64_t *out, int64_t n_words);
+int psamd_debug_download_liveness(psamd_ctx *ctx, uint32_t *out, int64_t n_words);
 
 int psamd_selftest_math(psamd_ctx *ctx, uint32_t lo_bits, uint32_t hi_bits, uint64_t out24[24]);
 #define PSAMD_NUM_TIMERS 9
diff --git a/particlesystem_amd/__init__.py b/particlesystem_amd/__init__.py
--- a/particlesystem_amd/__init__.py
+++ b/particlesystem_amd/__init__.py
@@ -245,6 +245,7 @@
     ("psamd_live_count", C.c_int, [_vp, C.POINTER(_i64)]),
     ("psamd_device_view_get", C.c_int, [_vp, C.POINTER(DeviceView)]),
     ("psamd_debug_wave_trace", C.c_int, [_vp, _vp, _i64]),
+    ("psamd_debug_download_liveness", C.c_int, [_vp, _vp, _i64]),
     ("psamd_selftest_math", C.c_int, [_vp, C.c_uint32, C.c_uint32, C.POINTER(C.c_uint64)]),
     ("psamd_set_graphs", C.c_int, [_vp, C.c_int]),
     ("psamd_get_graph_stats", C.c_int, [_vp, C.POINTER(_i64), C.POINTER(_i64)]),
@@ -721,6 +722,12 @@
         self._ck(self.lib.psamd_debug_wave_trace(self.h, _ptr(out), n))
         return out.reshape(-1, 3)
 
+    def liveness_bits(self):
+        n = self.owned_slots()
+        words = np.zeros((n + 31) // 32, np.uint32)
+        self._ck(self.lib.psamd_debug_download_liveness(self.h, _ptr(words), len(words)))
+        return np.unpackbits(words.view(np.uint8), bitorder="little")[:n].astype(bool)
+
     def selftest_math(self, lo_bits, hi_bits):
         out = (C.c_uint64 * 24)()
         self._ck(self.lib.psamd_selftest_math(self.h, lo_bits, hi_bits, out))
diff --git a/particlesystem_amd/csrc/apply.hip b/particlesystem_amd/csrc/apply.hip
--- a/particlesystem_amd/csrc/apply.hip
+++ b/particlesystem_amd/csrc/apply.hip
@@ -10,7 +10,7 @@
 __global__ __launch_bounds__(1024) void k_apply(DevParams P, SegLayout S, const StepState *__restrict__ stp,
                                                 const uint8_t *__restrict__ flag_slot,
                                                 float4 *pos4, float4 *vel4, float4 *acc4,
-                                                int *cell_arr, uint8_t *pflags,
+                                                int *cell_arr, unsigned *live_bits, uint8_t *pflags,
                                                 const CellInfo *__restrict__ celltab,
                                                 uint64_t *op_keys, int *op_args, int ops_cap,
                                                 MoveRec *moves, int moves_cap,
@@ -29,9 +29,8 @@
 #pragma unroll
     for (int it = 0; it < ITEMS; it++) {
         const int si = (blockIdx.x * ITEMS + it) * 1024 + (int)threadIdx.x;
-        int oc = -1;
-        if (si < P.slots_total) oc = cell_arr[si];
-        if (oc <= -2) { cell_arr[si] = -1; oc = -1; }
+        int oc = live_cell(P, live_bits, cell_arr, si);
+        if (oc <= -2) { cell_arr[si] = -1; live_clear(live_bits, si); oc = -1; }
         bool act = oc >= 0 && oc < P.num_cells_global;
         if (chunk_over && act && chunk_count[celltab[oc].chunk] > P.max_per_chunk && chunk_skip[si]) act = false;
         old_cells[it] = act ? oc : -1;
@@ -64,6 +63,7 @@
     if (killed) {
         died_of_age = v.w > P.life_thr;
         cell_arr[si] = -1; pflags[si] = 0;
+        live_clear(live_bits, si);
         pos4[si] = make_float4(0.f, 0.f, 0.f, 0.f);
         vel4[si] = make_float4(0.f, 0.f, 0.f, 0.f);
         acc4[si] = make_float4(0.f, 0.f, 0.f, 0.f);
@@ -239,7 +239,7 @@
 hipError_t launch_apply(hipStream_t st, const DevParams &P, const SegLayout &S, const DeviceState &d)
 {
     if (P.slots_total <= 0) return hipSuccess;
-    k_apply<<<(P.slots_total + 1023) / 1024, 1024, 0, st>>>(P, S, d.st, d.flag_slot, d.pos4, d.vel4, d.acc4, d.cell, d.pflags, d.celltab,
+    k_apply<<<(P.slots_total + 1023) / 1024, 1024, 0, st>>>(P, S, d.st, d.flag_slot, d.pos4, d.vel4, d.acc4, d.cell, d.live_bits, d.pflags, d.celltab,
                                                         d.op_keys, d.op_args, d.ops_cap, d.moves, d.moves_cap,
                                                         Outboxes{{d.xfer_out[0], d.xfer_out[1], d.xfer_out[2], d.xfer_out[3], d.xfer_out[4]}},
                                                         d.chunk_count, d.chunk_skip, d.fs, d.ctr);
diff --git a/particlesystem_amd/csrc/create.hip b/particlesystem_amd/csrc/create.hip
--- a/particlesystem_amd/csrc/create.hip
+++ b/particlesystem_amd/csrc/create.hip
@@ -277,6 +277,7 @@
     PS_HIP(c, dev_alloc(c, &c->rem.own, 1));
     PS_HIP(c, hipMemsetAsync(c->rem.own, 0, sizeof(psamd_remove_result), c->stream));
     PS_HIP(c, dev_alloc(c, &d.trace, 3 * (LC * P.slices + 4)));
+    PS_HIP(c, dev_alloc(c, &d.live_bits, live_words(P.slots_total)));
     PS_HIP(c, hipMemsetAsync(d.trace, 0, 3 * (LC * P.slices + 4) * sizeof(unsigned long long), c->stream));
     return PSAMD_OK;
 }
@@ -399,6 +400,7 @@
     PS_HIP(c, hipMemsetAsync(d.cell_count, 0, c->frame_ints * sizeof(int), c->stream));
     PS_HIP(c, hipMemsetAsync(d.cell_start, 0, (LC + 1) * sizeof(int), c->stream));
     PS_HIP(c, launch_fill_int(c->stream, d.cell, -1, C));
+    PS_HIP(c, hipMemsetAsync(d.live_bits, 0, live_words(P.slots_total) * sizeof(unsigned), c->stream));
     PS_HIP(c, launch_fill_int(c->stream, c->rem.claim, INT32_MAX, C));
     PS_HIP(c, launch_init_tdata(c->stream, P, d));
     g.initial_queues(c->h_qinfo, c->h_queue);
diff --git a/particlesystem_amd/csrc/grid.hip b/particlesystem_amd/csrc/grid.hip
--- a/particlesystem_amd/csrc/grid.hip
+++ b/particlesystem_amd/csrc/grid.hip
@@ -3,7 +3,7 @@
 namespace psamd {
 
 __global__ void k_unpack_aos(DevParams P, const uint32_t *__restrict__ aos, int first, int count, float half_box,
-                             float4 *pos4, float4 *vel4, float4 *acc4, int *cell, uint8_t *pflags,
+                             float4 *pos4, float4 *vel4, float4 *acc4, int *cell, unsigned *live_bits, uint8_t *pflags,
                              FrameScalars *fs)
 {
     const int i = blockIdx.x * blockDim.x + threadIdx.x;
@@ -32,6 +32,7 @@
         if (bad) atomicOr(&fs->error, ERR_BAD_POS);
     }
     cell[si] = (int)r[1];
+    if ((int)r[1] < 0) live_clear(live_bits, si); else live_set(live_bits, si);
     if ((int)r[1] < 0) {
         pflags[si] = 0;
         pos4[si] = vel4[si] = acc4[si] = make_float4(0.f, 0.f, 0.f, 0.f);
@@ -69,7 +70,7 @@
 __global__ void k_place(DevParams P, int n, const int *__restrict__ ids, const float4 *__restrict__ p,
                         const float4 *__restrict__ v, const float4 *__restrict__ a,
                         const int *__restrict__ cells, float4 *pos4, float4 *vel4, float4 *acc4,
-                        int *cell, uint8_t *pflags)
+                        int *cell, unsigned *live_bits, uint8_t *pflags)
 {
     const int i = blockIdx.x * blockDim.x + threadIdx.x;
     if (i >= n) return;
@@ -77,34 +78,36 @@
     if (si < 0) return;
     pos4[si] = p[i]; vel4[si] = v[i]; acc4[si] = a[i];
     cell[si] = cells[i]; pflags[si] = 0;
-}
-
-__global__ void k_restore(int n, const float4 *__restrict__ s_pos, const float4 *__restrict__ s_vel,
-                          const float4 *__restrict__ s_acc, const int *__restrict__ s_cell,
+    if (cells[i] < 0) live_clear(live_bits, si); else live_set(live_bits, si);
+}
+
+__global__ __launch_bounds__(256) void k_restore(int n, const float4 *__restrict__ s_pos, const float4 *__restrict__ s_vel,
+                          const float4 *__restrict__ s_acc, const int *__restrict__ s_cell, const unsigned *__restrict__ s_bits,
                           const uint8_t *__restrict__ s_flags, const int *__restrict__ s_queue,
                           const int *__restrict__ s_qinfo, int qinfo_words, int step, StepState *st,
-                          float4 *pos4, float4 *vel4, float4 *acc4, int *cell, uint8_t *pflags, int *queue, int *qinfo)
+                          float4 *pos4, float4 *vel4, float4 *acc4, int *cell, unsigned *live_bits, uint8_t *pflags, int *queue, int *qinfo)
 {
     const int i = blockIdx.x * blockDim.x + threadIdx.x;
     if (i == 0) { st->step = step; st->pending = 0; }
     if (i < qinfo_words) qinfo[i] = s_qinfo[i];
     if (i >= n) return;
     queue[i] = s_queue[i];
-    const int cs = s_cell[i];
-    if (cs < 0 && cell[i] < 0) return;
+    const unsigned then = s_bits[i >> 5], now = live_bits[i >> 5];
+    if ((i & 31) == 0 && then != now) live_bits[i >> 5] = then;
+    if (!(((then | now) >> (i & 31)) & 1u)) return;
     pos4[i] = s_pos[i]; vel4[i] = s_vel[i]; acc4[i] = s_acc[i];
-    cell[i] = cs; pflags[i] = s_flags[i];
+    cell[i] = s_cell[i]; pflags[i] = s_flags[i];
 }
 
 hipError_t launch_restore(hipStream_t st, int n, const void *s_pos, const void *s_vel, const void *s_acc,
-                          const void *s_cell, const void *s_flags, const void *s_queue, const void *s_qinfo, int qinfo_words,
+                          const void *s_cell, const void *s_bits, const void *s_flags, const void *s_queue, const void *s_qinfo, int qinfo_words,
                           int step, const DeviceState &d)
 {
     const int threads = std::max(std::max(n, qinfo_words), 1);
     k_restore<<<(threads + 255) / 256, 256, 0, st>>>(n, (const float4 *)s_pos, (const float4 *)s_vel, (const float4 *)s_acc,
-                                                    (const int *)s_cell, (const uint8_t *)s_flags, (const int *)s_queue,
+                                                    (const int *)s_cell, (const unsigned *)s_bits, (const uint8_t *)s_flags, (const int *)s_queue,
                                                     (const int *)s_qinfo, qinfo_words, step, d.st, d.pos4, d.vel4, d.acc4,
-                                                    d.cell, d.pflags, d.queue, (int *)d.qinfo);
+                                                    d.cell, d.live_bits, d.pflags, d.queue, (int *)d.qinfo);
     return hipGetLastError();
 }
 
@@ -139,19 +142,21 @@
 
 constexpr int SCAN_LDS_CHUNKS = 4096;
 
-__global__ __launch_bounds__(1024) void k_hist_lds(DevParams P, const int *__restrict__ cell, int *__restrict__ cell_count,
-                                                    FrameScalars *fs, StepState *st)
+__global__ __launch_bounds__(1024) void k_hist_lds(DevParams P, const int *__restrict__ cell, const unsigned *__restrict__ live_bits,
+                                                    int *__restrict__ cell_count, FrameScalars *fs, StepState *st)
 {
     __shared__ int h[LDS_CELLS];
     __shared__ int s_min;
     const int tid = threadIdx.x, base = blockIdx.x * SLOTS_PER_WG, ncell = P.n_own_cells;
     if (blockIdx.x == 0 && tid == 0 && st->pending) { st->step += 1; st->pending = 0; }
     int mine[SLOTS_PER_WG / 1024];
+    bool any = false;
 #pragma unroll
     for (int i = 0; i < SLOTS_PER_WG / 1024; i++) {
-        const int si = base + i * 1024 + tid;
-        mine[i] = si < P.slots_total ? own_local_cell(P, cell[si], fs) : -1;
-    }
+        mine[i] = own_local_cell(P, live_cell(P, live_bits, cell, base + i * 1024 + tid), fs);
+        any |= mine[i] >= 0;
+    }
+    if (!__syncthreads_or(any)) return;
     const int w0 = hist_window(P, mine, &s_min);
     if (w0 == 0x7fffffff) return;
     const int span = min(ncell - w0, LDS_CELLS);
@@ -170,7 +175,7 @@
     }
 }
 template <bool ROWS>
-__global__ __launch_bounds__(1024) void k_scatter_lds(DevParams P, int nwg, const int *__restrict__ cell, int *__restrict__ cursor,
+__global__ __launch_bounds__(1024) void k_scatter_lds(DevParams P, int nwg, const int *__restrict__ cell, const unsigned *__restrict__ live_bits, int *__restrict__ cursor,
                                                        int *__restrict__ sorted_id, const int *__restrict__ chunk_count,
                                                        const CellInfo *__restrict__ celltab, const int2 *__restrict__ chunk_segs,
                                                        uint8_t *__restrict__ chunk_skip,
@@ -182,17 +187,16 @@
     __shared__ int s_min;
     const int tid = threadIdx.x, base = blockIdx.x * SLOTS_PER_WG, ncell = P.n_own_cells;
     int mine[SLOTS_PER_WG / 1024];
+    bool any = false;
 #pragma unroll
     for (int i = 0; i < SLOTS_PER_WG / 1024; i++) {
-        const int si = base + i * 1024 + tid;
-        int c = -1;
-        if (si < P.slots_total) {
-            c = cell[si];
-            c = (c < 0 || c >= P.num_cells_global) ? -1 : c - P.reg_first[0] * P.G * P.G;
-            if (c < 0 || c >= ncell) c = -1;
-        }
+        int c = live_cell(P, live_bits, cell, base + i * 1024 + tid);
+        c = (c < 0 || c >= P.num_cells_global) ? -1 : c - P.reg_first[0] * P.G * P.G;
+        if (c < 0 || c >= ncell) c = -1;
         mine[i] = c;
-    }
+        any |= c >= 0;
+    }
+    if (!__syncthreads_or(any)) return;
     const int w0 = hist_window(P, mine, &s_min);
     if (w0 == 0x7fffffff) return;
     const int span = min(ncell - w0, LDS_CELLS);
@@ -328,7 +332,7 @@
 __device__ __forceinline__ void sort_cell(const DevParams &P, const int c, const bool take_big, const int *__restrict__ cell_start,
                                                      int *__restrict__ sorted_id, int *__restrict__ scratch_ids,
                                                      float4 *pos4, float4 *vel4, float4 *acc4,
-                                                     int *cell_arr, uint8_t *pflags,
+                                                     int *cell_arr, unsigned *live_bits, uint8_t *pflags,
                                                      float *__restrict__ snap_soa,
                                                      float *__restrict__ snap_age,
                                                      uint64_t *op_keys, int *op_args, int ops_cap,
@@ -426,6 +430,7 @@
         } else {
             sorted_id[start + e] = -1;
             cell_arr[si] = P.world > 1 ? -2 - cell_arr[si] : -1; pflags[si] = 0;
+            if (P.world == 1) live_clear(live_bits, si);
             pos4[si] = make_float4(0.f, 0.f, 0.f, 0.f);
             vel4[si] = make_float4(0.f, 0.f, 0.f, 0.f);
             acc4[si] = make_float4(0.f, 0.f, 0.f, 0.f);
@@ -509,7 +514,7 @@
 template <int CAP>
 __global__ __launch_bounds__(256) void k_sort_cells(DevParams P, int take_big, const int *__restrict__ cell_order, const int *__restrict__ cell_start, int *__restrict__ sorted_id,
                                                      int *__restrict__ scratch_ids,
-                                                     float4 *pos4, float4 *vel4, float4 *acc4, int *cell_arr, uint8_t *pflags,
+                                                     float4 *pos4, float4 *vel4, float4 *acc4, int *cell_arr, unsigned *live_bits, uint8_t *pflags,
                                                      float *__restrict__ snap_soa, float *__restrict__ snap_age,
                                                      uint64_t *op_keys, int *op_args, int ops_cap,
                                                      int *__restrict__ halo_count, float *__restrict__ halo_f,
@@ -517,13 +522,13 @@
                                                      int *__restrict__ status_out, FrameScalars *fs, DevCounters *ctr)
 {
     if (CAP == 1024) {
-        sort_cell<CAP>(P, cell_order[xcd_contiguous((int)blockIdx.x, (int)gridDim.x)], take_big != 0, cell_start, sorted_id, scratch_ids, pos4, vel4, acc4, cell_arr, pflags, snap_soa, snap_age,
+        sort_cell<CAP>(P, cell_order[xcd_contiguous((int)blockIdx.x, (int)gridDim.x)], take_big != 0, cell_start, sorted_id, scratch_ids, pos4, vel4, acc4, cell_arr, live_bits, pflags, snap_soa, snap_age,
                        op_keys, op_args, ops_cap, halo_count, halo_f, halo_id, snap_cid, status_out, fs, ctr);
         return;
     }
     if (fs->max_cell_raw <= 1024) return;
     for (int c = blockIdx.x; c < P.n_own_cells; c += gridDim.x) {
-        sort_cell<CAP>(P, c, true, cell_start, sorted_id, scratch_ids, pos4, vel4, acc4, cell_arr, pflags, snap_soa, snap_age,
+        sort_cell<CAP>(P, c, true, cell_start, sorted_id, scratch_ids, pos4, vel4, acc4, cell_arr, live_bits, pflags, snap_soa, snap_age,
                        op_keys, op_args, ops_cap, halo_count, halo_f, halo_id, snap_cid, status_out, fs, ctr);
         __syncthreads();
     }
@@ -534,7 +539,7 @@
 {
     if (count <= 0) return hipSuccess;
     k_unpack_aos<<<(count + 255) / 256, 256, 0, st>>>(P, (const uint32_t *)aos, first, count, half_box,
-                                                      d.pos4, d.vel4, d.acc4, d.cell, d.pflags, d.fs);
+                                                      d.pos4, d.vel4, d.acc4, d.cell, d.live_bits, d.pflags, d.fs);
     PS_LAUNCH_CHECK();
     return hipSuccess;
 }
@@ -552,7 +557,7 @@
                         const int *cells, const DeviceState &d)
 {
     if (n <= 0) return hipSuccess;
-    k_place<<<(n + 255) / 256, 256, 0, st>>>(P, n, ids, p, v, a, cells, d.pos4, d.vel4, d.acc4, d.cell, d.pflags);
+    k_place<<<(n + 255) / 256, 256, 0, st>>>(P, n, ids, p, v, a, cells, d.pos4, d.vel4, d.acc4, d.cell, d.live_bits, d.pflags);
     PS_LAUNCH_CHECK();
     return hipSuccess;
 }
@@ -621,24 +626,24 @@
 {
     const int nwg = std::max(1, (P.slots_total + SLOTS_PER_WG - 1) / SLOTS_PER_WG);
     if (ev) (void)hipEventRecord(ev[0], st);
-    k_hist_lds<<<nwg, 1024, 0, st>>>(P, d.cell, d.cell_count, d.fs, d.st);
+    k_hist_lds<<<nwg, 1024, 0, st>>>(P, d.cell, d.live_bits, d.cell_count, d.fs, d.st);
     PS_LAUNCH_CHECK();
     if (ev) (void)hipEventRecord(ev[1], st);
     k_scan<<<1, 1024, 0, st>>>(P, d.cell_count, d.cell_start, d.cursor, d.task_start, d.task_list, d.chunk_count, d.celltab, d.status_out, d.fs);
     PS_LAUNCH_CHECK();
     if (ev) (void)hipEventRecord(ev[2], st);
     const int grid = nwg + (P.world == 1 ? P.num_chunks : 0);
-    if (tdata_rows) k_scatter_lds<true><<<grid, 1024, 0, st>>>(P, nwg, d.cell, d.cursor, d.sorted_id, d.chunk_count, d.celltab, d.chunk_segs, d.chunk_skip, d.pos4, d.vel4, d.tdata);
-    else k_scatter_lds<false><<<grid, 1024, 0, st>>>(P, nwg, d.cell, d.cursor, d.sorted_id, d.chunk_count, d.celltab, d.chunk_segs, d.chunk_skip, d.pos4, d.vel4, d.tdata);
+    if (tdata_rows) k_scatter_lds<true><<<grid, 1024, 0, st>>>(P, nwg, d.cell, d.live_bits, d.cursor, d.sorted_id, d.chunk_count, d.celltab, d.chunk_segs, d.chunk_skip, d.pos4, d.vel4, d.tdata);
+    else k_scatter_lds<false><<<grid, 1024, 0, st>>>(P, nwg, d.cell, d.live_bits, d.cursor, d.sorted_id, d.chunk_count, d.celltab, d.chunk_segs, d.chunk_skip, d.pos4, d.vel4, d.tdata);
     PS_LAUNCH_CHECK();
     if (ev) (void)hipEventRecord(ev[3], st);
     k_sort_cells<1024><<<P.n_own_cells, 256, 0, st>>>(P, big_cells ? 0 : 1, d.cell_order, d.cell_start, d.sorted_id, d.active_list, d.pos4, d.vel4, d.acc4, d.cell,
-                                               d.pflags, d.snap_soa, d.snap_age, d.op_keys, d.op_args, d.ops_cap,
+                                               d.live_bits, d.pflags, d.snap_soa, d.snap_age, d.op_keys, d.op_args, d.ops_cap,
                                                P.two_pass ? d.halo_count : nullptr, d.halo_f, d.halo_id, d.snap_cid, d.status_out, d.fs, d.ctr);
     PS_LAUNCH_CHECK();
     if (big_cells) {
         k_sort_cells<SORT_MAX><<<std::min(P.n_own_cells, 512), 256, 0, st>>>(P, 1, d.cell_order, d.cell_start, d.sorted_id, d.active_list, d.pos4, d.vel4, d.acc4, d.cell,
-                                               d.pflags, d.snap_soa, d.snap_age, d.op_keys, d.op_args, d.ops_cap,
+                                               d.live_bits, d.pflags, d.snap_soa, d.snap_age, d.op_keys, d.op_args, d.ops_cap,
                                                P.two_pass ? d.halo_count : nullptr, d.halo_f, d.halo_id, d.snap_cid, d.status_out, d.fs, d.ctr);
         PS_LAUNCH_CHECK();
     }
diff --git a/particlesystem_amd/csrc/inject.hip b/particlesystem_amd/csrc/inject.hip
--- a/particlesystem_amd/csrc/inject.hip
+++ b/particlesystem_amd/csrc/inject.hip
@@ -88,7 +88,7 @@
                                const float4 *__restrict__ vel4, const float *__restrict__ fert, const int2 *__restrict__ ent,
                                const int *__restrict__ hdr, const QueueInfo *__restrict__ qinfo, int *__restrict__ queue,
                                int *__restrict__ ids, int *__restrict__ removed, float4 *d_pos4, float4 *d_vel4, float4 *d_acc4,
-                               int *d_cell, uint8_t *d_pflags)
+                               int *d_cell, unsigned *live_bits, uint8_t *d_pflags)
 {
     const int n = entry_count(count_dev, max_count);
     const int64_t i64 = (int64_t)blockIdx.x * blockDim.x + threadIdx.x;
@@ -113,6 +113,7 @@
             d_vel4[si] = vel4 ? vel4[i] : make_float4(0.f, 0.f, 0.f, 0.f);
             d_acc4[si] = make_float4(0.f, 0.f, 0.f, fert ? fert[i] : 0.f);
             d_cell[si] = cell;
+            if (cell >= 0) live_set(live_bits, si);
             d_pflags[si] = 0;
         }
         atomicMax(&removed[e.x], k + 1);
@@ -168,7 +169,7 @@
     k_inject_fail<<<blocks, 256, 0, st>>>(nrec, a.max_count, a.count_dev, s.e.tcount, d.qinfo, s.e.ent, s.hdr);
     PS_LAUNCH_CHECK();
     k_inject_place<<<blocks, 256, 0, st>>>(P, a.max_count, a.count_dev, a.pos4, a.vel4, a.fert_age, s.e.ent, s.hdr, d.qinfo, d.queue,
-                                           a.ids, s.removed, d.pos4, d.vel4, d.acc4, d.cell, d.pflags);
+                                           a.ids, s.removed, d.pos4, d.vel4, d.acc4, d.cell, d.live_bits, d.pflags);
     PS_LAUNCH_CHECK();
     k_inject_commit<<<1, 1024, 0, st>>>(nrec, a.max_count, a.count_dev, s.hdr, s.removed, d.qinfo, s.own, a.result);
     PS_LAUNCH_CHECK();
diff --git a/particlesystem_amd/csrc/io.hip b/particlesystem_amd/csrc/io.hip
--- a/particlesystem_amd/csrc/io.hip
+++ b/particlesystem_amd/csrc/io.hip
@@ -408,7 +408,8 @@
 static size_t snapshot_bytes(const psamd_ctx *c)
 {
     const size_t C = (size_t)c->P.slots_total;
-    return C * (3 * sizeof(float4) + sizeof(int) + 1) + (size_t)c->geo.queue_infos * sizeof(QueueInfo) + C * sizeof(int);
+    return C * (3 * sizeof(float4) + sizeof(int) + 1) + (size_t)c->geo.queue_infos * sizeof(QueueInfo) + C * sizeof(int) +
+           16 + live_words(c->P.slots_total) * sizeof(unsigned);
 }
 
 static int snapshot_copy(psamd_ctx *c, bool save)
@@ -420,17 +421,19 @@
     char *s_qinfo = s_cell + C * sizeof(int);
     char *s_queue = s_qinfo + (size_t)c->geo.queue_infos * sizeof(QueueInfo);
     char *s_flags = s_queue + C * sizeof(int);
+    char *s_bits = s_flags + (C + 15) / 16 * 16;
+    const size_t bits_bytes = live_words(c->P.slots_total) * sizeof(unsigned);
     if (save) {
         struct { void *dev; char *snap; size_t bytes; } parts[] = {
             {c->d.pos4, s_pos, C * sizeof(float4)}, {c->d.vel4, s_vel, C * sizeof(float4)},
             {c->d.acc4, s_acc, C * sizeof(float4)}, {c->d.cell, s_cell, C * sizeof(int)},
-            {c->d.pflags, s_flags, C},
+            {c->d.pflags, s_flags, C}, {c->d.live_bits, s_bits, bits_bytes},
         };
         for (auto &part : parts) PS_HIP(c, hipMemcpyAsync(part.snap, part.dev, part.bytes, hipMemcpyDeviceToDevice, c->stream));
         PS_HIP(c, hipMemcpyAsync(s_qinfo, c->d.qinfo, (size_t)c->geo.queue_infos * sizeof(QueueInfo), hipMemcpyDeviceToDevice, c->stream));
         PS_HIP(c, hipMemcpyAsync(s_queue, c->d.queue, C * sizeof(int), hipMemcpyDeviceToDevice, c->stream));
     } else {
-        PS_HIP(c, launch_restore(c->stream, (int)C, s_pos, s_vel, s_acc, s_cell, s_flags, s_queue, s_qinfo,
+        PS_HIP(c, launch_restore(c->stream, (int)C, s_pos, s_vel, s_acc, s_cell, s_bits, s_flags, s_queue, s_qinfo,
                                  (int)((size_t)c->geo.queue_infos * sizeof(QueueInfo) / sizeof(int)), c->step, c->d));
     }
     return PSAMD_OK;
@@ -462,6 +465,15 @@
     const int64_t have = 3 * ((int64_t)c->P.n_local_cells * c->P.slices + 4);
     PS_HIP(c, hipStreamSynchronize(c->stream));
     PS_HIP(c, hipMemcpy(out, c->d.trace, (size_t)std::min(have, n_words) * sizeof(uint64_t), hipMemcpyDeviceToHost));
+    return PSAMD_OK;
+}
+
+int psamd_debug_download_liveness(psamd_ctx *c, uint32_t *out, int64_t n_words)
+{
+    if (!c || !out || n_words < 0) return PSAMD_ERR_INVALID_ARG;
+    const int64_t have = ((int64_t)c->P.slots_total + 31) / 32;
+    PS_HIP(c, hipStreamSynchronize(c->stream));
+    PS_HIP(c, hipMemcpy(out, c->d.live_bits, (size_t)std::min(have, n_words) * sizeof(uint32_t), hipMemcpyDeviceToHost));
     return PSAMD_OK;
 }
 
diff --git a/particlesystem_amd/csrc/kernels.h b/particlesystem_amd/csrc/kernels.h
--- a/particlesystem_amd/csrc/kernels.h
+++ b/particlesystem_amd/csrc/kernels.h
@@ -11,6 +11,7 @@
 constexpr int SLOT_TILE = 4096;
 constexpr int ENTRY_TILE = 4096;
 inline int slot_tiles(int slots_total) { return (slots_total + SLOT_TILE - 1) / SLOT_TILE; }
+inline size_t live_words(int slots_total) { return (size_t)std::max(slot_tiles(slots_total), 1) * (SLOT_TILE / 32); }
 struct EntryScratch {
     int2 *ent;
     int *tcount;
@@ -87,6 +88,7 @@
     float4 *vel4 = nullptr;
     float4 *acc4 = nullptr;
     int *cell = nullptr;
+    unsigned *live_bits = nullptr;
     uint8_t *pflags = nullptr;
     uint32_t *tdata = nullptr;
     QueueInfo *qinfo = nullptr;
@@ -161,7 +163,7 @@
                         const int *cells, const DeviceState &d);
 hipError_t launch_fill_int(hipStream_t st, int *p, int v, size_t n);
 hipError_t launch_restore(hipStream_t st, int n, const void *s_pos, const void *s_vel, const void *s_acc,
-                          const void *s_cell, const void *s_flags, const void *s_queue, const void *s_qinfo, int qinfo_words,
+                          const void *s_cell, const void *s_bits, const void *s_flags, const void *s_queue, const void *s_qinfo, int qinfo_words,
                           int step, const DeviceState &d);
 hipError_t launch_validate_eps(hipStream_t st, uint32_t lo_bits, uint32_t hi_bits, double eps2, float eps2f,
                                unsigned long long *out);
diff --git a/particlesystem_amd/csrc/kernels_common.hpp b/particlesystem_amd/csrc/kernels_common.hpp
--- a/particlesystem_amd/csrc/kernels_common.hpp
+++ b/particlesystem_amd/csrc/kernels_common.hpp
@@ -62,6 +62,14 @@
     const int lc = gc - P.reg_first[0] * P.G * P.G;
     if (lc < 0 || lc >= P.n_own_cells) { atomicOr(&fs->error, ERR_FOREIGN_CELL); return -1; }
     return lc;
+}
+
+__device__ __forceinline__ bool live_bit(const unsigned *__restrict__ bits, int si) { return (bits[si >> 5] >> (si & 31)) & 1u; }
+__device__ __forceinline__ void live_set(unsigned *bits, int si) { atomicOr(&bits[si >> 5], 1u << (si & 31)); }
+__device__ __forceinline__ void live_clear(unsigned *bits, int si) { atomicAnd(&bits[si >> 5], ~(1u << (si & 31))); }
+__device__ __forceinline__ int live_cell(const DevParams &P, const unsigned *__restrict__ bits, const int *__restrict__ cell, int si)
+{
+    return (si < P.slots_total && live_bit(bits, si)) ? cell[si] : -1;
 }
 
 __device__ __forceinline__ void chunk_cap_block(const DevParams &P, int ch, const int *__restrict__ chunk_count,
diff --git a/particlesystem_amd/csrc/lifecycle.hip b/particlesystem_amd/csrc/lifecycle.hip
--- a/particlesystem_amd/csrc/lifecycle.hip
+++ b/particlesystem_amd/csrc/lifecycle.hip
@@ -6,7 +6,7 @@
 constexpr int MSD_LEVELS = 4;
 
 __device__ __forceinline__ void moves_stage_reset(const DevParams &P, int m, int n, MoveRec *moves,
-                                                  float4 *pos4, float4 *vel4, float4 *acc4, int *cell_arr, uint8_t *pflags,
+                                                  float4 *pos4, float4 *vel4, float4 *acc4, int *cell_arr, unsigned *live_bits, uint8_t *pflags,
                                                   float4 *stage)
 {
     const MoveRec r = moves[m];
@@ -15,7 +15,7 @@
     const int si = slot_index(P, r.src);
     const float4 zero = make_float4(0.f, 0.f, 0.f, 0.f);
     if (P.world > 1) {
-        if (kind == 0) { cell_arr[si] = -1; pflags[si] = 0; pos4[si] = zero; vel4[si] = zero; acc4[si] = zero; }
+        if (kind == 0) { cell_arr[si] = -1; live_clear(live_bits, si); pflags[si] = 0; pos4[si] = zero; vel4[si] = zero; acc4[si] = zero; }
         return;
     }
     if (kind == 1) {
@@ -33,19 +33,20 @@
         if (pv.src == r.src && (pv.kind & 0xff) == 1) { float4 *b = stage + (size_t)3 * (m - 1); b[0] = p; b[1] = v; b[2] = a; }
     }
     cell_arr[si] = -1; pflags[si] = 0; pos4[si] = zero; vel4[si] = zero; acc4[si] = zero;
+    live_clear(live_bits, si);
 }
 
 __global__ __launch_bounds__(1024) void k_ops_hist(DevParams P, int nhist, const uint64_t *__restrict__ keys, const FrameScalars *fs,
                                                     int ops_cap, int rec_shift, int nrec, int *rec_count,
                                                     MoveRec *moves, int moves_cap, float4 *pos4, float4 *vel4, float4 *acc4,
-                                                    int *cell_arr, uint8_t *pflags, float4 *stage)
+                                                    int *cell_arr, unsigned *live_bits, uint8_t *pflags, float4 *stage)
 {
     __shared__ int h[LDS_CELLS];
     const int tid = threadIdx.x;
     if ((int)blockIdx.x >= nhist) {
         const int nm = min(fs->n_moves, moves_cap), stride = ((int)gridDim.x - nhist) * 1024;
         for (int m = ((int)blockIdx.x - nhist) * 1024 + tid; m < nm; m += stride)
-            moves_stage_reset(P, m, nm, moves, pos4, vel4, acc4, cell_arr, pflags, stage);
+            moves_stage_reset(P, m, nm, moves, pos4, vel4, acc4, cell_arr, live_bits, pflags, stage);
         return;
     }
     const int n = min(fs->n_ops, ops_cap);
@@ -178,7 +179,7 @@
     }
 }
 
-struct ParticleArrays { float4 *pos4, *vel4, *acc4; int *cell; uint8_t *pflags; };
+struct ParticleArrays { float4 *pos4, *vel4, *acc4; int *cell; unsigned *live_bits; uint8_t *pflags; };
 
 __device__ __forceinline__ void commit_move(const DevParams &P, const StepState *__restrict__ stp, const MoveRec *__restrict__ moves, int m, int dst,
                                             const ParticleArrays &A, const float4 *__restrict__ stage)
@@ -190,6 +191,7 @@
     if ((r.kind & 0xff) == 0) {
         A.pos4[di] = s[0]; A.vel4[di] = s[1]; A.acc4[di] = s[2];
         A.cell[di] = r.new_cell;
+        live_set(A.live_bits, di);
         A.pflags[di] = (r.kind & MOVE_PARENT) ? 1 : 0;
     } else {
         const uint64_t h0 = splitmix64(P.seed ^ ((uint64_t)(uint32_t)stp->step << 32) ^ (uint64_t)(uint32_t)r.src);
@@ -202,6 +204,7 @@
                                  (float)(-1.0 * (double)pv.z), 0.0f);
         A.acc4[di] = make_float4(0.f, 0.f, 0.f, fert);
         A.cell[di] = r.new_cell;
+        live_set(A.live_bits, di);
         A.pflags[di] = 0;
     }
 }
@@ -684,7 +687,7 @@
     const int nhist = std::min(nwg, 512);
     const int nstage = stride_blocks(std::min<int64_t>(d.moves_cap, 2 * hint), 1024, 256);
     k_ops_hist<<<nhist + nstage, 1024, 0, st>>>(P, nhist, d.op_keys, d.fs, d.ops_cap, P.key_rec_shift, nrec, d.rec_count,
-                                                d.moves, d.moves_cap, d.pos4, d.vel4, d.acc4, d.cell, d.pflags, d.stage);
+                                                d.moves, d.moves_cap, d.pos4, d.vel4, d.acc4, d.cell, d.live_bits, d.pflags, d.stage);
     PS_LAUNCH_CHECK();
     if (nrec <= LDS_CELLS)
         k_ops_scatter<true><<<nwg, 1024, 0, st>>>(d.op_keys, d.op_args, d.fs, d.fs_host, d.st, d.ops_cap, P.key_rec_shift, nrec, d.rec_count, d.rec_start,
@@ -696,7 +699,7 @@
                                                    d.rec_cursor, d.op_keys_sorted, d.op_args_sorted);
     }
     PS_LAUNCH_CHECK();
-    const ParticleArrays A{d.pos4, d.vel4, d.acc4, d.cell, d.pflags};
+    const ParticleArrays A{d.pos4, d.vel4, d.acc4, d.cell, d.live_bits, d.pflags};
     const int grid = std::max(nrec, 64);
 #define PS_REPLAY(CAP) k_replay_commit<CAP><<<grid, REPLAY_THREADS, 0, st>>>(P, nrec, d.rec_start, d.op_keys_sorted, d.op_args_sorted, d.op_keys, d.op_args, \
         d.qinfo, d.queue, d.moves, d.ctr, d.st, A, d.stage, d.cell_count, (unsigned)frame_ints, d.fs, d.status_out, d.status_out ? status_table : 0)
diff --git a/particlesystem_amd/csrc/remove.hip b/particlesystem_amd/csrc/remove.hip
--- a/particlesystem_amd/csrc/remove.hip
+++ b/particlesystem_amd/csrc/remove.hip
@@ -12,8 +12,9 @@
     return slot_live(P, cell[si]) ? si : -1 - REM_NOT_LIVE;
 }
 
-__device__ __forceinline__ void remove_reset(int si, float4 *d_pos4, float4 *d_vel4, float4 *d_acc4, int *d_cell, uint8_t *d_pflags)
-{
+__device__ __forceinline__ void remove_reset(int si, float4 *d_pos4, float4 *d_vel4, float4 *d_acc4, int *d_cell, unsigned *live_bits, uint8_t *d_pflags)
+{
+    live_clear(live_bits, si);
     const float4 z = make_float4(0.f, 0.f, 0.f, 0.f);
     d_pos4[si] = z; d_vel4[si] = z; d_acc4[si] = z;
     d_cell[si] = -1;
@@ -121,7 +122,7 @@
 __global__ void k_remove_place(DevParams P, int nrec, int64_t max_count, const int64_t *count_dev, const int *__restrict__ ids,
                                const int2 *__restrict__ ent, const int *__restrict__ tcount, const QueueInfo *__restrict__ qinfo,
                                const int2 *__restrict__ ins, int *__restrict__ queue, int *__restrict__ claim,
-                               int *__restrict__ outcome, float4 *d_pos4, float4 *d_vel4, float4 *d_acc4, int *d_cell, uint8_t *d_pflags)
+                               int *__restrict__ outcome, float4 *d_pos4, float4 *d_vel4, float4 *d_acc4, int *d_cell, unsigned *live_bits, uint8_t *d_pflags)
 {
     const int n = entry_count(count_dev, max_count);
     const int64_t i64 = (int64_t)blockIdx.x * blockDim.x + threadIdx.x;
@@ -132,7 +133,7 @@
     if (e.x >= 0) {
         const int id = ids[i], si = slot_index(P, id);
         const int k = e.y + tcount[(size_t)(i / ENTRY_TILE) * nrec + e.x];
-        remove_reset(si, d_pos4, d_vel4, d_acc4, d_cell, d_pflags);
+        remove_reset(si, d_pos4, d_vel4, d_acc4, d_cell, live_bits, d_pflags);
         claim[si] = INT_MAX;
         code = remove_insert(P, qinfo, ins, queue, e.x, k, id);
     }
@@ -230,14 +231,14 @@
 __global__ void __launch_bounds__(SLOT_THREADS) k_remove_box_place(DevParams P, SegLayout S, RemoveBox B, const int *__restrict__ prefix,
                                                                          const QueueInfo *__restrict__ qinfo, const int2 *__restrict__ ins,
                                                                          int *__restrict__ queue, float4 *d_pos4, float4 *d_vel4,
-                                                                         float4 *d_acc4, int *d_cell, uint8_t *d_pflags)
+                                                                         float4 *d_acc4, int *d_cell, unsigned *live_bits, uint8_t *d_pflags)
 {
     const int i = (int)(blockIdx.x * SLOT_THREADS + threadIdx.x);
     bool live;
     if (!remove_box_selected(P, B, i, d_cell, d_pos4, live)) return;
     const int id = slot_of_index(P, i), r = segment_record_of_slot(S, id);
     const int k = prefix[i] - prefix[slot_index(P, qinfo[r].rloc)];
-    remove_reset(i, d_pos4, d_vel4, d_acc4, d_cell, d_pflags);
+    remove_reset(i, d_pos4, d_vel4, d_acc4, d_cell, live_bits, d_pflags);
     (void)remove_insert(P, qinfo, ins, queue, r, k, id);
 }
 
@@ -258,7 +259,7 @@
     k_remove_commit<<<1, 1024, 0, st>>>(nrec, a.max_count, a.count_dev, s.e.tcount, s.e.tile_out, d.qinfo, s.ins, s.own, a.result);
     PS_LAUNCH_CHECK();
     k_remove_place<<<blocks, 256, 0, st>>>(P, nrec, a.max_count, a.count_dev, a.ids, s.e.ent, s.e.tcount, d.qinfo, s.ins, d.queue, s.claim,
-                                           a.outcome, d.pos4, d.vel4, d.acc4, d.cell, d.pflags);
+                                           a.outcome, d.pos4, d.vel4, d.acc4, d.cell, d.live_bits, d.pflags);
     PS_LAUNCH_CHECK();
     return hipSuccess;
 }
@@ -280,7 +281,7 @@
     PS_LAUNCH_CHECK();
     if (ntiles > 0) {
         k_remove_box_place<<<ntiles * SLOT_ITEMS, SLOT_THREADS, 0, st>>>(P, S, B, s.prefix, d.qinfo, s.ins, d.queue,
-                                                                                                      d.pos4, d.vel4, d.acc4, d.cell, d.pflags);
+                                                                                                      d.pos4, d.vel4, d.acc4, d.cell, d.live_bits, d.pflags);
         PS_LAUNCH_CHECK();
     }
     return hipSuccess;
```

New measurement: 472.6 million. No clear change (-0.8%).
